# j04n-f/Encrypt-zkVM

Hardware: AMD Instinct MI355X
Metric: STARK prove: trace-steps/sec at 2^20 steps; achieved HBM GB/s vs 8 TB/s peak (higher is better)
Workload: dtype f128

## Files before the change

### encrypt-zkvm_amd/csrc/kernels.hip

```cpp
#include <hip/hip_runtime.h>
#include <bitset>
#include <mutex>
#include <stdlib.h>
#include <string.h>

#include "blake3.hpp"
#include "fri_small.hpp"
#include "rescue_consts.hpp"
#include "zk_internal.hpp"

namespace zk {

#define ZK_LAUNCH_CHECK() (void)hipGetLastError()

static inline unsigned cdiv(size_t a, size_t b) { return (unsigned)((a + b - 1) / b); }

__device__ __forceinline__ fe ld_fe(const fe *p) { return *p; }
__device__ __forceinline__ void st_fe(fe *p, fe v) { *p = v; }

template <class T>
__device__ __forceinline__ T pow_split(const T *lo, const T *hi, size_t t) {
    return ChalOf<T>::mul(lo[t & 2047], hi[t >> 11]);
}

// ... 1896 lines not shown
    comp_cross_mapped(st, m, T8n, inv3, scale, w8inv, inv3n, ncols, polys, nonzero_flag);
}

void comp_cross_mapped(hipStream_t st, const CrossMap &m, const NttTables &T8n, const PowTable &inv3, fe scale,
                       fe w8inv, fe inv3n, int ncols, fe *polys, unsigned *nonzero_flag) {
    unsigned blocks = cdiv(m.kcount, 256);
    if (blocks > 65536) blocks = 65536;
    ZK_PROF(st, "comp_cross", (128.0 + 16.0 * ncols) * m.kcount, hipLaunchKernelGGL(k_comp_cross, dim3(blocks), dim3(256), 0, st, m, T8n.inv_lo,
                                                 T8n.inv_hi, inv3.lo, inv3.hi, scale, w8inv, inv3n, ncols, polys,
                                                 nonzero_flag));
}

constexpr int OOD_GROUP = 7;

template <int KX>
__global__ void k_ood_tables(typename Chal<KX>::T z, typename Chal<KX>::T zg, uint64_t chunk, int nw,
                             typename Chal<KX>::T *tab) {
    typedef typename Chal<KX>::T T;
    const int t = blockIdx.x * blockDim.x + threadIdx.x;
    if (t >= 128 + 2 * nw) return;
    T x;
    uint64_t e;
    if (t < 128) {
        x = t < 64 ? z : zg;
        e = t & 63;
    } else {
        const int u = t - 128;
        x = u < nw ? z : zg;
        e = chunk * (uint64_t)(u < nw ? u : u - nw);
    }
    tab[t] = Chal<KX>::exp(x, e);
}

template <int KX, int E>
__global__ void __launch_bounds__(256) k_ood_eval(const fe *tpolys, int W, const fe *cpolys, int C, size_t n,
                                                  const typename Chal<KX>::T *tab, int nw, int w0, int w1,
                                                  fe *partials) {
    typedef Chal<KX> X;
    typedef typename X::T T;
    const int gw = w0 + (int)((blockIdx.x * blockDim.x + threadIdx.x) >> 6);
    const int lane = threadIdx.x & 63;
    const size_t plane = (size_t)(2 * W + C) * nw;
    const int tgroups = (W + OOD_GROUP - 1) / OOD_GROUP;
    const int g = blockIdx.y;
    const bool comp = g >= tgroups;
    const int p0 = comp ? 0 : g * OOD_GROUP;
    const int p1 = comp ? C : min(W, p0 + OOD_GROUP);
    const size_t base = (size_t)gw * 64 * E + lane;
    __shared__ T Y[2][E];
    if (threadIdx.x < 2 * E) {
        const int which = threadIdx.x / E, e = threadIdx.x % E;
        const T y = which ? X::mul(tab[127], tab[65]) : X::mul(tab[63], tab[1]);
        Y[which][e] = X::exp(y, (uint64_t)e);
    }
    __syncthreads();
    if (gw >= w1) return;
    const T wz = X::mul(tab[lane], tab[128 + gw]);
    const T wzg = comp ? X::zero() : X::mul(tab[64 + lane], tab[128 + nw + gw]);
    for (int p = p0; p < p1; p++) {
        const fe *c = (comp ? cpolys : tpolys) + (size_t)p * n;
        fe v[E];
#pragma unroll
        for (int e = 0; e < E; e++) {
            const size_t k = base + 64 * (size_t)e;
            v[e] = k < n ? c[k] : fe_zero();
        }
        const T hz = wave_sum(X::mul(dot_base<E>(v, Y[0]), wz));
        if (lane == 0) X::st(partials + (size_t)(comp ? 2 * W + p : p) * nw + gw, plane, hz);
        if (!comp) {
            const T hg = wave_sum(X::mul(dot_base<E>(v, Y[1]), wzg));
            if (lane == 0) X::st(partials + (size_t)(W + p) * nw + gw, plane, hg);
        }
    }
}

int ood_waves(size_t n) { return (int)std::max<size_t>(1, n / 1024); }

template <class T>
void ood_eval(hipStream_t st, const fe *tpolys, int W, const fe *cpolys, int C, int log_n, T z, T zg, fe *tab,
              fe *partials, fe *out, int rank, int G) {
    constexpr int KX = ChalOf<T>::KX;
    const size_t n = (size_t)1 << log_n;
    const int E = n >= 1024 ? 16 : std::max<int>(1, (int)(n / 64));
    const int nw = (int)((n + 64 * E - 1) / (64 * E));
    const int w0 = (int)((int64_t)nw * rank / G), w1 = (int)((int64_t)nw * (rank + 1) / G);
    T *t = reinterpret_cast<T *>(tab);
    hipLaunchKernelGGL(k_ood_tables<KX>, dim3(cdiv(128 + 2 * nw, 256)), dim3(256), 0, st, z, zg, (uint64_t)64 * E, nw, t);
    const dim3 grid(std::max(1u, cdiv(w1 - w0, 4)), (W + OOD_GROUP - 1) / OOD_GROUP + 1);
    const char *name = KX == 1 ? "ood_eval" : "ood_eval_ext";
#define ZK_OOD(EE) ZK_PROF(st, name, bytes, hipLaunchKernelGGL((k_ood_eval<KX, EE>), grid, dim3(256), 0, st, tpolys, W, cpolys, C, n, t, nw, w0, w1, partials))
    const double bytes = 16.0 * (W + C) * (double)n * (w1 - w0) / nw;
    switch (E) {
        case 16: ZK_OOD(16); break;
        case 8: ZK_OOD(8); break;
        case 4: ZK_OOD(4); break;
        case 2: ZK_OOD(2); break;
        default: ZK_OOD(1); break;
    }
#undef ZK_OOD
    sum_partials(st, partials, KX * (2 * W + C), nw, out, w0, w1);
}
template void ood_eval<fe>(hipStream_t, const fe *, int, const fe *, int, int, fe, fe, fe *, fe *, fe *, int, int);
template void ood_eval<fe2>(hipStream_t, const fe *, int, const fe *, int, int, fe2, fe2, fe *, fe *, fe *, int, int);

__global__ void k_sum_partials(const fe *partials, int nblk, int b0, int b1, fe *out) {
    __shared__ fe red[256];
    fe acc = fe_zero();
    for (int b = b0 + (int)threadIdx.x; b < b1; b += blockDim.x) acc = fe_add(acc, partials[(size_t)blockIdx.x * nblk + b]);
    red[threadIdx.x] = acc;
    __syncthreads();
    for (int s = 128; s > 0; s >>= 1) {
        if ((int)threadIdx.x < s) red[threadIdx.x] = fe_add(red[threadIdx.x], red[threadIdx.x + s]);
        __syncthreads();
    }
    if (threadIdx.x == 0) out[blockIdx.x] = red[0];
}

void sum_partials(hipStream_t st, const fe *partials, int npolys, int nblk, fe *out, int b0, int b1) {
    if (b1 < 0) b1 = nblk;
    hipLaunchKernelGGL(k_sum_partials, dim3(npolys), dim3(256), 0, st, partials, nblk, b0, b1, out);
}

constexpr int DIV_T = 256, DIV_E = 8, DIV_CH = DIV_T * DIV_E;
static_assert(DIV_CH == ZK_DEEP_RANGE_QUANTUM, "a sharded DEEP range is whole phase-3 chunks");
static_assert(DIV_T == ZK_DEEP_BLOCK, "DeepScratch counts phase-1 blocks");

template <int KX>
struct DeepPowBases {
    typename Chal<KX>::T b[4];
};
template <int KX>
__global__ void k_deep_pow_tables(DeepPowBases<KX> pb, size_t H, typename Chal<KX>::T *out) {
    const size_t per = 2048 + H;
    const size_t t = blockIdx.x * (size_t)blockDim.x + threadIdx.x;
    if (t >= 4 * per) return;
    const size_t b = t / per, e = t % per;
    const uint64_t ex = e < 2048 ? e : 2048 * (uint64_t)(e - 2048);
    out[t] = Chal<KX>::exp(pb.b[b], ex);
}

__device__ __forceinline__ fe block_sum256(fe v, fe *red) {
    v = wave_sum(v);
    const int w = threadIdx.x >> 6;
    if ((threadIdx.x & 63) == 0) red[w] = v;
    __syncthreads();
    fe r = red[0];
    for (int i = 1; i < DIV_T / 64; i++) r = fe_add(r, red[i]);
    __syncthreads();
    return r;
}

template <int KX>
__global__ void __launch_bounds__(DIV_T) k_deep_div_g(const fe *tpolys, const fe *cpolys, int ccols, size_t n,
                                                     const DeepConsts<KX> *D, const typename Chal<KX>::T *pw, size_t H,
                                                     typename Chal<KX>::T *g1, typename Chal<KX>::T *g2, fe *bs,
                                                     size_t kbase, size_t kend) {
    typedef Chal<KX> X;
    typedef typename X::T T;
    __shared__ fe red[DIV_T / 64];
    const size_t per = 2048 + H;
    const size_t k = kbase + blockIdx.x * (size_t)DIV_T + threadIdx.x;
    T v1 = X::zero(), v2 = X::zero();
    if (k < kend) {
        typename X::Acc aA = X::acc_zero();
#pragma unroll 4
        for (int c = 0; c < 28; c++) X::madd(aA, D->alpha_t[c], ld_fe(tpolys + (size_t)c * n + k));
        typename X::Acc aH = X::acc_zero();
        if constexpr (KX == 1) {
            for (int j = 0; j < ccols; j++) X::madd(aH, D->alpha_c[j], ld_fe(cpolys + (size_t)j * n + k));
        } else {
            for (int j = 0; j < ccols; j++) {
                const fe h0 = ld_fe(cpolys + (size_t)(2 * j) * n + k), h1 = ld_fe(cpolys + (size_t)(2 * j + 1) * n + k);
                const fe2 ac = D->alpha_c[j];
                acc288_madd(aH.a, ac.a, h0);
                acc288_madd(aH.a, ac.b, h1);
                acc288_madd(aH.b, ac.a, h1);
                acc288_madd(aH.b, ac.b, fe_add(h0, h1));
            }
        }
        const T A = X::reduce(aA);
        const T S = X::add(A, X::reduce(aH));
        v1 = X::mul(S, pow_split(pw, pw + 2048, k));
        v2 = X::mul(A, pow_split(pw + per, pw + per + 2048, k));
        g1[k] = v1;
        g2[k] = v2;
    }
    fe s[2 * KX];
#pragma unroll
    for (int c = 0; c < 2 * KX; c++) s[c] = block_sum256(X::comp(c < KX ? v1 : v2, c % KX), red);
    if (threadIdx.x == 0)
#pragma unroll
        for (int c = 0; c < 2 * KX; c++) bs[2 * KX * blockIdx.x + c] = s[c];
}

template <int NC>
__global__ void __launch_bounds__(1024) k_deep_div_scan(fe *bs, int nb, fe *total) {
    __shared__ fe t[NC][1024];
    const int per = (nb + 1023) / 1024, lo = threadIdx.x * per, hi = min(lo + per, nb);
    fe a[NC];
// ... 91 lines not shown
            if constexpr (!HOLD) r1 = X::add(r1, g1[k]), r2 = X::add(r2, g2[k]);
        }
        if constexpr (HOLD) r1 = X::add(r1, a[e]), r2 = X::add(r2, b[e]);
        pz = X::mul(pz, z);
        pg = X::mul(pg, zg);
    }
    if constexpr (KX == 1)
        if (rem_flag && k0 == 0 && !(fe_is_zero(r1) && fe_is_zero(r2))) atomicOr(rem_flag, 1u);
}

__global__ void __launch_bounds__(256) k_coset_to_natural(const fe *src, int log_n, int log_b, fe *out) {
    const size_t n = (size_t)1 << log_n, B = (size_t)1 << log_b, N = n << log_b;
    for (size_t i = blockIdx.x * (size_t)blockDim.x + threadIdx.x; i < N; i += (size_t)gridDim.x * blockDim.x)
        out[i] = ld_fe(src + (i & (B - 1)) * n + (i >> log_b));
}

void lde_cosets(hipStream_t st, const NttTables &Tn, const CosetTables &CT, const fe *coeffs, size_t n, size_t r0,
                size_t stride, int count, fe *out, fe *ntt_tmp) {
    ntt_lde(st, Tn, CT, coeffs, 0, 1, (int)r0, (int)stride, count, out, 0, n, ntt_tmp);
}

template <class T>
static void deep_tables(hipStream_t st, size_t n, T z, T zg, fe *scratch) {
    constexpr int KX = ChalOf<T>::KX;
    const DeepScratch S(scratch, n, KX);
    DeepPowBases<KX> pb;
    pb.b[0] = z;
    pb.b[1] = zg;
    pb.b[2] = ChalOf<T>::inv(z);
    pb.b[3] = ChalOf<T>::inv(zg);
    hipLaunchKernelGGL(k_deep_pow_tables<KX>, dim3(cdiv(4 * (2048 + S.H), 256)), dim3(256), 0, st, pb, S.H, (T *)S.pw);
}
template <class T>
static void deep_phase1(hipStream_t st, const fe *tpolys, const fe *cpolys, int ccols, size_t n,
                        const void *deep_consts_dev, fe *scratch, size_t k0, size_t kn, fe *total) {
    constexpr int KX = ChalOf<T>::KX;
    const DeepScratch S(scratch, n, KX);
    const size_t nb1 = (kn + DIV_T - 1) / DIV_T;
    ZK_PROF(st, "deep_combine", (16.0 * (28 + KX * ccols) + 32.0 * KX) * kn,
            hipLaunchKernelGGL(k_deep_div_g<KX>, dim3((unsigned)nb1), dim3(DIV_T), 0, st, tpolys, cpolys, ccols, n,
                               (const DeepConsts<KX> *)deep_consts_dev, (const T *)S.pw, S.H, (T *)S.g1, (T *)S.g2, S.bs, k0,
                               k0 + kn));
    hipLaunchKernelGGL(k_deep_div_scan<2 * KX>, dim3(1), dim3(1024), 0, st, S.bs, (int)nb1, total);
}
template <class T>
static void deep_phase3(hipStream_t st, size_t n, T z, T zg, fe *scratch, size_t k0, size_t kn, const fe *ext) {
    constexpr int KX = ChalOf<T>::KX;
    const DeepScratch S(scratch, n, KX);
    const size_t nb = (kn + DIV_CH - 1) / DIV_CH, nb1 = (kn + DIV_T - 1) / DIV_T;
    ZK_PROF(st, "deep_divide", KX * 48.0 * kn,
            hipLaunchKernelGGL((k_deep_div_q<KX, false>), dim3((unsigned)nb), dim3(DIV_T), 0, st, (const T *)S.g1,
                               (const T *)S.g2, S.bs, (int)nb1, k0 + kn, z, zg, (const T *)S.pw, S.H, S.out, n, nullptr, k0,
                               ext));
}
template <class T>
const fe *deep_poly(hipStream_t st, const fe *tpolys, const fe *cpolys, int ccols, int log_n,
                    const void *deep_consts_dev, T z, T zg, fe *scratch) {
    const size_t n = (size_t)1 << log_n;
    deep_tables(st, n, z, zg, scratch);
    deep_phase1<T>(st, tpolys, cpolys, ccols, n, deep_consts_dev, scratch, 0, n, nullptr);
    deep_phase3(st, n, z, zg, scratch, 0, n, nullptr);
    return DeepScratch(scratch, n, ChalOf<T>::KX).out;
}
template <class T>
const fe *deep_range_begin(hipStream_t st, const fe *tpolys, const fe *cpolys, int ccols, int log_n,
                           const void *deep_consts_dev, T z, T zg, fe *scratch, size_t k0, size_t kn) {
    const size_t n = (size_t)1 << log_n;
    deep_tables(st, n, z, zg, scratch);
    fe *total = DeepScratch(scratch, n, ChalOf<T>::KX).total;
    deep_phase1<T>(st, tpolys, cpolys, ccols, n, deep_consts_dev, scratch, k0, kn, total);
    return total;
}
template <class T>
const fe *deep_range_end(hipStream_t st, int log_n, T z, T zg, fe *scratch, size_t k0, size_t kn, const fe *ext) {
    const size_t n = (size_t)1 << log_n;
    deep_phase3(st, n, z, zg, scratch, k0, kn, ext);
    return DeepScratch(scratch, n, ChalOf<T>::KX).out;
}

struct BndPoly {
    fe cb[22];
    fe bnd1;
};
__global__ void __launch_bounds__(DIV_T) k_bnd_div_g(const fe *tpolys, size_t n, BndPoly bp, const fe *pw, size_t H,
                                                    fe *g1, fe *g2, fe *bs, size_t kbase, size_t kend) {
    __shared__ fe red[DIV_T / 64];
    const size_t per = 2048 + H;
    const size_t k = kbase + blockIdx.x * (size_t)DIV_T + threadIdx.x;
    fe v1 = fe_zero(), v2 = fe_zero();
    if (k < kend) {
        auto T = [&](int c) { return ld_fe(tpolys + (size_t)c * n + k); };
        acc288 a0 = acc288_zero(), a1 = acc288_zero();
        acc288_madd(a0, bp.cb[0], T(0));
        acc288_madd(a0, bp.cb[3], T(11));
        const fe t7 = T(7), t8 = T(8);
        acc288_madd(a0, bp.cb[1], t7);
        acc288_madd(a0, bp.cb[2], t8);
        acc288_madd(a1, bp.cb[12], t7);
        acc288_madd(a1, bp.cb[13], t8);
#pragma unroll
        for (int j = 0; j < 8; j++) {
            const fe c = T(12 + j);
            acc288_madd(a0, bp.cb[4 + j], c);
            acc288_madd(a1, bp.cb[14 + j], c);
        }
        v1 = acc288_reduce(a0);
        fe f1 = acc288_reduce(a1);
        if (k == 0) f1 = fe_sub(f1, bp.bnd1);
        v2 = fe_mul(f1, pow_split(pw + per, pw + per + 2048, k));
        g1[k] = v1;
        g2[k] = v2;
    }
    v1 = block_sum256(v1, red);
    v2 = block_sum256(v2, red);
    if (threadIdx.x == 0) {
        bs[2 * blockIdx.x] = v1;
        bs[2 * blockIdx.x + 1] = v2;
    }
}

static void bnd_tables_phase1(hipStream_t st, const fe *tpolys, size_t n, const AirConsts &K, fe c, fe *scratch,
                              size_t k0, size_t kn, fe *total) {
    const DeepScratch S(scratch, n, 1);
    const size_t nb1 = (kn + DIV_T - 1) / DIV_T;
    DeepPowBases<1> pb;
    pb.b[0] = fe_one();
    pb.b[1] = c;
    pb.b[2] = fe_one();
    pb.b[3] = fe_inv(c);
    hipLaunchKernelGGL(k_deep_pow_tables<1>, dim3(cdiv(4 * (2048 + S.H), 256)), dim3(256), 0, st, pb, S.H, S.pw);
    BndPoly bp;
    memcpy(bp.cb, K.coeff_b, sizeof bp.cb);
    bp.bnd1 = K.bnd1;
    ZK_PROF(st, "boundary_poly", (16.0 * 12 + 32.0) * kn,
            hipLaunchKernelGGL(k_bnd_div_g, dim3((unsigned)nb1), dim3(DIV_T), 0, st, tpolys, n, bp, S.pw, S.H, S.g1, S.g2,
                               S.bs, k0, k0 + kn));
    hipLaunchKernelGGL(k_deep_div_scan<2>, dim3(1), dim3(1024), 0, st, S.bs, (int)nb1, total);
}
static void bnd_phase3(hipStream_t st, size_t n, fe c, fe *scratch, size_t k0, size_t kn, const fe *ext, fe *col0,
                       unsigned *flag) {
    const DeepScratch S(scratch, n, 1);
    const size_t nb = (kn + DIV_CH - 1) / DIV_CH, nb1 = (kn + DIV_T - 1) / DIV_T;
    ZK_PROF(st, "boundary_poly", 64.0 * kn,
            hipLaunchKernelGGL((k_deep_div_q<1, true>), dim3((unsigned)nb), dim3(DIV_T), 0, st, S.g1, S.g2, S.bs, (int)nb1,
                               k0 + kn, fe_one(), c, S.pw, S.H, col0, 0, flag, k0, ext));
}

void boundary_poly_add(hipStream_t st, const fe *tpolys, int log_n, const AirConsts &K, fe c, fe *scratch, fe *col0,
                       unsigned *flag) {
    const size_t n = (size_t)1 << log_n;
    bnd_tables_phase1(st, tpolys, n, K, c, scratch, 0, n, nullptr);
    bnd_phase3(st, n, c, scratch, 0, n, nullptr, col0, flag);
}

const fe *boundary_range_begin(hipStream_t st, const fe *tpolys, int log_n, const AirConsts &K, fe c, fe *scratch,
                               size_t k0, size_t kn) {
    const size_t n = (size_t)1 << log_n;
    fe *total = DeepScratch(scratch, n, 1).total;
    bnd_tables_phase1(st, tpolys, n, K, c, scratch, k0, kn, total);
    return total;
}
void boundary_range_end(hipStream_t st, int log_n, fe c, fe *scratch, size_t k0, size_t kn, const fe *ext, fe *col0,
                        unsigned *flag) {
    bnd_phase3(st, (size_t)1 << log_n, c, scratch, k0, kn, ext, col0, flag);
}

template <class T>
void deep_coeff_launch(hipStream_t st, const NttTables &Tn, const fe *tpolys, const fe *cpolys, int ccols, int log_n,
                       int log_b, const void *deep_consts_dev, T z, T zg, const CosetTables &CT, fe *scratch,
                       fe *ulde, fe *ntt_tmp, fe *out) {
    constexpr int KX = ChalOf<T>::KX;
    const size_t n = (size_t)1 << log_n, B = (size_t)1 << log_b, N = n << log_b;
    const fe *Dk = deep_poly(st, tpolys, cpolys, ccols, log_n, deep_consts_dev, z, zg, scratch);
    for (int plane = 0; plane < KX; plane++) lde_cosets(st, Tn, CT, Dk + plane * n, n, 0, 1, (int)B, ulde + plane * N, ntt_tmp);
    if (!out) return;
    unsigned pb2 = cdiv(N, 256);
    if (pb2 > 65536) pb2 = 65536;
    for (int plane = 0; plane < KX; plane++)
        ZK_PROF(st, "deep", 32.0 * N,
                hipLaunchKernelGGL(k_coset_to_natural, dim3(pb2), dim3(256), 0, st, ulde + plane * N, log_n, log_b, out + plane * N));
}
#define ZK_DEEP_INSTANCES(T)                                                                                           \
    template const fe *deep_poly<T>(hipStream_t, const fe *, const fe *, int, int, const void *, T, T, fe *);          \
    template const fe *deep_range_begin<T>(hipStream_t, const fe *, const fe *, int, int, const void *, T, T, fe *,    \
                                           size_t, size_t);                                                            \
    template const fe *deep_range_end<T>(hipStream_t, int, T, T, fe *, size_t, size_t, const fe *);                    \
    template void deep_coeff_launch<T>(hipStream_t, const NttTables &, const fe *, const fe *, int, int, int,          \
                                       const void *, T, T, const CosetTables &, fe *, fe *, fe *, fe *);
ZK_DEEP_INSTANCES(fe)
ZK_DEEP_INSTANCES(fe2)
#undef ZK_DEEP_INSTANCES

__device__ __forceinline__ bool fe_canon_dev(uint32_t w0, uint32_t w1, uint32_t w2, uint32_t w3) {
    const uint64_t lo = (uint64_t)w0 | ((uint64_t)w1 << 32), hi = (uint64_t)w2 | ((uint64_t)w3 << 32);
    return !(hi == ZK_P_HI && lo >= ZK_P_LO);
}
__global__ void k_fri_coin(uint32_t *seed, const uint8_t *root, int k, fe *alpha_out, fe *alpha_log) {
    if (threadIdx.x != 0 || blockIdx.x != 0) return;
    uint32_t s[8], r[8], h[8];
    for (int i = 0; i < 8; i++) s[i] = seed[i];
    load_digest(root, r);
    b3::merge(s, r, h);
    for (int i = 0; i < 8; i++) seed[i] = h[i];
    for (uint32_t ctr = 1; ctr < 1000; ctr++) {
        uint32_t m[16] = {h[0], h[1], h[2], h[3], h[4], h[5], h[6], h[7], ctr, 0, 0, 0, 0, 0, 0, 0};
        uint32_t d[8];
        b3::iv(d);
        b3::compress(d, m, 0, 0, 40, b3::CHUNK_START | b3::CHUNK_END | b3::ROOT);
        if (fe_canon_dev(d[0], d[1], d[2], d[3]) && (k == 1 || fe_canon_dev(d[4], d[5], d[6], d[7]))) {
            const fe a0 = fe{(uint64_t)d[0] | ((uint64_t)d[1] << 32), (uint64_t)d[2] | ((uint64_t)d[3] << 32)};
            const fe a1 = fe{(uint64_t)d[4] | ((uint64_t)d[5] << 32), (uint64_t)d[6] | ((uint64_t)d[7] << 32)};
            alpha_out[0] = alpha_log[0] = a0;
            if (k == 2) alpha_out[1] = alpha_log[1] = a1;
            return;
        }
    }
}

void fri_coin_launch(hipStream_t st, uint32_t *seed_dev, const uint8_t *root_dev, int k, fe *alpha_dev,
                     fe *alpha_log) {
// ... 179 lines not shown
```

### encrypt-zkvm_amd/csrc/prover.hip

```cpp
#include <hip/hip_runtime.h>
#include <stdio.h>
#include <string.h>

#include <algorithm>
#include <chrono>
#include <cstdlib>
#include <map>
#include <memory>
#include <new>
#include <string>
#include <vector>

#include "host_pool.hpp"
#include "prover_internal.hpp"
#include "rescue_consts.hpp"

namespace zk {
thread_local std::string g_err;
struct HostTimer {
    bool on = getenv("ZK_HOST_TIMING") != nullptr;
    std::chrono::steady_clock::time_point t = std::chrono::steady_clock::now();
    std::string log;
    void start() { t = std::chrono::steady_clock::now(); }
    void stop(const char *what) {
// ... 485 lines not shown
    out->hint_redos = p->hint_redos;
    for (const auto &h : p->hint_sets) out->hint_sets += h.n != 0 && h.have ? 1u : 0u;
    out->hinted_sparse = p->tc.sp_hinted;
    out->derived = p->tc.clk_used ? 1u : 0u;
    for (int i = 0; i < zk_prover::ZK_FIXED_SNAPS; i++) {
        const auto &s = p->fix_snaps[i];
        out->fixed_sets += s.live && s.owner >= 0 && p->hint_sets[s.owner].snap == i ? 1u : 0u;
    }
    return ZK_OK;
}

int zk_prover_upload_stats(zk_prover *p, uint64_t *bytes, uint32_t *sparse_cols, uint32_t *narrow8_cols,
                           uint32_t *narrow32_cols) {
    if (!p) ZK_FAIL(ZK_ERR_INVALID_ARG, "null prover");
    if (bytes) *bytes = p->tc.up_bytes;
    if (sparse_cols) *sparse_cols = p->tc.up_sparse;
    if (narrow8_cols) *narrow8_cols = p->tc.up_nw8;
    if (narrow32_cols) *narrow32_cols = p->tc.up_nw32;
    return ZK_OK;
}

int zk_prover_upload_derived(zk_prover *p, uint32_t *derived_cols) {
    if (!p || !derived_cols) ZK_FAIL(ZK_ERR_INVALID_ARG, "null argument");
    *derived_cols = p->tc.clk_used ? 1u : 0u;
    return ZK_OK;
}

int zk_prover_upload_fixed(zk_prover *p, uint32_t *fixed_cols) {
    if (!p || !fixed_cols) ZK_FAIL(ZK_ERR_INVALID_ARG, "null argument");
    *fixed_cols = p->tc.fix_used;
    return ZK_OK;
}

int zk_prover_exchange_stats_ex(zk_prover *p, const char **names, float *ms, float *exposed_ms, double *bytes,
                                int *calls, int cap, int *count) {
    if (!p) ZK_FAIL(ZK_ERR_INVALID_ARG, "null prover");
    std::vector<const char *> nm;
    std::vector<float> t, w;
    std::vector<double> b;
    std::vector<int> c;
    if (p->stage_done)
        for (const auto &r : p->xchg) {
            float x = 0, y = 0;
            (void)hipEventElapsedTime(&x, p->xchg_pool[r.ev], p->xchg_pool[r.ev + 1]);
            if (r.waited) (void)hipEventElapsedTime(&y, p->xchg_pool[r.ev + 2], p->xchg_pool[r.ev + 3]);
            size_t i = 0;
            while (i < nm.size() && strcmp(nm[i], r.name)) i++;
            if (i == nm.size()) {
                nm.push_back(r.name);
                t.push_back(0);
                w.push_back(0);
                b.push_back(0);
                c.push_back(0);
            }
            t[i] += x;
            w[i] += y;
            b[i] += r.bytes;
            c[i] += 1;
        }
    const int k = (int)nm.size();
    for (int i = 0; i < k && i < cap; i++) {
        if (names) names[i] = nm[i];
        if (ms) ms[i] = t[i];
        if (exposed_ms) exposed_ms[i] = w[i];
        if (bytes) bytes[i] = b[i];
        if (calls) calls[i] = c[i];
// ... 525 lines not shown
    return d2h_small(p, root, nodes + 32, 32);
}

static void coset_major_rows_to_host(zk_prover *p, const fe *base, int ncols, size_t n, uint32_t B, uint8_t *dst) {
    size_t N = n * B;
    std::vector<fe> h((size_t)ncols * N);
    (void)hipMemcpy(h.data(), base, h.size() * sizeof(fe), hipMemcpyDeviceToHost);
    fe *o = reinterpret_cast<fe *>(dst);
    for (int c = 0; c < ncols; c++)
        for (size_t i = 0; i < N; i++) o[i * ncols + c] = h[((size_t)c * B + (i % B)) * n + i / B];
}

int zk::ensure_ext(zk_prover *p) {
    if (p->x_comp) return ZK_OK;
    const size_t n = p->max_n, N = n * p->max_b, CE = 8 * n;
    const size_t Nl = p->shard_world ? N / (size_t)p->shard_world : N;
    DeviceArena &A = p->arena;
    ZK_CHECK_HIP(A.alloc(&p->x_comp, 2 * CE));
    ZK_CHECK_HIP(A.alloc(&p->x_ctmp, 2 * CE));
    ZK_CHECK_HIP(A.alloc(&p->x_clde, (size_t)2 * 8 * Nl));
    ZK_CHECK_HIP(A.alloc(&p->x_deep, 2 * Nl));
    ZK_CHECK_HIP(A.alloc(&p->x_fri, 2 * (N + 16)));
    ZK_CHECK_HIP(A.alloc(&p->x_partials, (size_t)2 * (2 * ZK_MAX_COLS + ZK_MAX_CCOLS) * ood_waves(n)));
    ZK_CHECK_HIP(A.alloc(&p->x_tab, (size_t)2 * (128 + 2 * ood_waves(n))));
    ZK_CHECK_HIP(A.alloc((uint8_t **)&p->x_air, 2 * sizeof(AirConsts)));
    ZK_CHECK_HIP(A.alloc((uint8_t **)&p->x_deep_consts, sizeof(DeepConsts<2>)));
    ZK_CHECK_HIP(A.alloc((uint8_t **)&p->x_fold_consts, sizeof(FoldConsts<2>)));
    if (!p->shard_world) ZK_CHECK_HIP(A.alloc(&p->x_ulde, 2 * N));
    ZK_CHECK_HIP(A.alloc(&p->x_dscratch, DeepScratch::size(n, 2)));
    return ZK_OK;
}

static int composition_stage(zk_prover *p, Plan *pl, int KX, int C, fe *comp, fe *ctmp, fe *clde, uint8_t root[32],
                             const AirConsts *bnd = nullptr, int nce = 8) {
    const size_t n = (size_t)1 << pl->log_n, CE = 8 * n;
    const int CK = C * KX;
    if (nce != 8 && (nce != 7 || C > 7)) ZK_FAIL(ZK_ERR_INVALID_ARG, "composition: unsupported CE coset count");
    if (nce == 8) ntt(p->st, pl->Tn, comp, n, ctmp, n, 8 * KX, true, nullptr, nullptr, p->tmp);
    else
        for (int j = 0; j < KX; j++) ntt(p->st, pl->Tn, comp + j * CE, n, ctmp + j * CE, n, nce, true, nullptr, nullptr, p->tmp);
    ZK_CHECK_HIP(hipMemsetAsync(p->flag, 0, 4, p->st));
    const fe w8 = h_root_of_unity(3);
    for (int j = 0; j < KX; j++) {
        CrossMap m;
        for (int r = 0; r < 8; r++) m.c[r] = ctmp + (size_t)(8 * j + r) * n;
        m.k0 = 0;
        m.kcount = n;
        m.pstride = (size_t)KX * n;
        if (nce == 7) {
            m.derive7 = 1;
            fe w = w8;
            for (int r = 0; r < 7; r++, w = fe_mul(w, w8)) m.k7[r] = fe_sub(fe_zero(), w);
        }
        comp_cross_mapped(p->st, m, pl->Tce, pl->inv3, h_inv(fe_make(CE)), h_inv(w8), h_inv(h_pow(fe_make(3), n)), C,
                          p->cpolys + (size_t)j * n, p->flag);
    }
    if (bnd)
        for (int j = 0; j < KX; j++)
            boundary_poly_add(p->st, p->polys, pl->log_n, bnd[j], bnd[0].g_last2, p->dscratch, p->cpolys + (size_t)j * n,
                              p->flag);
    return lde_commit(p, pl, p->cpolys, CK, clde, p->cleaves, p->cnodes, root);
}

static int check_ood_identity(const std::vector<fe2> &e, int C, const AirConsts *K, int KX, fe2 z, size_t n,
                              const zk_pub_inputs *pub) {
    fe2 ct[NUM_TCONS], cb[NUM_ASSERTS];
    for (int k = 0; k < NUM_TCONS; k++) ct[k] = fe2{K[0].coeff_t[k], KX == 2 ? K[1].coeff_t[k] : fe_zero()};
    for (int k = 0; k < NUM_ASSERTS; k++) cb[k] = fe2{K[0].coeff_b[k], KX == 2 ? K[1].coeff_b[k] : fe_zero()};
    if (!ood_identity(e.data(), C, ct, cb, z, n, pub))
        ZK_FAIL(ZK_ERR_DEGREE, "the trace does not satisfy ProcessorAir (out-of-domain constraint identity failed)");
    return ZK_OK;
}

static int prove_once(zk_prover *p, const TraceSrc &src, size_t n, const zk_options *opt, const zk_pub_inputs *pub,
                      uint8_t *proof_out, size_t *proof_len, zk_record *rec, const zk_dump *dump);

static int prove_impl(zk_prover *p, TraceSrc src, size_t n, const zk_options *opt, const zk_pub_inputs *pub,
                      uint8_t *proof_out, size_t *proof_len, zk_record *rec, const zk_dump *dump) {
    if (dump) src.no_virtual = true;
    if (src.cols && pub) {
        src.key = &pub->program_hash[0][0];
        src.lwe = pub->lwe_size;
    }
    p->tc = {};
    const size_t cap = proof_len ? *proof_len : 0;
    int rc = prove_once(p, src, n, opt, pub, proof_out, proof_len, rec, dump);
    if (trace_hints_refuted(p, src, n, rc)) {
        src.hint_ok = false;
        *proof_len = cap;
        rc = prove_once(p, src, n, opt, pub, proof_out, proof_len, rec, dump);
    }
    trace_hints_learn(p, src, n, rc);
    return rc;
// ... 50 lines not shown
    if (ht) {
        ht->stop("fri_replay");
        ht->start();
    }
    return remainder_step(KX, rv, B, coin, R, degree_flag, Y.rem_flat);
}

void Openings::unpack(const fe *got, size_t nu, int CK, const std::vector<std::vector<uint64_t>> &fri_pos,
                      uint32_t fold, int KX, size_t off_dig) {
    trace_rows.assign(got, got + nu * W);
    size_t off = nu * W;
    comp_rows.assign(got + off, got + off + nu * CK);
    off += nu * CK;
    for (size_t l = 0; l < fri_rows.size(); l++) {
        fri_rows[l].assign(got + off, got + off + fri_pos[l].size() * fold * KX);
        off += fri_pos[l].size() * fold * KX;
    }
    const uint8_t *dg = (const uint8_t *)(got + off_dig);
    for (size_t b = 0; b < plans.size(); b++) {
        const size_t bytes = 32 * plans[b].count();
        digests[b].assign(dg, dg + bytes);
        dg += bytes;
    }
}

template <int KX>
static int ood_deep_stage(zk_prover *p, Plan *pl, Coin &coin, zk_record &R, HostTimer &HT, int C, const AirConsts *Kp,
                          const zk_pub_inputs *pub, fe *deep_out, std::vector<fe> &h) {
    typedef Chal<KX> X;
    const Planes b = planes(p, KX);
    const int log_n = pl->log_n;
    const typename X::T z = X::make(coin.draw_ext(KX)), zg = X::mulb(z, h_root_of_unity(log_n));
    fe_to_bytes(X::comp(z, 0), R.z);
    ood_eval(p->st, p->polys, W, p->cpolys, C * KX, log_n, z, zg, b.ood_tab, b.partials, p->ood);
    HT.stop("z");
    std::vector<fe> hv((size_t)KX * (2 * W + C * KX));
    ZK_TRY(d2h_small(p, hv.data(), p->ood, hv.size() * sizeof(fe)));
    ZK_TRY(d2h_flush(p));
    HT.start();
    std::vector<fe2> e;
    ood_reseed(coin, KX, hv, C, R, e, h);
    stage_mark(p, "ood");
    const DeepConsts<KX> D = draw_deep_consts<KX>(coin, e, C, z, zg, R);
    ZK_TRY(h2d_small(p, b.deep_consts, &D, sizeof D));
    deep_coeff_launch(p->st, pl->Tn, p->polys, p->cpolys, C, log_n, pl->log_b, b.deep_consts, z, zg, pl->ct, b.dscratch,
                      b.ulde, p->tmp, deep_out);
    HT.stop("deep_consts");
    return check_ood_identity(e, C, Kp, KX, X::wide(z), (size_t)1 << log_n, pub);
}

static int prove_once(zk_prover *p, const TraceSrc &src, size_t n, const zk_options *opt, const zk_pub_inputs *pub,
                      uint8_t *proof_out, size_t *proof_len, zk_record *rec, const zk_dump *dump) {
    if (!p || !proof_len) ZK_FAIL(ZK_ERR_INVALID_ARG, "null argument");
    ZK_REQUIRE_FULL_PROVER(p);
    ZK_TRY(check_prove_args(n, p->max_n, p->max_b, opt, pub));
    DeviceBusy busy{p->dev_busy};
    struct CopyGuard {
        zk_prover *p;
        ~CopyGuard() {
            upload_drain(p);
            (void)hipStreamSynchronize(p->st);
        }
    } copy_guard{p};
    const int sched = p->upload_sched;
    p->lat_sched = sched == ZK_SCHED_LATENCY || (sched == ZK_SCHED_AUTO && busy.others == 0);
    p->last_sched = src.cols ? (p->lat_sched ? ZK_SCHED_LATENCY : ZK_SCHED_THROUGHPUT) : 0;
    const uint32_t B = opt->blowup, fold = opt->fri_folding;
    const size_t N = n * B;
    ZK_CHECK_HIP(hipSetDevice(p->device));
    IoScope io_scope(p);
    Plan *pl = nullptr;
    ZK_TRY(get_plan(p, n, B, &pl));
    const int log_n = pl->log_n, log_b = pl->log_b;
    const int C = num_comp_cols(n);
    if (C > 8) ZK_FAIL(ZK_ERR_INVALID_ARG, "composition column count exceeds 8");
    zk_record R = record_init(n, N, C);
    stage_begin(p);
    stage_mark(p, "start");

    Coin coin = seed_coin(n, opt, pub);

    ZK_TRY(trace_lde_commit(p, pl, src, n, R.trace_root));
    ZK_TRY(d2h_flush(p));
    stage_mark(p, "trace_commit");
    HostTimer HT;
    HT.start();
    coin.reseed(R.trace_root);

    const int KX = (int)opt->field_extension, CK = C * KX;
    if (KX == 2) ZK_TRY(ensure_ext(p));
    const Planes pb = planes(p, KX);
    fe *comp = pb.comp, *ctmp = pb.ctmp, *clde = pb.clde, *deep = pb.deep;
    const bool bnd_rows = dump && dump->composition;
    const int nce = (!bnd_rows && C <= 7) ? 7 : 8;
    AirConsts Kp[2];
    draw_air_consts(coin, pub, n, KX, Kp, R);
    ZK_TRY(h2d_small(p, pb.air_consts, Kp, KX * sizeof Kp[0]));
    const fe *binv = boundary_inverses(p, pl);
    if (!binv) ZK_FAIL(ZK_ERR_OUT_OF_MEMORY, "boundary divisor table");
    ZK_CHECK_HIP((KX == 1 ? eval_constraints : eval_constraints_ext)(p->st, p->lde, log_n, log_b, pl->periodic, binv,
                                                                     (const AirConsts *)pb.air_consts, comp, bnd_rows, nce));
    HT.stop("air_consts");
    stage_mark(p, "constraints");

    ZK_TRY(composition_stage(p, pl, KX, C, comp, ctmp, clde, R.constraint_root, bnd_rows ? nullptr : Kp, nce));
    unsigned degree_flag = 0;
    ZK_TRY(d2h_small(p, &degree_flag, p->flag, 4));
    ZK_TRY(d2h_flush(p));
    stage_mark(p, "composition");
    HT.start();
    coin.reseed(R.constraint_root);

    const int nl = fri_num_layers(N, opt);
    const int lb0 = nl > 0 ? log_b : 0;
    std::vector<fe> h;
    ZK_TRY(with_kx(KX, [&](auto kx) {
        return ood_deep_stage<decltype(kx)::value>(p, pl, coin, R, HT, C, Kp, pub, lb0 ? nullptr : deep, h);
    }));
    stage_mark(p, "deep");

    if (nl > ZK_MAX_FRI_LAYERS) ZK_FAIL(ZK_ERR_INVALID_ARG, "too many FRI layers");
    R.num_fri_layers = (uint32_t)nl;
    {
        size_t tot = 0, s = N;
        for (int l = 0; l < nl; l++) tot += (s /= fold);
        if (tot > p->max_n * p->max_b) ZK_FAIL(ZK_ERR_INVALID_ARG, "FRI layers exceed the prover's buffers");
    }
    FriLayers Y(nl);
    const fe *deep0 = lb0 ? pb.ulde : deep;
    Y.vals[0] = deep0;
    Y.len[0] = N;
    ZK_TRY(fri_lead_layers(p, pl, KX, fold, B, N, 0, lb0, pb.fri, p->fri_dig, Y, coin, R, degree_flag, &HT));
    stage_mark(p, "fri");

    HT.stop("remainder");
    HT.start();
    std::vector<uint64_t> pos;
    ZK_TRY(grind_and_positions(p, coin, opt, N, R, pos));
// ... 224 lines not shown
    return ZK_OK;
}

static int validate_first(zk_prover *p, const void *d_trace, const uint8_t *const *cols, size_t n, const zk_options *opt,
                          const zk_pub_inputs *pub, size_t *proof_len) {
    if (!p || !p->validate || !proof_len || p->shard_world > 1) return ZK_OK;
    if (check_prove_args(n, p->max_n, p->max_b, opt, pub) != ZK_OK) return ZK_OK;
    zk_validation v;
    const int rc = cols ? zk_validate_columns(p, cols, n, pub, &v) : zk_validate_device(p, d_trace, n, pub, &v);
    if (rc != ZK_OK) *proof_len = 0;
    return rc;
}

int zk_prove_device(zk_prover *p, const void *d_trace, size_t n, const zk_options *opt, const zk_pub_inputs *pub,
                    uint8_t *proof_out, size_t *proof_len, zk_record *rec, const zk_dump *dump) {
    if (!d_trace) ZK_FAIL(ZK_ERR_INVALID_ARG, "null argument");
    ZK_TRY(validate_first(p, d_trace, nullptr, n, opt, pub, proof_len));
    TraceSrc src;
    src.dev = (const fe *)d_trace;
    return prove_impl(p, src, n, opt, pub, proof_out, proof_len, rec, dump);
}

int zk::fixed_prefix(zk_prover *p, size_t n, uint32_t B, const FixedCols &fx) {
    p->fix_prefix_blocks = 0;
    Plan *pl = nullptr;
    ZK_TRY(get_plan(p, n, B, &pl));
    if (!p->fix_ws) ZK_CHECK_HIP(p->arena.alloc(&p->fix_ws, W));
    fe_ws ws[W];
    for (int c = 0; c < W; c++) ws[c] = make_fe_ws(fx.last[c]);
    ZK_TRY(h2d_small(p, p->fix_ws, ws, sizeof ws));
    constexpr int nb = 12 / 4;
    const size_t Bn = n << pl->log_b;
    if (fixed_fuse_on()) {
        fixed_axpy(p->st, fx, p->fix_ws, n, (size_t)1 << pl->log_b, p->polys, p->lde, 4 * nb);
        FixedHashCols A{};
        for (int c = 0; c < 4 * nb; c++) {
            A.mode[c] = FixedHashCols::FORM;
            A.src[c] = fx.flde + (size_t)c * Bn;
            A.wsi[c] = (uint8_t)c;
        }
        fixed_hash(p->st, A, fx.lagr_lde, p->fix_ws, p->lde, W, pl->log_n, pl->log_b, nb, p->leaves);
    } else {
        fixed_axpy(p->st, fx, p->fix_ws, n, (size_t)1 << pl->log_b, p->polys, p->lde);
        hash_rows_blocks(p->st, p->lde, W, pl->log_n, pl->log_b, 0, nb, p->leaves);
    }
    p->fix_prefix_blocks = nb;
    return ZK_OK;
}

int zk::prove_fixed(zk_prover *p, size_t n, const zk_options *opt, const zk_pub_inputs *pub, const FixedCols *fx,
                    uint8_t *proof_out, size_t *proof_len) {
    TraceSrc src;
    src.dev = p->d_trace;
    src.fixed = fx;
    return prove_impl(p, src, n, opt, pub, proof_out, proof_len, nullptr, nullptr);
}

int zk::prove_single(zk_prover *p, const uint8_t *trace, size_t n, const zk_options *opt, const zk_pub_inputs *pub,
                     uint8_t *proof_out, size_t *proof_len, zk_record *rec) {
    const uint8_t *cols[W];
    TraceSrc src;
    if (trace) {
        for (int c = 0; c < W; c++) cols[c] = trace + (size_t)c * n * sizeof(fe);
        src.cols = cols;
    } else {
        src.dev = p->d_trace;
    }
    return prove_impl(p, src, n, opt, pub, proof_out, proof_len, rec, nullptr);
}

int zk_prove_columns_ex(zk_prover *p, const uint8_t *const *columns, size_t n, const zk_options *opt,
                        const zk_pub_inputs *pub, uint8_t *proof_out, size_t *proof_len, zk_record *rec,
                        const zk_dump *dump) {
    if (!columns) ZK_FAIL(ZK_ERR_INVALID_ARG, "null argument");
    for (int c = 0; c < W; c++)
        if (!columns[c]) ZK_FAIL(ZK_ERR_INVALID_ARG, "null trace column");
// ... 182 lines not shown
    uint8_t r[32];
    if ((rc = composition_stage(p, pl, 1, (int)num_cols, p->comp, p->ctmp, p->clde, r))) return rc;
    unsigned degree_flag = 0;
    if ((rc = d2h_small(p, &degree_flag, p->flag, 4)) || (rc = d2h_flush(p))) return rc;
    if (degree_flag) ZK_FAIL(ZK_ERR_DEGREE, "composition polynomial degree exceeds num_cols * trace_len");
    if (polys_out)
        ZK_CHECK_HIP(hipMemcpy(polys_out, p->cpolys, (size_t)num_cols * n * sizeof(fe), hipMemcpyDeviceToHost));
    if (root) memcpy(root, r, 32);
    *out = new zk_comp_commit{p, n, h->B, (int)num_cols};
    return ZK_OK;
}

int zk_comp_query(zk_comp_commit *h, const uint64_t *positions, size_t k, uint8_t *rows_out, uint8_t *proof_out,
                  size_t *proof_len) {
    if (!h) ZK_FAIL(ZK_ERR_INVALID_ARG, "null argument");
    zk_prover *p = h->p;
    return query_committed_rows(p, p->clde, h->ncols, h->n, h->B, p->cleaves, p->cnodes, positions, k, rows_out,
                                proof_out, proof_len);
}

void zk_comp_free(zk_comp_commit *h) { delete h; }

extern "C" void zk_diag_dot_host(const uint8_t *a, const uint8_t *b, size_t count, uint8_t *out) {
    acc288 acc = acc288_zero();
    for (size_t i = 0; i < count; i++) acc288_madd(acc, fe_from_bytes(a + 16 * i), fe_from_bytes(b + 16 * i));
    fe_to_bytes(acc288_reduce(acc), out);
}

extern "C" void zk_diag_mul_limbs_host(const uint8_t *a, const uint8_t *b, uint8_t *out, size_t count) {
    for (size_t i = 0; i < count; i++) fe_to_bytes(fe_mul_limbs(fe_from_bytes(a + 16 * i), fe_from_bytes(b + 16 * i)), out + 16 * i);
}
extern "C" void zk_diag_blake3_host(const uint8_t *in, size_t len, uint8_t out[32]) { b3::hash_bytes(in, len, out); }

extern "C" int zk_diag_upload_plan(const uint32_t *in, size_t n, uint32_t *masks, int32_t *counts, int32_t *cols,
                                   int32_t *width, uint64_t *off, int32_t *pb, int32_t *gsz) {
    UploadPlanIn q;
    q.have = in[0], q.sparse = in[1], q.nw8 = in[2], q.nw32 = in[3], q.clk_off = in[4], q.fixed_off = in[5];
    q.snap = in[6], q.snap_mask = in[7], q.hint_ok = in[8], q.no_virtual = in[9], q.lat_sched = in[10], q.detect = in[11];
    q.sparse_on = in[12] & 1u, q.narrow_on = in[12] & 2u, q.clock_on = in[12] & 4u, q.fixed_on = in[12] & 8u;
    q.fixed_fuse_on = in[12] & 16u, q.virtual_on = in[12] & 32u;
    q.n = n;
    const UploadPlan u = upload_plan(q);
    const uint32_t m[8] = {u.hint, u.nw8, u.nw32, u.clk, u.fixm, u.virt, u.snap_now, u.lat};
    const int32_t k[7] = {u.nd, u.nh, u.nhv, u.nn, u.np, u.ngroups, u.fuse_nb};
    memcpy(masks, m, sizeof m);
    memcpy(counts, k, sizeof k);
    for (int i = 0; i < W; i++) {
        cols[i] = i < u.nd ? u.dense[i] : -1;
        cols[W + i] = i < u.nh ? u.hin[i] : -1;
        cols[2 * W + i] = i < u.nhv ? u.hnv[i] : -1;
        cols[3 * W + i] = i < u.nn ? u.nar[i] : -1;
        width[i] = i < u.nn ? u.width[i] : 0;
        off[i] = i < u.nn ? u.off[i] : 0;
        gsz[i] = i < u.ngroups ? u.gsz[i] : 0;
    }
    off[W] = u.pack_bytes;
    for (int i = 0; i <= W; i++) pb[i] = i <= u.np ? u.pb[i] : -1;
    if (u.status != ZK_OK) ZK_FAIL(u.status, "too many upload groups");
    return ZK_OK;
}

extern "C" int zk_diag_shard_rounds(const int32_t *U, int nU, int G, int rep, int32_t *out, size_t cap, int32_t *rounds) {
    if (!U || !out || !rounds || nU < 0 || nU > W || rep < 0 || rep > nU || (G != 2 && G != 4 && G != 8))
        ZK_FAIL(ZK_ERR_INVALID_ARG, "zk_diag_shard_rounds: up to 28 columns, 0 <= rep <= nU, G = 2, 4 or 8");
    const ShardRounds r = shard_round_plan(U, nU, G, rep);
    if (cap < (size_t)r.rounds * (3 + 2 * G)) ZK_FAIL(ZK_ERR_BUFFER_TOO_SMALL, "zk_diag_shard_rounds: out too small");
    for (int k = 0; k < r.rounds; k++) {
        int32_t *o = out + (size_t)k * (3 + 2 * G);
        o[0] = G * k, o[1] = r.real(k), o[2] = r.inplace(k);
        for (int g = 0; g < G; g++) {
            o[3 + g] = r.column(k, g);
            o[3 + G + g] = r.inplace(k) ? r.first(k) + g : -1;
        }
    }
    *rounds = r.rounds;
// ... 129 lines not shown
static bool diag_read_fe(const uint8_t *b, int ext, fe2 *out) {
    out->a = fe_from_bytes(b);
    out->b = ext == 2 ? fe_from_bytes(b + 16) : fe_zero();
    return fe_canonical(out->a) && fe_canonical(out->b);
}
static int diag_back_half_args(const char *who, const void *tpolys, const void *cpolys, int ccols, size_t n, int ext,
                               const uint8_t *z, const uint8_t *zg, const void *out, fe2 *zv, fe2 *zgv) {
    const bool ok = tpolys && cpolys && z && zg && out && n >= 16 && !(n & (n - 1)) && n <= ((size_t)1 << 22) &&
                    (ext == 1 ? ccols >= 1 && ccols <= 8 : ext == 2 && ccols >= 2 && ccols <= 16 && ccols % 2 == 0);
    if (!ok || !diag_read_fe(z, ext, zv) || !diag_read_fe(zg, ext, zgv))
        ZK_FAIL(ZK_ERR_INVALID_ARG, std::string(who) + ": n a power of two in [16, 2^22]; ext 1 with 1 .. 8 composition "
                                    "columns or ext 2 with 2, 4 .. 16 base columns; z and zg canonical");
    return ZK_OK;
}
static int diag_back_half_upload(zk_prover *p, const uint8_t *tpolys, const uint8_t *cpolys, int ccols, size_t n, int ext) {
    if (ext == 2) ZK_TRY(ensure_ext(p));
    ZK_CHECK_HIP(hipMemcpy(p->polys, tpolys, (size_t)W * n * 16, hipMemcpyHostToDevice));
    ZK_CHECK_HIP(hipMemcpy(p->cpolys, cpolys, (size_t)ccols * n * 16, hipMemcpyHostToDevice));
    return ZK_OK;
}

extern "C" int zk_diag_ood(int device, const uint8_t *tpolys, const uint8_t *cpolys, int ccols, size_t n, int ext,
                           const uint8_t *z, const uint8_t *zg, int rank, int G, uint8_t *out) {
    fe2 zv, zgv;
    ZK_TRY(diag_back_half_args("zk_diag_ood", tpolys, cpolys, ccols, n, ext, z, zg, out, &zv, &zgv));
    if (G < 1 || G > 64 || rank < 0 || rank >= G) ZK_FAIL(ZK_ERR_INVALID_ARG, "zk_diag_ood: 0 <= rank < G <= 64");
    zk_prover *p = nullptr;
    ZK_TRY(zk_prover_create(device, n, 8, &p));
    std::unique_ptr<zk_prover, void (*)(zk_prover *)> guard(p, zk_prover_destroy);
    ZK_TRY(diag_back_half_upload(p, tpolys, cpolys, ccols, n, ext));
    const Planes b = planes(p, ext);
    with_kx(ext, [&](auto kx) {
        typedef Chal<decltype(kx)::value> X;
        ood_eval(p->st, p->polys, W, p->cpolys, ccols, ilog2(n), X::make(zv), X::make(zgv), b.ood_tab, b.partials, p->ood, rank, G);
        return 0;
    });
    ZK_CHECK_HIP(hipStreamSynchronize(p->st));
    ZK_CHECK_HIP(hipMemcpy(out, p->ood, (size_t)ext * (2 * W + ccols) * 16, hipMemcpyDeviceToHost));
    return ZK_OK;
}

static int diag_deep(int device, const uint8_t *tpolys, const uint8_t *cpolys, int ccols, size_t n, int ext,
                     const uint8_t *z, const uint8_t *zg, const uint8_t *alpha_t, const uint8_t *alpha_c, int parts,
                     uint8_t *out) {
    fe2 zv, zgv;
    ZK_TRY(diag_back_half_args("zk_diag_deep", tpolys, cpolys, ccols, n, ext, z, zg, out, &zv, &zgv));
    if (!alpha_t || !alpha_c) ZK_FAIL(ZK_ERR_INVALID_ARG, "zk_diag_deep: null argument");
    if ((fe_is_zero(zv.a) && fe_is_zero(zv.b)) || (fe_is_zero(zgv.a) && fe_is_zero(zgv.b)))
        ZK_FAIL(ZK_ERR_INVALID_ARG, "zk_diag_deep: z and zg must be non-zero (their inverses are taken)");
    const int C = ccols / ext, log_n = ilog2(n);
    fe2 at[W], ac[8];
    for (int c = 0; c < W + C; c++)
        if (!diag_read_fe((c < W ? alpha_t + 16 * ext * c : alpha_c + 16 * ext * (c - W)), ext, c < W ? &at[c] : &ac[c - W]))
            ZK_FAIL(ZK_ERR_INVALID_ARG, "zk_diag_deep: non-canonical coefficient");
    zk_prover *p = nullptr;
    ZK_TRY(zk_prover_create(device, n, 8, &p));
    std::unique_ptr<zk_prover, void (*)(zk_prover *)> guard(p, zk_prover_destroy);
    ZK_TRY(diag_back_half_upload(p, tpolys, cpolys, ccols, n, ext));
    const Planes b = planes(p, ext);
    return with_kx(ext, [&](auto kx) -> int {
        constexpr int KX = decltype(kx)::value;
        typedef Chal<KX> X;
        const typename X::T z = X::make(zv), zg = X::make(zgv);
        DeepConsts<KX> D;
        memset(&D, 0, sizeof D);
        for (int c = 0; c < W; c++) D.alpha_t[c] = X::make(at[c]);
        for (int c = 0; c < C; c++) D.alpha_c[c] = X::make(ac[c]);
        D.z = z, D.zg = zg;
        ZK_CHECK_HIP(hipMemcpy(b.deep_consts, &D, sizeof D, hipMemcpyHostToDevice));
        const fe *Dk = nullptr;
        if (parts == 1) {
            Dk = deep_poly(p->st, p->polys, p->cpolys, C, log_n, b.deep_consts, z, zg, b.dscratch);
        } else {
            const DeepScratch S(b.dscratch, n, KX);
            const size_t kn = n / parts, nc = 2 * KX, ncarry = nc * (kn / ZK_DEEP_BLOCK);
            std::vector<fe> tot((size_t)parts * nc);
            for (int g = 0; g < parts; g++) {
                const fe *t = deep_range_begin(p->st, p->polys, p->cpolys, C, log_n, b.deep_consts, z, zg, b.dscratch, g * kn, kn);
                ZK_CHECK_HIP(hipMemcpyAsync(p->comp + g * ncarry, S.bs, ncarry * sizeof(fe), hipMemcpyDeviceToDevice, p->st));
                ZK_CHECK_HIP(hipMemcpyAsync(&tot[g * nc], t, nc * sizeof(fe), hipMemcpyDeviceToHost, p->st));
            }
            ZK_CHECK_HIP(hipStreamSynchronize(p->st));
            std::vector<fe> later((size_t)parts * nc, fe_zero());
            for (int g = parts - 2; g >= 0; g--)
                for (size_t c = 0; c < nc; c++) later[g * nc + c] = fe_add(later[(g + 1) * nc + c], tot[(g + 1) * nc + c]);
            ZK_CHECK_HIP(hipMemcpy(p->ood, later.data(), later.size() * sizeof(fe), hipMemcpyHostToDevice));
            for (int g = 0; g < parts; g++) {
                ZK_CHECK_HIP(hipMemcpyAsync(S.bs, p->comp + g * ncarry, ncarry * sizeof(fe), hipMemcpyDeviceToDevice, p->st));
                Dk = deep_range_end(p->st, log_n, z, zg, b.dscratch, g * kn, kn, p->ood + g * nc);
            }
        }
        ZK_CHECK_HIP(hipStreamSynchronize(p->st));
        ZK_CHECK_HIP(hipMemcpy(out, Dk, (size_t)KX * n * 16, hipMemcpyDeviceToHost));
        return ZK_OK;
    });
}
extern "C" int zk_diag_deep(int device, const uint8_t *tpolys, const uint8_t *cpolys, int ccols, size_t n, int ext,
                            const uint8_t *z, const uint8_t *zg, const uint8_t *alpha_t, const uint8_t *alpha_c,
                            uint8_t *out) {
    return diag_deep(device, tpolys, cpolys, ccols, n, ext, z, zg, alpha_t, alpha_c, 1, out);
}
extern "C" int zk_diag_deep_parts(int device, const uint8_t *tpolys, const uint8_t *cpolys, int ccols, size_t n, int ext,
                                  const uint8_t *z, const uint8_t *zg, const uint8_t *alpha_t, const uint8_t *alpha_c,
                                  int parts, uint8_t *out) {
    if (parts < 2 || parts > 8 || (parts & (parts - 1)) || n < (size_t)parts * ZK_DEEP_RANGE_QUANTUM)
        ZK_FAIL(ZK_ERR_INVALID_ARG, "zk_diag_deep_parts: 2, 4 or 8 ranges of at least 2048 coefficients");
    return diag_deep(device, tpolys, cpolys, ccols, n, ext, z, zg, alpha_t, alpha_c, parts, out);
}

extern "C" int zk_diag_fri_layer(int device, const uint8_t *layer, size_t L, int ext, int fold, int lb, size_t wstride,
                                 const uint8_t *alpha, uint8_t *root_out, uint8_t *next_out) {
    fe2 av;
    const size_t N = L * wstride;
    const bool ok = layer && alpha && root_out && next_out && (ext == 1 || ext == 2) &&
                    (fold == 2 || fold == 4 || fold == 8 || fold == 16) && L && !(L & (L - 1)) && wstride &&
                    !(wstride & (wstride - 1)) && L >= 4 * (size_t)fold && N >= 128 && N <= ((size_t)1 << 22) && lb >= 0 &&
                    ((size_t)1 << lb) <= L / fold;
    if (!ok || !diag_read_fe(alpha, ext, &av))
        ZK_FAIL(ZK_ERR_INVALID_ARG, "zk_diag_fri_layer: L and wstride powers of two, 128 <= L wstride <= 2^22, fold 2 .. 16, "
                                    "at least 4 rows, 2^lb <= L / fold, alpha canonical");
    zk_prover *p = nullptr;
    ZK_TRY(zk_prover_create(device, N / 8, 8, &p));
    std::unique_ptr<zk_prover, void (*)(zk_prover *)> guard(p, zk_prover_destroy);
    Plan *pl = nullptr;
    ZK_TRY(get_plan(p, N / 8, 8, &pl));
    if (ext == 2) ZK_TRY(ensure_ext(p));
    const Planes b = planes(p, ext);
    const size_t rows = L / fold;
    uint8_t *leaves = p->fri_dig, *nodes = leaves + 32 * rows;
    ZK_CHECK_HIP(hipMemcpy(b.deep, layer, (size_t)ext * L * 16, hipMemcpyHostToDevice));
    ZK_TRY(with_kx(ext, [&](auto kx) -> int {
        const auto F = fold_consts<decltype(kx)::value>(av, (uint32_t)fold);
        ZK_CHECK_HIP(hipMemcpy(b.fold_consts, &F, sizeof F, hipMemcpyHostToDevice));
        return ZK_OK;
    }));
    commit_fri_layer(p->st, ext, b.deep, L, fold, leaves, nodes, lb);
    fri_fold_launch(p->st, ext, b.deep, L, fold, b.fold_consts, pl->TN, wstride, b.fri, lb);
    ZK_CHECK_HIP(hipStreamSynchronize(p->st));
    ZK_CHECK_HIP(hipMemcpy(root_out, nodes + 32, 32, hipMemcpyDeviceToHost));
    ZK_CHECK_HIP(hipMemcpy(next_out, b.fri, (size_t)ext * rows * 16, hipMemcpyDeviceToHost));
// ... 22 lines not shown
```

### encrypt-zkvm_amd/csrc/prover_internal.hpp

```cpp
#pragma once
#include <hip/hip_runtime.h>
#include <stdlib.h>
#include <string.h>

#include <atomic>
#include <map>
#include <memory>
#include <mutex>
#include <string>
#include <vector>

#include "../../include/zkvm_gpu.h"
#include "air_shape.hpp"
#include "host_field.hpp"
#include "shard_plan.hpp"
#include "upload_plan.hpp"
#include "zk_internal.hpp"

namespace zk {

extern thread_local std::string g_err;

#define ZK_CHECK_HIP(expr)                                                                     \
    do {                                                                                       \
// ... 150 lines not shown
    HintSet hint_sets[ZK_HINT_SETS];
    struct FixedSnap {
        bool live = false;
        int owner = -1;
        size_t n = 0;
        uint32_t B = 0, lwe = 0;
        uint32_t mask = 0;
        int k = 0;
        uint8_t slot[zk::W] = {}, width[zk::W] = {};
        fe *fpolys = nullptr, *flde = nullptr;
        size_t cap_polys = 0, cap_lde = 0;
        std::unique_ptr<uint8_t[]> host[zk::W];
        uint64_t used = 0;
    };
    static constexpr int ZK_FIXED_SNAPS = 2;
    FixedSnap fix_snaps[ZK_FIXED_SNAPS];
    uint64_t hint_stamp = 0;
    uint32_t hint_redos = 0;
    unsigned *sp_h = nullptr;
    uint8_t *h_pack = nullptr;
    size_t h_pack_cap = 0;
    struct TraceOutcome {
        bool sp_used = false;
        uint32_t sp_hinted = 0, sp_bad = 0;
        bool clk_used = false, clk_bad = false;
        uint32_t fix_used = 0;
        bool fix_bad = false;
        int fix_pending = -1;
        uint64_t up_bytes = 0;
        uint32_t up_sparse = 0, up_nw8 = 0, up_nw32 = 0;
        uint32_t virt = 0;
        fe virt_last[28] = {};
        const fe *virt_lagr = nullptr;
    } tc;
    uint32_t sh_sparse = 0, sh_nw8 = 0, sh_nw32 = 0;
    bool sh_clock = false;
    size_t sh_hint_n = 0, sh_clock_off_n = 0;
    int sh_hint_g = 0;
    uint8_t sh_hint_key[32] = {};
    fe *sh_buf = nullptr;
    fe *sh_xr = nullptr;
    fe *sh_zero = nullptr;
    uint8_t *sh_roots = nullptr;
    uint8_t *sh_blk = nullptr, *sh_cblk = nullptr, *sh_fblk = nullptr;
    uint8_t *sh_f1blk = nullptr;
    unsigned *sh_flags = nullptr;
    fe *x_comp = nullptr, *x_ctmp = nullptr, *x_clde = nullptr, *x_deep = nullptr, *x_fri = nullptr,
       *x_partials = nullptr, *x_tab = nullptr;
    void *x_air = nullptr, *x_deep_consts = nullptr, *x_fold_consts = nullptr;
    uint32_t *pow_seed = nullptr;
    unsigned long long *pow_best = nullptr;
    std::map<std::pair<int, int>, std::unique_ptr<zk::Plan>> plans;
    std::vector<hipEvent_t> stage_pool;
    std::vector<const char *> stage_names;
    bool stage_done = false;
    std::vector<std::pair<const char *, float>> stage_ms;
    struct XchgRec {
        const char *name;
        double bytes;
        size_t ev;
        int op;
        bool waited;
    };
    std::vector<hipEvent_t> xchg_pool;
    size_t xchg_next = 0;
    std::vector<XchgRec> xchg;
    struct SchedEnt {
// ... 45 lines not shown
        ZK_CHECK_HIP(hipEventRecord(ev, st));
        return ZK_OK;
    }
    ~UploadEvent() {
        if (!done) (void)hipEventRecord(ev, st);
    }
};

struct FixedCols {
    int md;
    const fe *fpolys;
    const fe *flde;
    const fe *lagr;
    const fe *lagr_lde;
    fe last[W];
};
struct TraceSrc {
    const fe *dev = nullptr;
    const uint8_t *const *cols = nullptr;
    const FixedCols *fixed = nullptr;
    bool hint_ok = true;
    bool no_virtual = false;
    const uint8_t *key = nullptr;
    uint32_t lwe = 0;
};
int trace_lde_commit(zk_prover *p, Plan *pl, const TraceSrc &src, size_t n, uint8_t root[32]);
bool trace_hints_refuted(zk_prover *p, const TraceSrc &src, size_t n, int rc);
void trace_hints_learn(zk_prover *p, const TraceSrc &src, size_t n, int rc);
int ensure_pack(zk_prover *p, size_t bytes);
int sparse_begin(zk_prover *p, Plan *pl, SparseCols *out, const SparseCols **sp);
int prove_fixed(zk_prover *p, size_t n, const zk_options *opt, const zk_pub_inputs *pub, const FixedCols *fx,
                uint8_t *proof_out, size_t *proof_len);
void fixed_axpy(hipStream_t st, const FixedCols &fx, const fe_ws *ws_dev, size_t n, size_t B, fe *polys, fe *lde,
                int lde_c0 = 0);
struct FixedColList {
    int count = 0;
    uint8_t col[W], slot[W];
};
void fixed_cols_axpy(hipStream_t st, const FixedColList &L, bool snapshot, const fe *src_polys, const fe *src_lde,
                     const fe *lagr, const fe *lagr_lde, const fe_ws *ws_dev, size_t n, size_t B, fe *polys, fe *lde,
                     int lde_c0 = 0);
bool fixed_on();
bool fixed_fuse_on();
bool same_rows(const uint8_t *col, const uint8_t *snap, size_t r0, size_t r1, int width);
int fixed_prefix(zk_prover *p, size_t n, uint32_t B, const FixedCols &fx);
bool sparse_on();
bool clock_on();
bool narrow_on();
bool pack_rows(const uint8_t *col, size_t r0, size_t r1, int width, uint8_t *dst);
int clock_tables(zk_prover *p, Plan *pl);
bool zero_rows(const uint8_t *col, size_t r0, size_t r1);
bool clock_rows(const uint8_t *col, size_t r0, size_t r1);
int prove_sharded_entry(zk_comm *comm, zk_prover **provers, int nlocal, const uint8_t *trace, size_t n,
                        const zk_options *opt, const zk_pub_inputs *pub, uint8_t *proof_out, size_t *proof_len,
                        zk_record *rec, const FixedCols *fixed);
int shard_rank_of(const zk_comm *comm, int l);

int prove_single(zk_prover *p, const uint8_t *trace, size_t n, const zk_options *opt, const zk_pub_inputs *pub,
                 uint8_t *proof_out, size_t *proof_len, zk_record *rec);

inline uint8_t *io_take(zk_prover *p, size_t len) {
    const size_t a = (len + 63) & ~(size_t)63;
    if (p->io_used + a > p->io_cap) return nullptr;
    uint8_t *r = p->h_io + p->io_used;
    p->io_used += a;
    return r;
}
inline int h2d_small(zk_prover *p, void *dst_dev, const void *src, size_t len) {
    uint8_t *s = io_take(p, len);
    if (!s) ZK_FAIL(ZK_ERR_OUT_OF_MEMORY, "pinned staging area exhausted");
    memcpy(s, src, len);
    ZK_CHECK_HIP(hipMemcpyAsync(dst_dev, s, len, hipMemcpyHostToDevice, p->st));
    return ZK_OK;
}
// ... 151 lines not shown
```

### encrypt-zkvm_amd/csrc/shard.hip

```cpp
#include <hip/hip_runtime.h>
#include <string.h>

#include <algorithm>
#include <array>
#include <atomic>
#include <memory>
#include <string>
#include <type_traits>
#include <vector>

#include "blake3.hpp"
#include "comm.hpp"
#include "fri_small.hpp"
#include "host_pool.hpp"
#include "prover_internal.hpp"

using namespace zk;

namespace {

static inline unsigned cdiv(size_t a, size_t b) { return (unsigned)((a + b - 1) / b); }

struct LoopbackComm : zk_comm {
    bool loopback() const override { return true; }
// ... 818 lines not shown
    }
    size_t recv0() const { return (size_t)KX * Bl * n; }
    int constraints() {
        ZK_TRY(air_tables());
        hs.assign(Bl, XH{});
        for (int j = 0; j < Bl; j++) {
            ZK_TRY(each_rank(X, [this, j](int l, zk_prover *p, Plan *pl) -> int {
                const EvalMap em{1, X.rank[l] * Bl + j, 1, 0, Bl, (size_t)Bl * n};
                const Planes b = pb(p);
                if (KX == 1)
                    ZK_CHECK_HIP(eval_constraints_mapped(p->st, p->lde + (size_t)j * n, log_n, em, pl->periodic,
                                                         pl->sh_divs + (size_t)j * n, (const AirConsts *)p->air_consts,
                                                         p->comp + (size_t)j * n, !range_split));
                else
                    ZK_CHECK_HIP(eval_constraints_ext_mapped(p->st, p->lde + (size_t)j * n, log_n, em, pl->periodic,
                                                             pl->sh_divs + (size_t)j * n, (const AirConsts *)p->x_air,
                                                             (size_t)Bl * n, p->x_comp + (size_t)j * n, !range_split));
                fe *scr = p->tmp, *send = scr + (size_t)KX * n * (1 + j);
                ntt(p->st, pl->Tn, b.comp + (size_t)j * n, (size_t)Bl * n, b.ctmp + (size_t)j * n, (size_t)Bl * n, KX, true,
                    nullptr, nullptr, scr);
                hipLaunchKernelGGL(k_sh_pack_coset, dim3(cdiv((size_t)KX * n, 256)), dim3(256), 0, p->st,
                                   (const fe *)b.ctmp + (size_t)j * n, (size_t)Bl * n, log_n, KX, ilog2(kg), send);
                xb.set(l, send, b.comp + recv0() + (size_t)j * KX * n);
                return ZK_OK;
            }));
            ZK_TRY(xchg_start(X, "comp_slices", A2A, xb, (size_t)KX * kg * sizeof(fe), &hs[j]));
        }
        stage_mark(P0, "constraints");
        return ZK_OK;
    }

    int boundary_begin(int pln) {
        return each_rank(X, [this, pln](int l, zk_prover *p, Plan *) -> int {
            const void *sums = boundary_range_begin(p->st, p->polys, log_n, Kp[pln], K.g_last2, p->dscratch,
                                                    (size_t)X.rank[l] * kg, kg);
            xb.set(l, sums, p->sh_buf);
            return ZK_OK;
        });
    }
    int cross_step() {
        const fe scale = h_inv(fe_make(8 * n)), w8inv = h_inv(h_root_of_unity(3)), inv3n = h_inv(h_pow(fe_make(3), n));
        return each_rank(X, [=](int l, zk_prover *p, Plan *pl) -> int {
            const Planes b = pb(p);
            ZK_CHECK_HIP(hipMemsetAsync(p->flag, 0, 4, p->st));
            for (int pln = 0; pln < KX; pln++) {
                CrossMap cm;
                for (int r = 0; r < 8; r++)
                    cm.c[r] = b.comp + recv0() + ((size_t)(r % Bl) * G * KX + (size_t)(r / Bl) * KX + pln) * kg;
                cm.k0 = (size_t)X.rank[l] * kg;
                cm.kcount = kg;
                cm.pstride = (size_t)KX * kg;
                comp_cross_mapped(p->st, cm, pl->Tce, pl->inv3, scale, w8inv, inv3n, C, b.ctmp + pln * kg, p->flag);
            }
            return ZK_OK;
        });
    }
    int start_columns(int c0, int c1) {
        for (int c = c0; c < c1; c++)
            ZK_TRY(xchg_start(X, "comp_columns", AG, bufs([this, c](int, zk_prover *p) {
                return SR{pb(p).ctmp + c * kg, p->cpolys + (size_t)c * n};
            }), kg * sizeof(fe), &hc[c]));
        return ZK_OK;
    }
    int boundary_quotient(XH &hb0) {
        for (int pln = 0; range_split && pln < KX; pln++) {
            if (pln == 0) {
                ZK_TRY(xchg_wait(X, hb0));
            } else {
// ... 85 lines not shown
        ZK_TRY(xchg(X, "deep_totals", AG, xb, (size_t)nc * sizeof(fe)));
        ZK_TRY(each_rank(X, [this, end, nc](int l, zk_prover *p, Plan *) -> int {
            hipLaunchKernelGGL(k_sh_suffix_carry, dim3(1), dim3(64), 0, p->st, p->sh_buf, G, X.rank[l], nc, p->ood);
            Dk[l] = end(p, (size_t)X.rank[l] * kg, p->ood);
            return ZK_OK;
        }));
        XH hp[2];
        for (int plane = 0; plane < kx; plane++)
            ZK_TRY(xchg_start(X, "deep_slices", AG, bufs([this, plane](int l, zk_prover *) {
                fe *d = const_cast<fe *>(Dk[l]) + (size_t)plane * n;
                return SR{d + (size_t)X.rank[l] * kg, d};
            }), kg * sizeof(fe), &hp[plane]));
        for (int plane = 0; plane < kx; plane++) ZK_TRY(xchg_wait(X, hp[plane]));
        return ZK_OK;
    }
    int lde_deep() {
        ZK_TRY(each_rank(X, [this](int l, zk_prover *p, Plan *pl) -> int {
            for (int plane = 0; plane < KX; plane++)
                lde_cosets(p->st, pl->Tn, pl->ct, Dk[l] + plane * n, n, X.rank[l] * Bl, 1, Bl,
                           pb(p).deep + (size_t)plane * Bl * n, p->tmp);
            return ZK_OK;
        }));
        stage_mark(P0, "deep");
        return ZK_OK;
    }
    template <int KX_>
    int ood_deep_kx() {
        typedef Chal<KX_> XF;
        typedef typename XF::T T;
        const T z = XF::make(coin.draw_ext(KX_)), zg = XF::mulb(z, g);
        fe_to_bytes(XF::comp(z, 0), R.z);
        std::vector<fe> hv;
        ZK_TRY(ood_parts(KX_ * (2 * W + CK), [this, z, zg](zk_prover *p, int rank) {
            ood_eval(p->st, p->polys, W, p->cpolys, CK, log_n, z, zg, pb(p).ood_tab, pb(p).partials, p->ood, rank, G);
        }, hv));
        std::vector<fe2> e;
        ood_reseed(coin, KX_, hv, C, R, e, h);
        stage_mark(P0, "ood");
        const DeepConsts<KX_> D = draw_deep_consts<KX_>(coin, e, C, z, zg, R);
        auto upload = [this, D](zk_prover *p) { return h2d_small(p, pb(p).deep_consts, &D, sizeof D); };
        if (range_split) {
            ZK_TRY(deep_split_ranges(KX_, [this, z, zg](zk_prover *p, size_t k0) {
                return deep_range_begin(p->st, p->polys, p->cpolys, C, log_n, pb(p).deep_consts, z, zg, pb(p).dscratch, k0, kg);
            }, [this, z, zg](zk_prover *p, size_t k0, const fe *ext) {
                return deep_range_end(p->st, log_n, z, zg, pb(p).dscratch, k0, kg, ext);
            }, upload));
        } else {
            ZK_TRY(each_rank(X, [this, z, zg, upload](int l, zk_prover *p, Plan *) -> int {
                ZK_TRY(upload(p));
                Dk[l] = deep_poly(p->st, p->polys, p->cpolys, C, log_n, pb(p).deep_consts, z, zg, pb(p).dscratch);
                return ZK_OK;
            }));
        }
        return lde_deep();
    }
    int ood_deep() {
        return with_kx(KX, [this](auto kx) { return ood_deep_kx<decltype(kx)::value>(); });
    }

    void permute_gathered(const fe *stage, size_t mg) {
        for (int pln = 0; pln < KX; pln++)
            hipLaunchKernelGGL(k_sh_permute, dim3(cdiv(8 * mg, 256)), dim3(256), 0, P0->st,
                               (const uint8_t *)(stage + (size_t)pln * Bl * mg), G, Bl, ilog2(mg), 16, (size_t)KX * Bl * mg,
                               (uint8_t *)(pb(P0).fri + pln * 8 * mg));
    }
    int fri_none() {
        ZK_TRY(xchg(X, "remainder_layer", AG, bufs([this](int, zk_prover *p) { return SR{pb(p).deep, pb(p).comp}; }),
                    (size_t)KX * Bl * n * sizeof(fe)));
        ZK_TRY(lead_segment(X));
        ZK_CHECK_HIP(hipSetDevice(P0->device));
        permute_gathered(pb(P0).comp, n);
        std::vector<fe> rv(KX * N);
        ZK_TRY(d2h_small(P0, rv.data(), pb(P0).fri, rv.size() * sizeof(fe)));
        ZK_TRY(d2h_flush(P0));
        return remainder_step(KX, rv, 8, coin, R, degree_flag, Y.rem_flat);
    }
    int commit_sharded_layer(int layer, DistTree &T, bool ctmp, int log_len, int log_rows, const char *digests,
                             const char *roots) {
        ZK_TRY(dist_commit(X, T, rows0 >> (layer * ilog2(fold)), [=, &T](int l, uint8_t *send, int log_QG, int log_K, int k) {
            zk_prover *p = X.P[l];
            const fe *vals = ctmp ? pb(p).ctmp : pb(p).deep;
            with_bl(Bl, [=, &T](auto bl) {
                launch_fri0_blk<decltype(bl)::value>(p->st, KX, vals, log_len, (int)fold, log_rows, log_QG, log_K, k,
// ... 376 lines not shown
```

### encrypt-zkvm_amd/csrc/trace_commit.hip

```cpp
#include <hip/hip_runtime.h>
#include <string.h>

#include <new>

#include "host_pool.hpp"
#include "prover_internal.hpp"

using namespace zk;

bool zk::sparse_on() { static const bool on = env_switch("ZK_SPARSE"); return on; }
bool zk::narrow_on() { static const bool on = env_switch("ZK_NARROW"); return on; }
bool zk::clock_on() { static const bool on = env_switch("ZK_CLOCK"); return on; }
bool zk::fixed_on() { static const bool on = env_switch("ZK_FIXED"); return on; }
bool zk::fixed_fuse_on() { static const bool on = env_switch("ZK_FIXED_FUSE"); return on; }
static bool virtual_on() { static const bool on = env_switch("ZK_VIRTUAL"); return on; }

static void fixed_drop(zk_prover *p, int i) {
    if (i < 0) return;
    zk_prover::FixedSnap &s = p->fix_snaps[i];
    if (s.owner >= 0 && p->hint_sets[s.owner].snap == i) p->hint_sets[s.owner].snap = -1;
    s.live = false;
    s.owner = -1;
    s.mask = 0;
    for (auto &h : s.host) h.reset();
    if (p->tc.fix_pending == i) p->tc.fix_pending = -1;
}

static int fixed_slot(zk_prover *p, int owner, size_t n, uint32_t B, int k) {
    const size_t np = (size_t)k * n, nl = np * B;
    int best = -1;
    for (int i = 0; i < zk_prover::ZK_FIXED_SNAPS; i++) {
        const auto &s = p->fix_snaps[i];
        if (s.live) continue;
        if (best < 0 || (s.cap_polys == np && s.cap_lde == nl)) best = i;
    }
    if (best < 0) {
        best = 0;
        for (int i = 1; i < zk_prover::ZK_FIXED_SNAPS; i++)
            if (p->fix_snaps[i].used < p->fix_snaps[best].used) best = i;
        fixed_drop(p, best);
    }
    zk_prover::FixedSnap &s = p->fix_snaps[best];
    if (s.cap_polys != np || s.cap_lde != nl) {
        (void)hipFree(s.fpolys);
        (void)hipFree(s.flde);
        s.fpolys = s.flde = nullptr;
        s.cap_polys = s.cap_lde = 0;
        if (hipMalloc((void **)&s.fpolys, np * sizeof(fe)) != hipSuccess ||
// ... 134 lines not shown
        ZK_TRY(clock_tables(p, pl));
        out->id_poly = pl->id_poly;
        out->id_lde = pl->id_lde;
        out->idoff = 3 * W;
    }
    *sp = out;
    return ZK_OK;
}

int zk::ensure_pack(zk_prover *p, size_t bytes) {
    if (bytes <= p->h_pack_cap) return ZK_OK;
    if (p->h_pack) (void)hipHostFree(p->h_pack);
    p->h_pack = nullptr;
    p->h_pack_cap = 0;
    ZK_CHECK_HIP(hipHostMalloc((void **)&p->h_pack, bytes, hipHostMallocMapped | hipHostMallocCoherent));
    p->h_pack_cap = bytes;
    return ZK_OK;
}


static int upload_trace_group(zk_prover *p, const TraceSrc &src, size_t n, int c0, int nc) {
    const size_t col = n * sizeof(fe);
    p->tc.up_bytes += (uint64_t)nc * col;
    for (int c = c0; c < c0 + nc;) {
        int e = c + 1;
        while (e < c0 + nc && src.cols[e] == src.cols[e - 1] + col) e++;
        ZK_CHECK_HIP(hipMemcpyAsync(p->d_trace + (size_t)c * n, src.cols[c], (size_t)(e - c) * col, hipMemcpyHostToDevice,
                                    p->up));
        c = e;
    }
    return ZK_OK;
}

static int commit_device_fixed(zk_prover *p, Plan *pl, const TraceSrc &src, size_t n, uint8_t root[32]) {
    const FixedCols &fx = *src.fixed;
    const fe inv_n = h_inv(fe_make(n));
    const size_t B = (size_t)1 << pl->log_b, c0 = 12;
    if (fx.md > 0) {
        ntt(p->st, pl->Tn, src.dev + c0 * n, n, p->polys + c0 * n, n, fx.md, true, nullptr, &inv_n, p->tmp);
        ntt_lde(p->st, pl->Tn, pl->ct, p->polys + c0 * n, n, fx.md, 0, 1, (int)B, p->lde + c0 * B * n, B * n, n, p->tmp);
    }
    const int pre = p->fix_prefix_blocks;
    p->fix_prefix_blocks = 0;
    if (pre) {
        hash_rows_blocks(p->st, p->lde, W, pl->log_n, pl->log_b, pre, W / 4, p->leaves);
    } else {
        if (!p->fix_ws) ZK_CHECK_HIP(p->arena.alloc(&p->fix_ws, W));
        fe_ws ws[W];
        for (int c = 0; c < W; c++) ws[c] = make_fe_ws(fx.last[c]);
        ZK_TRY(h2d_small(p, p->fix_ws, ws, sizeof ws));
        fixed_axpy(p->st, fx, p->fix_ws, n, B, p->polys, p->lde);
        hash_rows_cosets(p->st, p->lde, W, pl->log_n, pl->log_b, 0, pl->log_b, p->leaves);
    }
    merkle_tree(p->st, p->leaves, n * B, p->nodes);
    return d2h_small(p, root, p->nodes + 32, 32);
}

static int commit_device(zk_prover *p, Plan *pl, const TraceSrc &src, size_t n, const SparseCols *sp, uint8_t root[32]) {
    const fe inv_n = h_inv(fe_make(n));
    const size_t B = (size_t)1 << pl->log_b;
    if (sp) sparse_detect(p->st, src.dev, n, 0, W, *sp);
    ntt(p->st, pl->Tn, src.dev, n, p->polys, n, W, true, nullptr, &inv_n, p->tmp, sp);
    ntt_lde(p->st, pl->Tn, pl->ct, p->polys, n, W, 0, 1, (int)B, p->lde, B * n, n, p->tmp, sp);
    hash_rows_cosets(p->st, p->lde, W, pl->log_n, pl->log_b, 0, pl->log_b, p->leaves);
    merkle_tree(p->st, p->leaves, n * B, p->nodes);
    return d2h_small(p, root, p->nodes + 32, 32);
}

namespace {

struct HostTraceCommit {
    zk_prover *const p;
    Plan *const pl;
    const TraceSrc &src;
    const size_t n, B;
    SparseCols spc;
    const SparseCols *const sp;
    const fe inv_n = h_inv(fe_make(n));
    zk_prover::HintSet *H = nullptr;
    bool fresh = false;
    zk_prover::FixedSnap *FS = nullptr;
    zk_prover::FixedSnap *snap = nullptr;
    UploadPlan u;
    bool ready[W] = {};
// ... 6 lines not shown
        const int *cols = nullptr;
        int nc = 0, part = -1, ev = 0;
    };
    int fallback[W], nfb = 0, good[W], ev = 0, gi = 0, di = 0;
    bool narrow_done[2] = {}, fb_done = false;
    NarrowCols G[W] = {};
    size_t part_off[W + 1];
    uint8_t *const stage = reinterpret_cast<uint8_t *>(p->ctmp);

    HostTraceCommit(zk_prover *p_, Plan *pl_, const TraceSrc &s, size_t n_, const SparseCols &c, bool detect)
        : p(p_), pl(pl_), src(s), n(n_), B((size_t)1 << pl_->log_b), spc(c), sp(detect ? &spc : nullptr) {}
    ~HostTraceCommit() {
        for (auto &l : packed) l.wait();
        for (Latch *l : {&checked, &clocked, &compared, &copied}) l->wait();
    }

    void classify() {
        H = sp && src.hint_ok ? hint_find(p, n, src.key) : nullptr;
        UploadPlanIn in;
        fresh = H && H->have;
        if (H) {
            in.have = H->have, in.sparse = H->sparse, in.nw8 = H->nw8, in.nw32 = H->nw32;
            in.clk_off = H->clk_off, in.fixed_off = H->fixed_off;
            if (H->snap >= 0) {
                zk_prover::FixedSnap &s = p->fix_snaps[H->snap];
                if (s.live && s.n == n && s.B == B && s.lwe == src.lwe) FS = &s;
            }
            in.snap = FS != nullptr;
            in.snap_mask = FS ? FS->mask : 0u;
        }
        in.hint_ok = src.hint_ok, in.no_virtual = src.no_virtual, in.lat_sched = p->lat_sched, in.detect = sp != nullptr;
        in.sparse_on = sparse_on(), in.narrow_on = narrow_on(), in.clock_on = clock_on();
        in.fixed_on = fixed_on(), in.fixed_fuse_on = fixed_fuse_on(), in.virtual_on = virtual_on(), in.n = n;
        u = upload_plan(in);
        if (!u.fix_ok) FS = nullptr;
        else if (!FS && H->snap >= 0) fixed_drop(p, H->snap);
        if (FS) FS->used = ++p->hint_stamp;
        zk_prover::TraceOutcome &tc = p->tc;
        tc.clk_used = u.clk;
        tc.fix_used = u.fixm;
        tc.clk_bad = tc.fix_bad = false;
        tc.fix_pending = -1;
        tc.sp_hinted = tc.up_sparse = u.hint;
        tc.up_nw8 = u.nw8 & u.fixm;
        tc.up_nw32 = u.nw32 & u.fixm;
        if (sp) spc.wstride = W;
        narrow_done[0] = u.np < 1, narrow_done[1] = u.np < 2;
        for (int k = 0; k <= u.np; k++) part_off[k] = u.pb[k] < u.nn ? u.off[u.pb[k]] : u.pack_bytes;
    }

    fe last_of(int c) const { return fe_from_bytes(src.cols[c] + (n - 1) * sizeof(fe)); }
    enum { INTERP = 1, LDE = 2 };
    int transform(int c0, int nc, bool fused, bool all = false, int what = INTERP | LDE) {
        SparseCols g = spc;
        g.col0 = c0, g.fused = fused, g.all = all;
        const SparseCols *gs = sp ? &g : nullptr;
        const size_t o = (size_t)c0 * n;
        if (what & INTERP) ntt(p->st, pl->Tn, p->d_trace + o, n, p->polys + o, n, nc, true, nullptr, &inv_n, p->tmp, gs);
        if (what & LDE)
            ntt_lde(p->st, pl->Tn, pl->ct, p->polys + o, n, nc, 0, 1, (int)B, p->lde + o * B, B * n, n, p->tmp, gs);
        return ZK_OK;
    }
    void hash_ready(bool last) {
        int b = hashed;
        while (b < W / 4 && ready[4 * b] && ready[4 * b + 1] && ready[4 * b + 2] && ready[4 * b + 3]) b++;
        if (b - hashed >= 2 || (last && b > hashed)) {
            hash_rows_blocks(p->st, p->lde, W, pl->log_n, pl->log_b, hashed, b, p->leaves,
                             VirtCols{p->tc.virt, p->sp_last, pl->lagr_lde});
            hashed = b;
        }
    }
    int process(const int *cols, int nc) {
        if (sp && !fresh)
            ZK_TRY(for_runs(cols, nc, [this](int c0, int k) {
                sparse_detect(p->st, p->d_trace, n, c0, k, spc);
                return ZK_OK;
            }));
        ZK_TRY(for_runs(cols, nc, [this](int c0, int k) { return transform(c0, k, fresh); }));
        for (int i = 0; i < nc; i++) ready[cols[i]] = true;
        hash_ready(false);
        return ZK_OK;
    }

    int start_checks() {
        ZK_TRY(ensure_pack(p, u.pack_bytes));
        for (int i = 0, k = 0; i < u.nn; i++) {
            if (i == u.pb[k + 1]) k++;
            row_tasks(packed[k], i, 0, n - 1, u.lat ? (size_t)1 << 16 : R, [this](int j, size_t r0, size_t r1) {
                uint8_t *dst = p->h_pack + u.off[j];
                if (!pack_rows(src.cols[u.nar[j]], r0, r1, u.width[j], dst)) pack_bad.fetch_or(1u << u.nar[j]);
                if (r1 == n - 1) memset(dst + (size_t)u.width[j] * (n - 1), 0, u.width[j]);
            });
        }
        for (int i = 0; i < u.nh; i++)
            row_tasks(checked, u.hin[i], 0, n - 1, R, [this](int c, size_t r0, size_t r1) {
                if (!zero_rows(src.cols[c], r0, r1)) sparse_bad.fetch_or(1u << c);
            });
        return ZK_OK;
    }

    int fill_sparse() {
        if (!u.nh) return ZK_OK;
        fe lastv[W] = {};
        for (int i = 0; i < u.nh; i++) lastv[u.hin[i]] = last_of(u.hin[i]);
        ZK_TRY(h2d_small(p, p->sp_last, lastv, sizeof lastv));
        ZK_TRY(for_runs(u.hin, u.nh, [this](int c0, int nc) { return transform(c0, nc, false, true, INTERP); }));
        ZK_TRY(for_runs(u.hnv, u.nhv, [this](int c0, int nc) { return transform(c0, nc, false, true, LDE); }));
        p->tc.virt = u.virt;
        memcpy(p->tc.virt_last, lastv, sizeof lastv);
        p->tc.virt_lagr = pl->lagr_lde;
        for (int i = 0; i < u.nh; i++) ready[u.hin[i]] = true;
        return ZK_OK;
    }

    int derive_clock() {
        if (!u.clk) return ZK_OK;
        ZK_TRY(clock_tables(p, pl));
        row_tasks(clocked, 0, 0, n - 1, R, [this](int, size_t r0, size_t r1) {
            if (!clock_rows(src.cols[0], r0, r1)) clock_bad.store(1u);
        });
        clk_d = make_fe_ws(fe_sub(last_of(0), fe_make(n - 1)));
        axpy_fill(p->st, pl->id_poly, pl->lagr, clk_d, n, p->polys);
        if (!u.fuse_nb) axpy_fill(p->st, pl->id_lde, pl->lagr_lde, clk_d, B * n, p->lde);
        ready[0] = true;
        return ZK_OK;
    }

    int form_fixed() {
        if (!u.fixm) return ZK_OK;
        if (!p->fix_ws) ZK_CHECK_HIP(p->arena.alloc(&p->fix_ws, W));
        fe_ws ws[W] = {};
        FixedColList L;
        for (int c = 0; c < W; c++) {
            if (!((u.fixm >> c) & 1u)) continue;
            ws[c] = make_fe_ws(last_of(c));
            L.col[L.count] = (uint8_t)c;
            L.slot[L.count] = FS->slot[c];
            L.count++;
        }
        if (u.fuse_nb) ws[0] = clk_d;
        ZK_TRY(h2d_small(p, p->fix_ws, ws, sizeof ws));
        fixed_cols_axpy(p->st, L, false, FS->fpolys, FS->flde, pl->lagr, pl->lagr_lde, p->fix_ws, n, B, p->polys, p->lde,
                        4 * u.fuse_nb);
        for (int k = 0; k < L.count; k++) ready[L.col[k]] = true;
        if (u.fuse_nb) {
            FixedHashCols A{};
            for (int c = 0; c < 4 * u.fuse_nb; c++) {
                A.wsi[c] = (uint8_t)c;
                A.mode[c] = FixedHashCols::LOAD;
                if ((u.clk && c == 0) || ((u.fixm >> c) & 1u)) {
                    A.mode[c] = FixedHashCols::FORM;
                    A.src[c] = c == 0 ? pl->id_lde : FS->flde + (size_t)FS->slot[c] * B * n;
                }
            }
            fixed_hash(p->st, A, pl->lagr_lde, p->fix_ws, p->lde, W, pl->log_n, pl->log_b, u.fuse_nb, p->leaves);
            hashed = u.fuse_nb;
        }
        hash_ready(false);
        for (int k = 0; k < L.count; k++)
            row_tasks(compared, L.col[k], 0, n - 1, R, [this](int c, size_t r0, size_t r1) {
                if (!same_rows(src.cols[c], FS->host[c].get(), r0, r1, FS->width[c])) fixed_bad.fetch_or(1u << c);
            });
        return ZK_OK;
    }

    bool narrow_item(int k, Item *it) {
        packed[k].wait();
        if (k < 2) narrow_done[k] = true;
        const uint32_t bad = pack_bad.load();
        NarrowCols &g = G[k];
        int *gd = good + u.pb[k], ng = 0;
        for (int i = u.pb[k]; i < u.pb[k + 1]; i++) {
            const int c = u.nar[i];
            if ((bad >> c) & 1u) {
                fallback[nfb++] = c;
                continue;
// ... 138 lines not shown
        p->tc.fix_pending = si;
        return ZK_OK;
    }

    void collect_verdicts() {
        for (Latch *l : {&checked, &clocked, &compared}) l->wait();
        p->tc.sp_bad = sparse_bad.load();
        p->tc.clk_bad = clock_bad.load() != 0;
        p->tc.fix_bad = fixed_bad.load() != 0;
    }

    int run(uint8_t root[32]) {
        classify();
        if (u.status != ZK_OK) ZK_FAIL(u.status, "too many upload groups");
        ZK_TRY(start_checks());
        ZK_TRY(fill_sparse());
        ZK_TRY(derive_clock());
        ZK_TRY(form_fixed());
        if (u.lat) ZK_TRY(run_latency());
        ZK_TRY(run_throughput());
        ZK_TRY(finish());
        ZK_TRY(take_snapshot());
        collect_verdicts();
        return d2h_small(p, root, p->nodes + 32, 32);
    }
};

}

int zk::trace_lde_commit(zk_prover *p, Plan *pl, const TraceSrc &src, size_t n, uint8_t root[32]) {
    zk_prover::TraceOutcome &tc = p->tc;
    tc.up_bytes = 0;
    tc.up_sparse = tc.up_nw8 = tc.up_nw32 = tc.virt = 0;
    SparseCols spc{};
    const SparseCols *sp = nullptr;
    if (!src.fixed) ZK_TRY(sparse_begin(p, pl, &spc, &sp));
    tc.sp_used = sp != nullptr;
    if (src.dev) return src.fixed ? commit_device_fixed(p, pl, src, n, root) : commit_device(p, pl, src, n, sp, root);
    return HostTraceCommit(p, pl, src, n, spc, sp != nullptr).run(root);
}

bool zk::trace_hints_refuted(zk_prover *p, const TraceSrc &src, size_t n, int rc) {
    zk_prover::TraceOutcome &tc = p->tc;
    const bool voided = tc.sp_bad || tc.clk_bad || tc.fix_bad;
    if (tc.fix_pending >= 0) {
        const int si = tc.fix_pending;
        tc.fix_pending = -1;
        if (rc == ZK_OK && !voided && src.cols && tc.sp_used) p->hint_sets[p->fix_snaps[si].owner].snap = si;
        else fixed_drop(p, si);
    }
    if (!src.cols || !tc.sp_used || !voided) return false;
    if (zk_prover::HintSet *h = hint_find(p, n, src.key)) {
        if (tc.clk_bad) h->clk_off = true;
        if (tc.fix_bad) h->fixed_off = true;
        fixed_drop(p, h->snap);
        h->have = false;
        h->sparse = h->nw8 = h->nw32 = 0;
    }
    p->hint_redos++;
    tc = {};
    return true;
}

void zk::trace_hints_learn(zk_prover *p, const TraceSrc &src, size_t n, int rc) {
    const zk_prover::TraceOutcome &tc = p->tc;
    const bool completed = rc == ZK_OK || rc == ZK_ERR_DEGREE || rc == ZK_ERR_BUFFER_TOO_SMALL;
// ... 21 lines not shown
```

### encrypt-zkvm_amd/csrc/upload_plan.hpp

```cpp
#pragma once
#include <stddef.h>
#include <stdint.h>

#include "../../include/zkvm_gpu.h"

namespace zk {

static constexpr int ZK_UPLOAD_GROUPS_MAX = 14;
constexpr int ZK_VIRT_MIN_COL = 22;
constexpr uint32_t ZK_FIXED_CAND = 0xFFEu;

struct UploadPlanIn {
    bool have = false, clk_off = false, fixed_off = false;
    uint32_t sparse = 0, nw8 = 0, nw32 = 0;
    bool snap = false;
    uint32_t snap_mask = 0;
    bool hint_ok = true, no_virtual = false;
    bool lat_sched = false, detect = true;
    bool sparse_on = true, narrow_on = true, clock_on = true, fixed_on = true, fixed_fuse_on = true, virtual_on = true;
    size_t n = 0;
};

struct UploadPlan {
    static constexpr int W = ZK_TRACE_WIDTH;
    int status = ZK_OK;
    uint32_t hint = 0, nw8 = 0, nw32 = 0, fixm = 0, virt = 0;
    bool clk = false;
    bool fix_ok = false;
    bool snap_now = false;
    bool lat = false;
    int dense[W] = {}, nd = 0, hin[W] = {}, nh = 0, hnv[W] = {}, nhv = 0, nar[W] = {}, nn = 0;
    int width[W] = {};
    size_t off[W] = {}, pack_bytes = 0;
    int pb[W + 1] = {}, np = 0;
    int gsz[W] = {}, ngroups = 0;
    int fuse_nb = 0;
};

inline UploadPlan upload_plan(const UploadPlanIn &in) {
    constexpr int W = UploadPlan::W;
    UploadPlan P;
    const bool fresh = in.detect && in.sparse_on && in.hint_ok && in.have;
    P.hint = fresh ? in.sparse : 0u;
    P.nw8 = fresh && in.narrow_on ? in.nw8 & ~P.hint : 0u;
    P.nw32 = fresh && in.narrow_on ? in.nw32 & ~P.hint & ~P.nw8 : 0u;
    P.clk = fresh && in.clock_on && (P.nw32 & 1u) && !in.clk_off;
    if (P.clk) P.nw32 &= ~1u;
    P.fix_ok = fresh && in.fixed_on && !in.fixed_off;
    const bool snap = P.fix_ok && in.snap;
    P.fixm = snap ? in.snap_mask & ~P.hint : 0u;
    P.snap_now = P.fix_ok && !snap;
    P.virt = !in.no_virtual && in.virtual_on ? P.hint & ~((1u << ZK_VIRT_MIN_COL) - 1u) : 0u;
    for (int c = 0; c < W; c++) {
        if ((P.clk && c == 0) || ((P.fixm >> c) & 1u)) continue;
        if ((P.hint >> c) & 1u) {
            P.hin[P.nh++] = c;
            if (!((P.virt >> c) & 1u)) P.hnv[P.nhv++] = c;
        } else if (((P.nw8 | P.nw32) >> c) & 1u) {
            P.nar[P.nn++] = c;
        } else {
            P.dense[P.nd++] = c;
        }
    }
    for (int i = 0; i < P.nn; i++) {
        P.width[i] = ((P.nw8 >> P.nar[i]) & 1u) ? 1 : 4;
        P.off[i] = P.pack_bytes;
        P.pack_bytes += ((size_t)P.width[i] * in.n + 15) & ~(size_t)15;
    }
    P.lat = in.lat_sched && P.nn > 0;
    if (P.lat) {
        for (int i = 0; i < P.nn;) {
            i += P.np == 0 ? 1 : 2;
            if (i > P.nn) i = P.nn;
            P.pb[++P.np] = i;
        }
    } else if (P.nn) {
        P.pb[1] = (P.nn + 1) / 2;
        P.pb[2] = P.nn;
        P.np = P.pb[1] < P.nn ? 2 : 1;
    }
    for (int left = P.nd; left > 0; left -= P.gsz[P.ngroups - 1]) {
        const int k = left > 4 ? 4 : left > 2 ? 2 : left;
        P.gsz[P.ngroups++] = left == 4 ? 2 : k;
    }
    if (P.ngroups + (P.lat ? 1 : P.np + 1) > ZK_UPLOAD_GROUPS_MAX) P.status = ZK_ERR_INVALID_ARG;
    if (P.fixm && in.fixed_fuse_on) {
        const uint32_t pre = (P.clk ? 1u : 0u) | P.fixm | (P.hint & ~P.virt);
        while (P.fuse_nb < W / 4 && ((pre >> (4 * P.fuse_nb)) & 0xFu) == 0xFu) P.fuse_nb++;
    }
    return P;
}

}
```

### encrypt-zkvm_amd/csrc/vm_gpu.hip

```cpp
#include <hip/hip_runtime.h>
#include <string.h>

#include <random>
#include <string>
#include <vector>

#include "comm.hpp"
#include "prover_internal.hpp"
#include "vm_internal.hpp"

using namespace zk;
using zk::vm::Op;
using zk::vm::VmState;

namespace {

constexpr int VM_S = 64;
constexpr int VM_K = 8;
constexpr int NREG = zk::vm::MAX_STACK;

struct DevState {
    fe t[NREG];
    uint32_t d, ta, tb;
};
// ... 329 lines not shown
            (void)hipFree(g->lagr);
            (void)hipFree(g->lagr_lde);
        }
    } unwind{&g};
    ZK_CHECK_HIP(hipMalloc(&g.fpolys, 12 * n * sizeof(fe)));
    ZK_CHECK_HIP(hipMalloc(&g.flde, 12 * nb * n * sizeof(fe)));
    ZK_CHECK_HIP(hipMalloc(&g.lagr, n * sizeof(fe)));
    ZK_CHECK_HIP(hipMalloc(&g.lagr_lde, nb * n * sizeof(fe)));
    fe zero[28], outs[NREG];
    memset(zero, 0, sizeof zero);
    uint32_t md = 0;
    size_t nn = 0;
    const DevProg dp{d->code, d->sponge};
    ZK_TRY(vm_generate(p, prog, in, zero, GenMode{true, NREG}, &nn, outs, &md, &dp));
    const fe inv_n = h_inv(fe_make(n));
    ntt(p->st, pl->Tn, p->d_trace, n, g.fpolys, n, 12, true, nullptr, &inv_n, p->tmp);
    ntt_lde(p->st, pl->Tn, pl->ct, g.fpolys, n, 12, r0, 1, (int)nb, g.flde, nb * n, n, p->tmp);
    ZK_CHECK_HIP(hipMemsetAsync(p->polys, 0, n * sizeof(fe), p->st));
    const fe one = fe_one();
    ZK_TRY(h2d_small(p, p->polys + (n - 1), &one, sizeof one));
    ntt(p->st, pl->Tn, p->polys, n, g.lagr, n, 1, true, nullptr, &inv_n, p->tmp);
    ntt_lde(p->st, pl->Tn, pl->ct, g.lagr, n, 1, r0, 1, (int)nb, g.lagr_lde, nb * n, n, p->tmp);
    ZK_TRY(io_rewind(p));
    g.md = (int)md;
    d->fixed.push_back(g);
    unwind.g = nullptr;
    *out = g;
    return ZK_OK;
}

}

void zk::fixed_axpy(hipStream_t st, const FixedCols &fx, const fe_ws *ws_dev, size_t n, size_t B, fe *polys, fe *lde,
                    int lde_c0) {
    AxpyCols A, E;
    A.ncol = E.ncol = 0;
    size_t ef = 0;
    for (int c = 0; c < W; c++) {
        if (c >= 12 && c < 12 + fx.md) continue;
        A.col[A.ncol] = (uint8_t)c;
        A.src[A.ncol] = (int8_t)(c < 12 ? c : -1);
        A.wsi[A.ncol] = (uint8_t)c;
        A.ncol++;
        if (c < lde_c0) continue;
        E.col[E.ncol] = (uint8_t)c;
        E.src[E.ncol] = (int8_t)(c < 12 ? c : -1);
        E.wsi[E.ncol] = (uint8_t)c;
        E.ncol++;
        ef += c < 12;
    }
    const size_t nf = 12, nz = (size_t)A.ncol - nf;
    ZK_PROF(st, "fixed_axpy", (double)n * 16 * (1 + 2 * nf + nz),
            hipLaunchKernelGGL(k_fixed_axpy, dim3((unsigned)((n + 255) / 256)), dim3(256), 0, st, fx.fpolys, fx.lagr, n, A,
                               ws_dev, polys));
    if (!E.ncol) return;
    ZK_PROF(st, "fixed_axpy", (double)B * n * 16 * (1 + ef + E.ncol),
            hipLaunchKernelGGL(k_fixed_axpy, dim3((unsigned)((B * n + 255) / 256)), dim3(256), 0, st, fx.flde,
                               fx.lagr_lde, B * n, E, ws_dev, lde));
}

void zk::fixed_cols_axpy(hipStream_t st, const FixedColList &L, bool snapshot, const fe *src_polys, const fe *src_lde,
                         const fe *lagr, const fe *lagr_lde, const fe_ws *ws_dev, size_t n, size_t B, fe *polys, fe *lde,
                         int lde_c0) {
    if (L.count <= 0) return;
    AxpyCols A, E;
    A.ncol = L.count;
    E.ncol = 0;
    for (int k = 0; k < L.count; k++) {
        A.col[k] = (uint8_t)(snapshot ? L.slot[k] : L.col[k]);
        A.src[k] = (int8_t)(snapshot ? L.col[k] : L.slot[k]);
        A.wsi[k] = (uint8_t)L.col[k];
        if (L.col[k] < lde_c0) continue;
        E.col[E.ncol] = A.col[k];
        E.src[E.ncol] = A.src[k];
        E.wsi[E.ncol] = A.wsi[k];
        E.ncol++;
    }
    const char *name = snapshot ? "fixed_snapshot" : "fixed_axpy";
    ZK_PROF(st, name, (double)n * 16.0 * (1 + 2 * A.ncol),
            hipLaunchKernelGGL(k_fixed_axpy, dim3((unsigned)((n + 255) / 256)), dim3(256), 0, st, src_polys, lagr, n, A,
                               ws_dev, polys));
    if (!E.ncol) return;
    ZK_PROF(st, name, (double)B * n * 16.0 * (1 + 2 * E.ncol),
            hipLaunchKernelGGL(k_fixed_axpy, dim3((unsigned)((B * n + 255) / 256)), dim3(256), 0, st, src_lde, lagr_lde,
                               B * n, E, ws_dev, lde));
}

zk_program::~zk_program() {
    for (auto &d : dev) {
        (void)hipSetDevice(d->device);
        (void)hipFree(d->code);
        (void)hipFree(d->sponge);
        for (auto &f : d->fixed) {
            (void)hipFree(f.fpolys);
            (void)hipFree(f.flde);
            (void)hipFree(f.lagr);
            (void)hipFree(f.lagr_lde);
        }
    }
}

static void read_last(const uint8_t *last_row, fe last[28]) {
    if (last_row)
        for (int c = 0; c < 28; c++) last[c] = fe_from_bytes(last_row + 16 * c);
    else
        random_last_row(last);
}

int zk_vm_trace_device(zk_prover *p, zk_program *prog, const uint8_t *public_in, size_t num_public,
                       const uint8_t *secret, size_t num_secret, uint32_t lwe_size, uint32_t delta,
                       const uint8_t *last_row, size_t *n_out, uint8_t *outputs) {
    if (!p || !prog || !n_out || (num_secret && !secret) || (num_public && !public_in))
        ZK_FAIL(ZK_ERR_INVALID_ARG, "null argument");
    fe outs[NREG], last[28];
// ... 119 lines not shown
```

### encrypt-zkvm_amd/csrc/zk_internal.hpp

```cpp
#pragma once
#include <hip/hip_runtime.h>
#include <stddef.h>
#include <stdint.h>

#include <string>
#include <vector>

#include "chal.hpp"
#include "f128.hpp"

namespace zk {

struct KernelProfiler {
    bool on = false;
    struct Rec {
        const char *name;
        hipEvent_t a, b;
        double bytes;
        double muls, addsubs;
    };
    std::vector<Rec> recs;
    std::vector<hipEvent_t> pool;
    size_t used = 0;
    hipEvent_t get() {
// ... 84 lines not shown

struct CosetTables {
    fe *full = nullptr, *stage = nullptr, *pass = nullptr;
    fe_ws *stage_ws = nullptr;
    fe_w2 *stage_w2 = nullptr;
};
void ntt_lde(hipStream_t st, const NttTables &T, const CosetTables &CT, const fe *in, size_t in_stride, int ncols,
             int r0, int rstride, int ncos, fe *out, size_t out_cstride, size_t out_jstride, fe *tmp,
             const SparseCols *sp = nullptr);
void axpy_fill(hipStream_t st, const fe *F, const fe *L, const fe_ws &d, size_t cnt, fe *out);

void grind_launch(hipStream_t st, const uint32_t *seed_dev, uint64_t start, uint32_t count, int bits,
                  unsigned long long *best_dev);

void hash_rows_cosets(hipStream_t st, const fe *base, int ncols, int log_n, int log_b, int r0, int log_rc,
                      uint8_t *leaves);
void commit_rows_coset_major(hipStream_t st, const fe *base, int ncols, int log_n, int log_b, uint8_t *leaves,
                             uint8_t *nodes);
struct VirtCols {
    uint32_t mask = 0;
    const fe *last = nullptr, *lagr_lde = nullptr;
};
void hash_rows_blocks(hipStream_t st, const fe *base, int ncols, int log_n, int log_b, int b0, int b1, uint8_t *leaves,
                      VirtCols virt = VirtCols());
struct FixedHashCols {
    enum : uint8_t { FORM = 0, FORM_NOSRC = 1, LOAD = 2 };
    static constexpr int MAXC = 28;
    const fe *src[MAXC];
    uint8_t wsi[MAXC];
    uint8_t mode[MAXC];
};
void fixed_hash(hipStream_t st, const FixedHashCols &A, const fe *lagr_lde, const fe_ws *ws_dev, fe *lde, int ncols,
                int log_n, int log_b, int nb, uint8_t *leaves);
struct FriLayout {
    int lb, lcn;
};
FriLayout fri_layout(size_t L, int lb);
void merkle_tree(hipStream_t st, const uint8_t *leaves, size_t nl, uint8_t *nodes);
constexpr size_t ZK_GATHER_CAP = 1 << 17;
void gather_chunks(hipStream_t st, const uint64_t *addr, size_t k, fe *out);
constexpr int ZK_COPY_LIST_MAX = 32;
struct CopyList {
    int n;
    const uint32_t *src[ZK_COPY_LIST_MAX];
    uint32_t *dst[ZK_COPY_LIST_MAX];
    uint32_t words[ZK_COPY_LIST_MAX];
};
hipError_t copy_to_host(hipStream_t st, const CopyList &L, size_t max_words);
void gather_digests(hipStream_t st, const uint8_t *src, const uint64_t *idx, size_t k, uint8_t *out);
void gather_rows(hipStream_t st, const fe *base, int ncols, int log_n, int log_b, const uint64_t *pos, size_t k,
                 fe *out);

struct AirConsts {
    fe coeff_t[20];
    fe coeff_b[22];
    int assert_col[22];
    int assert_grp[22];
    fe assert_val[22];
    fe inv_zn[8];
    fe xr[8];
    fe g_last2, g_last1;
    fe delta;
    fe bnd1;
    int lwe_size;
};
void batch_inv_pairs(hipStream_t st, const NttTables &Tn, const fe *xr, int log_b, int log_n, fe a, fe b,
                     fe *out);
struct Fe8 {
    fe v[8];
};
void divisor_tables(hipStream_t st, const NttTables &Tn, const fe *xr, int log_cos, int log_n, fe g1, fe g2,
                    const Fe8 &inv_zn, fe *out);
struct EvalMap {
    int nce, ce0, cestep, lshift, lde_cosets;
    size_t dplane = 0;
};
hipError_t upload_rescue_consts(hipStream_t st);
hipError_t eval_constraints_mapped(hipStream_t st, const fe *lde, int log_n, EvalMap map, const fe *periodic,
                             const fe *divs, const AirConsts *consts_dev, fe *comp, bool bnd = true);
struct ValReport {
    unsigned long long t_count[20];
    unsigned long long t_first[20];
    unsigned long long failing_steps;
    unsigned a_mask, pad_;
    fe a_found[22];
};
static_assert(sizeof(ValReport) < 1024, "the validation report stays a small transfer");
hipError_t validate_trace(hipStream_t st, const fe *trace, size_t n, const fe *per_tab, fe delta, int lwe_size,
                          ValReport *rep);
struct CrossMap {
    const fe *c[8];
    size_t k0, kcount, pstride;
    int derive7 = 0;
    fe k7[7] = {};
};
void comp_cross_mapped(hipStream_t st, const CrossMap &m, const NttTables &T8n, const PowTable &inv3, fe scale,
                       fe w8inv, fe inv3n, int ncols, fe *polys, unsigned *nonzero_flag);
hipError_t eval_constraints(hipStream_t st, const fe *lde, int log_n, int log_b, const fe *periodic, const fe *divs,
                      const AirConsts *consts_dev, fe *comp, bool bnd = true, int nce = 8);
void boundary_poly_add(hipStream_t st, const fe *tpolys, int log_n, const AirConsts &K, fe c, fe *scratch, fe *col0,
                       unsigned *flag);
const fe *boundary_range_begin(hipStream_t st, const fe *tpolys, int log_n, const AirConsts &K, fe c, fe *scratch,
                               size_t k0, size_t kn);
void boundary_range_end(hipStream_t st, int log_n, fe c, fe *scratch, size_t k0, size_t kn, const fe *ext, fe *col0,
                        unsigned *flag);
void comp_cross_coset(hipStream_t st, const fe *c, int log_n, const NttTables &T8n, const PowTable &inv3,
                      fe scale, fe w8inv, fe inv3n, int ncols, fe *polys, unsigned *nonzero_flag);

int ood_waves(size_t n);
template <class T>
void ood_eval(hipStream_t st, const fe *tpolys, int W, const fe *cpolys, int C, int log_n, T z, T zg, fe *tab,
              fe *partials, fe *out, int rank = 0, int G = 1);
void sum_partials(hipStream_t st, const fe *partials, int npolys, int nblk, fe *out, int b0 = 0, int b1 = -1);
template <int KX>
struct DeepConsts {
    typename Chal<KX>::T alpha_t[32];
    typename Chal<KX>::T alpha_c[16];
    typename Chal<KX>::T k1, k2, z, zg;
};
static_assert(sizeof(DeepConsts<1>) == 52 * sizeof(fe) && sizeof(DeepConsts<2>) == 52 * sizeof(fe2), "DeepConsts layout");
void lde_cosets(hipStream_t st, const NttTables &Tn, const CosetTables &CT, const fe *coeffs, size_t n, size_t r0,
                size_t stride, int count, fe *out, fe *ntt_tmp);
constexpr size_t ZK_DEEP_BLOCK = 256;
struct DeepScratch {
    size_t H;
    fe *pw, *g1, *g2, *out, *bs, *total;
    DeepScratch(fe *s, size_t n, int KX)
        : H(n / 2048 + 2),
          pw(s),
          g1(pw + 4 * KX * (2048 + H)),
          g2(g1 + KX * n),
          out(g2 + KX * n),
          bs(out + KX * n),
          total(bs + 2 * KX * ((n + ZK_DEEP_BLOCK - 1) / ZK_DEEP_BLOCK)) {}
    static size_t size(size_t n, int KX) { return KX * (4 * (2048 + n / 2048 + 2) + 3 * n + 2 * (n / ZK_DEEP_BLOCK + 1)); }
};
template <class T>
const fe *deep_poly(hipStream_t st, const fe *tpolys, const fe *cpolys, int ccols, int log_n,
                    const void *deep_consts_dev, T z, T zg, fe *scratch);
constexpr size_t ZK_DEEP_RANGE_QUANTUM = 2048;
template <class T>
const fe *deep_range_begin(hipStream_t st, const fe *tpolys, const fe *cpolys, int ccols, int log_n,
                           const void *deep_consts_dev, T z, T zg, fe *scratch, size_t k0, size_t kn);
template <class T>
const fe *deep_range_end(hipStream_t st, int log_n, T z, T zg, fe *scratch, size_t k0, size_t kn, const fe *ext);
template <class T>
void deep_coeff_launch(hipStream_t st, const NttTables &Tn, const fe *tpolys, const fe *cpolys, int ccols, int log_n,
                       int log_b, const void *deep_consts_dev, T z, T zg, const CosetTables &CT, fe *scratch,
                       fe *ulde, fe *ntt_tmp, fe *out);
template <int KX>
struct FoldConsts {
    fe zinv[16];
    typename Chal<KX>::T alpha;
    fe inv_offset, inv_fold;
};
static_assert(sizeof(FoldConsts<1>) == 19 * sizeof(fe) && offsetof(FoldConsts<1>, alpha) == 16 * sizeof(fe) &&
                  offsetof(FoldConsts<2>, alpha) == 16 * sizeof(fe),
              "FoldConsts layout");
void commit_fri_layer(hipStream_t st, int KX, const fe *layer, size_t L, int fold, uint8_t *leaves, uint8_t *nodes,
                      int lb = 0);
void fri_fold_launch(hipStream_t st, int KX, const fe *layer, size_t L, int fold, const void *fold_consts_dev,
                     const NttTables &TN, size_t wstride, fe *next, int lb = 0);
void coset_major_to_natural(hipStream_t st, const fe *src, int log_n, int log_b, fe *dst);
void fri_coin_launch(hipStream_t st, uint32_t *seed_dev, const uint8_t *root_dev, int k, fe *alpha_dev,
                     fe *alpha_log);

hipError_t eval_constraints_ext(hipStream_t st, const fe *lde, int log_n, int log_b, const fe *periodic, const fe *divs,
                          const AirConsts *consts2_dev, fe *comp, bool bnd = true, int nce = 8);
hipError_t eval_constraints_ext_mapped(hipStream_t st, const fe *lde, int log_n, EvalMap map, const fe *periodic,
                                 const fe *divs, const AirConsts *consts2_dev, size_t plane, fe *comp, bool bnd = true);
void gather_fe(hipStream_t st, const fe *src, const uint64_t *idx, size_t k, fe *out);

}

namespace zk {
void diag_field_op(hipStream_t st, int op, const fe *a, const fe *b, fe *out, size_t count, const fe_ws *ws = nullptr,
                   const fe_w2 *w2 = nullptr);
void diag_blake3_elems(hipStream_t st, const fe *in, int k, size_t count, uint8_t *out);
}
```

### encrypt-zkvm_amd/zkvm_amd/native.py

```python
from __future__ import annotations

import ctypes as C
import os
from pathlib import Path

PKG_ROOT = Path(__file__).resolve().parent.parent
LIB_PATH = Path(os.environ.get("ZKVM_GPU_LIB", PKG_ROOT / "lib" / "libzkvm_gpu.so"))

ZK_OK = 0
ZK_ERR_INVALID_ARG = -1
ZK_ERR_BUFFER_TOO_SMALL = -2
ZK_ERR_DEVICE = -3
ZK_ERR_OUT_OF_MEMORY = -4
ZK_ERR_PROGRAM = -10
ZK_ERR_STACK = -11
ZK_ERR_CHIPLETS = -12
ZK_ERR_DEGREE = -20
ZK_ERR_TRACE = -21
ZK_ERR_VERIFY = -30

MAX_COLS, MAX_TCONS, MAX_ASSERTS, MAX_CCOLS, MAX_FRI, MAX_REM, MAX_Q = 32, 32, 32, 16, 16, 256, 255

EXPORTED = (
    "zk_last_error", "zk_device_count", "zk_runtime_versions", "zk_device_pci_bus_id", "zk_device_synchronize",
    "zk_prover_create", "zk_prover_create_shard", "zk_prover_destroy",
    "zk_prover_acquire", "zk_prover_release", "zk_prover_pool_trim", "zk_prover_trace_buffer",
    "zk_prove", "zk_prove_columns", "zk_prove_columns_ex", "zk_host_alloc", "zk_host_free", "zk_host_register",
    "zk_host_unregister", "zk_prove_device", "zk_lde_new", "zk_lde_read_frame", "zk_lde_query", "zk_lde_free",
    "zk_eval_constraints", "zk_commit_composition", "zk_comp_query", "zk_comp_free", "zk_prover_stage_times", "zk_prover_profile", "zk_prover_kernel_stats", "zk_prover_kernel_ops", "zk_prover_exchange_stats", "zk_prover_exchange_stats_ex", "zk_prover_shard_schedule", "zk_prover_upload_stats", "zk_prover_upload_derived", "zk_prover_upload_fixed", "zk_prover_set_upload_schedule", "zk_prover_proof_info", "zk_vm_trace",
    "zk_verify", "zk_comm_create_loopback", "zk_comm_unique_id", "zk_comm_create_rccl", "zk_comm_create_host", "zk_comm_destroy", "zk_comm_set_measure", "zk_comm_set_trace_split", "zk_prove_sharded",
    "zk_program_compile", "zk_program_trace", "zk_program_free", "zk_vm_last_error", "zk_vm_trace_device",
    "zk_vm_prove",
    "zk_vm_prove_sharded",
    "zk_validate_device", "zk_validate_columns", "zk_prover_set_validate", "zk_prover_validation",
)


EXCHANGE_FN = C.CFUNCTYPE(C.c_int, C.c_void_p, C.c_int, C.c_void_p, C.c_void_p, C.c_size_t)
XCHG_ALL_TO_ALL, XCHG_ALL_GATHER = 0, 1


class ZkError(RuntimeError):
    def __init__(self, code: int, message: str):
        super().__init__(f"[{code}] {message}")
        self.code = code


class Options(C.Structure):
    _fields_ = [(f, C.c_uint32) for f in
                ("num_queries", "blowup", "grinding", "field_extension", "fri_folding", "fri_rem_max_deg")]


class PubInputs(C.Structure):
    _fields_ = [("program_hash", C.c_uint8 * 32), ("stack_outputs", C.c_uint8 * 256),
                ("lwe_size", C.c_uint32), ("delta", C.c_uint32)]


class ProofInfo(C.Structure):
    _fields_ = [("schedule", C.c_int32), ("hint_redos", C.c_uint32), ("hint_sets", C.c_uint32),
                ("hinted_sparse", C.c_uint32), ("derived", C.c_uint32), ("fixed_sets", C.c_uint32)]


# ... 120 lines not shown
        L.zk_prove_columns_ex.argtypes = [vp, C.POINTER(vp), sz, C.POINTER(Options), C.POINTER(PubInputs), vp,
                                          C.POINTER(sz), C.POINTER(Record), C.POINTER(Dump)]
        L.zk_host_alloc.argtypes = [sz, C.POINTER(vp)]
        L.zk_host_free.argtypes = [vp]
        L.zk_host_free.restype = None
        L.zk_host_register.argtypes = [vp, sz]
        L.zk_host_unregister.argtypes = [vp]
        L.zk_prove_device.argtypes = [vp, vp, sz, C.POINTER(Options), C.POINTER(PubInputs), vp, C.POINTER(sz),
                                      C.POINTER(Record), C.POINTER(Dump)]
        L.zk_validate_device.argtypes = [vp, vp, sz, C.POINTER(PubInputs), C.POINTER(Validation)]
        L.zk_validate_columns.argtypes = [vp, C.POINTER(vp), sz, C.POINTER(PubInputs), C.POINTER(Validation)]
        L.zk_prover_set_validate.argtypes = [vp, i32]
        L.zk_prover_validation.argtypes = [vp, C.POINTER(Validation)]
        L.zk_lde_new.argtypes = [vp, vp, sz, sz, u32, C.POINTER(vp), vp]
        L.zk_lde_read_frame.argtypes = [vp, sz, vp, vp]
        L.zk_lde_query.argtypes = [vp, vp, sz, vp, vp, C.POINTER(sz)]
        L.zk_lde_free.argtypes = [vp]
        L.zk_lde_free.restype = None
        L.zk_eval_constraints.argtypes = [vp, C.POINTER(PubInputs), vp, vp, vp]
        L.zk_commit_composition.argtypes = [vp, vp, u32, C.POINTER(vp), vp, vp]
        L.zk_comp_query.argtypes = [vp, vp, sz, vp, vp, C.POINTER(sz)]
        L.zk_comp_free.argtypes = [vp]
        L.zk_comp_free.restype = None
        L.zk_prover_stage_times.argtypes = [vp, C.POINTER(C.c_char_p), C.POINTER(C.c_float), i32, C.POINTER(i32)]
        L.zk_prover_profile.argtypes = [vp, i32]
        L.zk_prover_set_upload_schedule.argtypes = [vp, i32]
        L.zk_prover_proof_info.argtypes = [vp, C.POINTER(ProofInfo)]
        L.zk_prover_kernel_stats.argtypes = [vp, C.POINTER(C.c_char_p), C.POINTER(C.c_float), C.POINTER(i32),
                                             C.POINTER(C.c_double), i32, C.POINTER(i32)]
        L.zk_prover_kernel_ops.argtypes = [vp, C.POINTER(C.c_double), C.POINTER(C.c_double), i32, C.POINTER(i32)]
        L.zk_prover_upload_stats.argtypes = [vp, C.POINTER(C.c_uint64), C.POINTER(u32), C.POINTER(u32), C.POINTER(u32)]
        L.zk_prover_upload_derived.argtypes = [vp, C.POINTER(u32)]
        L.zk_prover_upload_fixed.argtypes = [vp, C.POINTER(u32)]
        L.zk_prover_exchange_stats.argtypes = [vp, C.POINTER(C.c_char_p), C.POINTER(C.c_float), C.POINTER(C.c_double),
                                               C.POINTER(i32), i32, C.POINTER(i32)]
        L.zk_verify.argtypes = [vp, sz, C.POINTER(PubInputs), u32, C.c_char_p, sz]
        L.zk_comm_create_loopback.argtypes = [i32, C.POINTER(vp)]
        L.zk_comm_unique_id.argtypes = [vp]
        L.zk_comm_create_rccl.argtypes = [vp, i32, i32, i32, C.POINTER(vp)]
        L.zk_comm_create_host.argtypes = [i32, i32, EXCHANGE_FN, vp, C.POINTER(vp)]
        L.zk_comm_destroy.argtypes = [vp]
        L.zk_comm_destroy.restype = None
        L.zk_comm_set_measure.argtypes = [vp, i32]
        L.zk_comm_set_trace_split.argtypes = [vp, i32]
        L.zk_prover_exchange_stats_ex.argtypes = [vp, C.POINTER(C.c_char_p), C.POINTER(C.c_float), C.POINTER(C.c_float),
                                                  C.POINTER(C.c_double), C.POINTER(i32), i32, C.POINTER(i32)]
        L.zk_prover_shard_schedule.argtypes = [vp, C.c_char_p, sz, C.POINTER(sz)]
        L.zk_prove_sharded.argtypes = [vp, C.POINTER(vp), i32, vp, sz, C.POINTER(Options), C.POINTER(PubInputs), vp,
                                       C.POINTER(sz), C.POINTER(Record)]
        L.zk_vm_trace.argtypes = [C.c_char_p, vp, sz, vp, sz, u32, u32, vp, vp, sz, C.POINTER(sz), vp, vp]
        L.zk_vm_last_error.restype = C.c_char_p
        L.zk_program_compile.argtypes = [C.c_char_p, C.POINTER(vp), vp, C.POINTER(sz)]
        L.zk_program_trace.argtypes = [vp, vp, sz, vp, sz, u32, u32, vp, vp, sz, C.POINTER(sz), vp]
        L.zk_vm_trace_device.argtypes = [vp, vp, vp, sz, vp, sz, u32, u32, vp, C.POINTER(sz), vp]
        L.zk_vm_prove.argtypes = [vp, vp, vp, sz, vp, sz, u32, u32, vp, C.POINTER(Options), vp, C.POINTER(sz), vp, vp]
        L.zk_vm_prove_sharded.argtypes = [vp, vp, C.c_int, vp, vp, sz, vp, sz, u32, u32, vp, C.POINTER(Options), vp,
                                          C.POINTER(sz), vp, vp]
        L.zk_diag_vm_states.argtypes = [vp, vp, sz, vp, sz, u32, u32, sz, sz, vp, vp]
        L.zk_program_free.argtypes = [vp]
        L.zk_program_free.restype = None
        L.zk_diag_mul_limbs_host.argtypes = [vp, vp, vp, sz]
        L.zk_diag_mul_limbs_host.restype = None
        L.zk_diag_dot_host.argtypes = [vp, vp, sz, vp]
        L.zk_diag_dot_host.restype = None
        L.zk_diag_blake3_host.argtypes = [vp, sz, vp]
        L.zk_diag_blake3_host.restype = None
# ... 50 lines not shown
```

### encrypt-zkvm_amd/zkvm_amd/prover.py

```python
from __future__ import annotations

import ctypes as C
from dataclasses import dataclass

import numpy as np

from . import native
from .native import Dump, Options, PubInputs, Record, ZkError, check, lib

P = 2**128 - 45 * 2**40 + 1
FIELD_EXTENSION_NONE = 1
FIELD_EXTENSION_QUADRATIC = 2


@dataclass(frozen=True)
class ProofOptions:
    num_queries: int = 32
    blowup_factor: int = 8
    grinding_factor: int = 0
    field_extension: int = FIELD_EXTENSION_NONE
    fri_folding_factor: int = 8
    fri_remainder_max_degree: int = 127

    def to_c(self) -> Options:
# ... 127 lines not shown
        n = trace.shape[1]
        if n > self.max_trace_len:
            raise ZkError(native.ZK_ERR_INVALID_ARG, "trace longer than max_trace_len")
        d = self.trace_buffer()
        hip = _hip()
        rc = hip.hipMemcpy(ctypes.c_void_p(d), trace.ctypes.data_as(ctypes.c_void_p), trace.nbytes, 1)
        if rc != 0:
            raise ZkError(native.ZK_ERR_DEVICE, f"hipMemcpy failed ({rc})")
        return d, n

    def prove(self, trace: np.ndarray, pub: PubInputs, options: ProofOptions = REFERENCE_OPTIONS, **kw):
        if trace.shape[1] > self.max_trace_len:
            raise ZkError(native.ZK_ERR_INVALID_ARG, "trace longer than max_trace_len")
        return self.prove_host(trace, pub, options, **kw)

    def stage_times(self) -> dict:
        names = (C.c_char_p * 32)()
        ms = (C.c_float * 32)()
        cnt = C.c_int(0)
        check(lib().zk_prover_stage_times(self.handle, names, ms, 32, C.byref(cnt)))
        return {names[i].decode(): ms[i] for i in range(min(cnt.value, 32))}

    def upload_stats(self) -> dict:
        b = C.c_uint64(0)
        sp, n8, n32 = C.c_uint32(0), C.c_uint32(0), C.c_uint32(0)
        check(lib().zk_prover_upload_stats(self.handle, C.byref(b), C.byref(sp), C.byref(n8), C.byref(n32)))
        dv = C.c_uint32(0)
        check(lib().zk_prover_upload_derived(self.handle, C.byref(dv)))
        fx = C.c_uint32(0)
        check(lib().zk_prover_upload_fixed(self.handle, C.byref(fx)))
        cols = lambda m: [c for c in range(28) if (m >> c) & 1]
        return {"bytes": b.value, "sparse": cols(sp.value), "narrow8": cols(n8.value), "narrow32": cols(n32.value),
                "derived": cols(dv.value), "fixed": cols(fx.value)}

    UPLOAD_SCHEDULES = {"auto": 0, "throughput": 1, "latency": 2}

    def proof_info(self) -> dict:
        from .native import ProofInfo
        info = ProofInfo()
        check(lib().zk_prover_proof_info(self.handle, C.byref(info)))
        cols = lambda m: [c for c in range(28) if (m >> c) & 1]
        return {"schedule": {1: "throughput", 2: "latency"}.get(info.schedule), "hint_redos": info.hint_redos,
                "hint_sets": info.hint_sets, "hinted_sparse": cols(info.hinted_sparse), "derived": cols(info.derived),
                "fixed_sets": info.fixed_sets}

    def set_upload_schedule(self, schedule: str):
        check(lib().zk_prover_set_upload_schedule(self.handle, self.UPLOAD_SCHEDULES[schedule]))

    def profile(self, on: bool):
        check(lib().zk_prover_profile(self.handle, 1 if on else 0))
        check(lib().zk_prover_kernel_stats(self.handle, None, None, None, None, 0, None))

    def kernel_stats(self) -> dict:
        names = (C.c_char_p * 64)()
        ms = (C.c_float * 64)()
        nl = (C.c_int * 64)()
        by = (C.c_double * 64)()
        cnt = C.c_int(0)
        check(lib().zk_prover_kernel_stats(self.handle, names, ms, nl, by, 64, C.byref(cnt)))
        return {names[i].decode(): (ms[i], nl[i], by[i]) for i in range(min(cnt.value, 64))}

    def kernel_ops(self) -> dict:
        names = (C.c_char_p * 64)()
        ms = (C.c_float * 64)()
        nl = (C.c_int * 64)()
        by = (C.c_double * 64)()
# ... 203 lines not shown
```

### include/zkvm_gpu.h

```cpp
#ifndef ZKVM_GPU_H
#define ZKVM_GPU_H

#include <stddef.h>
#include <stdint.h>

#ifdef __cplusplus
extern "C" {
#endif

#define ZK_OK 0
#define ZK_ERR_INVALID_ARG -1
#define ZK_ERR_BUFFER_TOO_SMALL -2
#define ZK_ERR_DEVICE -3
#define ZK_ERR_OUT_OF_MEMORY -4
#define ZK_ERR_PROGRAM -10
#define ZK_ERR_STACK -11
#define ZK_ERR_CHIPLETS -12
#define ZK_ERR_DEGREE -20
#define ZK_ERR_VERIFY -30

#define ZK_TRACE_WIDTH 28
#define ZK_MAX_COLS 32
#define ZK_MAX_TCONS 32
#define ZK_MAX_ASSERTS 32
// ... 113 lines not shown

int zk_eval_constraints(zk_trace_lde *lde, const zk_pub_inputs *pub, const uint8_t *coeff_t, const uint8_t *coeff_b,
                        uint8_t *out);

typedef struct zk_comp_commit zk_comp_commit;
int zk_commit_composition(zk_trace_lde *lde, const uint8_t *composition, uint32_t num_cols, zk_comp_commit **out,
                          uint8_t root[32], uint8_t *polys_out);
int zk_comp_query(zk_comp_commit *comp, const uint64_t *positions, size_t k, uint8_t *rows_out, uint8_t *proof_out,
                  size_t *proof_len);
void zk_comp_free(zk_comp_commit *comp);

typedef struct zk_comm zk_comm;
int zk_comm_create_loopback(int world, zk_comm **out);
int zk_comm_unique_id(uint8_t id[128]);
int zk_comm_create_rccl(const uint8_t id[128], int rank, int world, int device, zk_comm **out);
typedef int (*zk_exchange_fn)(void *ctx, int op, const void *send, void *recv, size_t bytes);
enum { ZK_XCHG_ALL_TO_ALL = 0, ZK_XCHG_ALL_GATHER = 1 };
int zk_comm_create_host(int rank, int world, zk_exchange_fn fn, void *ctx, zk_comm **out);
void zk_comm_destroy(zk_comm *comm);
int zk_comm_set_measure(zk_comm *comm, int on);
int zk_comm_set_trace_split(zk_comm *comm, int replicated);
int zk_prove_sharded(zk_comm *comm, zk_prover **provers, int nlocal, const uint8_t *trace, size_t n,
                     const zk_options *opt, const zk_pub_inputs *pub, uint8_t *proof_out, size_t *proof_len,
                     zk_record *rec);
int zk_prover_exchange_stats(zk_prover *p, const char **names, float *ms, double *bytes, int *calls, int cap,
                             int *count);
int zk_prover_exchange_stats_ex(zk_prover *p, const char **names, float *ms, float *exposed_ms, double *bytes,
                                int *calls, int cap, int *count);
int zk_prover_shard_schedule(zk_prover *p, char *buf, size_t cap, size_t *len);
int zk_prover_upload_stats(zk_prover *p, uint64_t *bytes, uint32_t *sparse_cols, uint32_t *narrow8_cols,
                           uint32_t *narrow32_cols);
int zk_prover_upload_derived(zk_prover *p, uint32_t *derived_cols);
int zk_prover_upload_fixed(zk_prover *p, uint32_t *fixed_cols);
enum { ZK_SCHED_AUTO = 0, ZK_SCHED_THROUGHPUT = 1, ZK_SCHED_LATENCY = 2 };
int zk_prover_set_upload_schedule(zk_prover *p, int schedule);
typedef struct {
    int32_t schedule;
    uint32_t hint_redos;
    uint32_t hint_sets;
    uint32_t hinted_sparse;
    uint32_t derived;
    uint32_t fixed_sets;
} zk_proof_info;
int zk_prover_proof_info(const zk_prover *p, zk_proof_info *out);

int zk_verify(const uint8_t *proof, size_t proof_len, const zk_pub_inputs *pub, uint32_t min_security, char *msg,
              size_t msg_cap);

int zk_prover_stage_times(zk_prover *p, const char **names, float *ms, int cap, int *count);
int zk_prover_profile(zk_prover *p, int enable);
int zk_prover_kernel_stats(zk_prover *p, const char **names, float *total_ms, int *launches, double *total_bytes,
                           int cap, int *count);
int zk_prover_kernel_ops(zk_prover *p, double *total_muls, double *total_addsubs, int cap, int *count);

int zk_vm_trace(const char *source, const uint8_t *public_in, size_t num_public, const uint8_t *secret,
                size_t num_secret, uint32_t lwe_size, uint32_t delta, const uint8_t *last_row, uint8_t *trace_out,
                size_t cap_rows, size_t *n_out, uint8_t *outputs, uint8_t *program_hash);
typedef struct zk_program zk_program;
int zk_program_compile(const char *source, zk_program **out, uint8_t *program_hash, size_t *trace_len);
int zk_program_trace(const zk_program *prog, const uint8_t *public_in, size_t num_public, const uint8_t *secret,
                     size_t num_secret, uint32_t lwe_size, uint32_t delta, const uint8_t *last_row,
                     uint8_t *trace_out, size_t cap_rows, size_t *n_out, uint8_t *outputs);
void zk_program_free(zk_program *prog);
const char *zk_vm_last_error(void);

int zk_vm_trace_device(zk_prover *p, zk_program *prog, const uint8_t *public_in, size_t num_public,
// ... 15 lines not shown
```

Baseline: 116.2 million.

## Use per-column coefficient sources to skip zero and derived trace polys

Introduces a CoeffSrc descriptor so OOD evaluation, DEEP combine and boundary-poly kernels read trace coefficient planes per column. Zero columns are skipped, and derived columns are folded through one shared Lagrange poly with host-side weights. This cuts HBM reads in these bandwidth-bound kernels when trace columns are zero or derived. The cost is extra host bookkeeping, pointer-array kernel arguments and a post-hoc fold of OOD values, which must stay in sync with the verifier's expectations.

After: 118.4 million, median of 6. 1.02x the previous value.

```diff
diff --git a/encrypt-zkvm_amd/csrc/kernels.hip b/encrypt-zkvm_amd/csrc/kernels.hip
--- a/encrypt-zkvm_amd/csrc/kernels.hip
+++ b/encrypt-zkvm_amd/csrc/kernels.hip
@@ -1952,20 +1952,25 @@
     tab[t] = Chal<KX>::exp(x, e);
 }
 
+struct OodPolys {
+    static constexpr int MAXP = CoeffSrc::MAXC + 16 + 1;
+    int count, count2;
+    uint32_t zero;
+    const fe *poly[MAXP];
+    uint8_t rz[MAXP], rg[MAXP];
+};
 template <int KX, int E>
-__global__ void __launch_bounds__(256) k_ood_eval(const fe *tpolys, int W, const fe *cpolys, int C, size_t n,
-                                                  const typename Chal<KX>::T *tab, int nw, int w0, int w1,
-                                                  fe *partials) {
+__global__ void __launch_bounds__(256) k_ood_eval(OodPolys L, int W, int np, size_t n, const typename Chal<KX>::T *tab,
+                                                  int nw, int w0, int w1, fe *partials) {
     typedef Chal<KX> X;
     typedef typename X::T T;
     const int gw = w0 + (int)((blockIdx.x * blockDim.x + threadIdx.x) >> 6);
     const int lane = threadIdx.x & 63;
-    const size_t plane = (size_t)(2 * W + C) * nw;
-    const int tgroups = (W + OOD_GROUP - 1) / OOD_GROUP;
-    const int g = blockIdx.y;
-    const bool comp = g >= tgroups;
-    const int p0 = comp ? 0 : g * OOD_GROUP;
-    const int p1 = comp ? C : min(W, p0 + OOD_GROUP);
+    const size_t plane = (size_t)np * nw;
+    const int tg = (L.count2 + OOD_GROUP - 1) / OOD_GROUP, g = blockIdx.y;
+    const bool two = g < tg;
+    const int p0 = two ? g * OOD_GROUP : L.count2 + (g - tg) * OOD_GROUP;
+    const int p1 = min(two ? L.count2 : L.count, p0 + OOD_GROUP);
     const size_t base = (size_t)gw * 64 * E + lane;
     __shared__ T Y[2][E];
     if (threadIdx.x < 2 * E) {
@@ -1975,21 +1980,24 @@
     }
     __syncthreads();
     if (gw >= w1) return;
+    if (blockIdx.y == 0 && L.zero && lane == 0)
+        for (int c = 0; c < W; c++)
+            if ((L.zero >> c) & 1u) {
+                X::st(partials + (size_t)c * nw + gw, plane, X::zero());
+                X::st(partials + (size_t)(W + c) * nw + gw, plane, X::zero());
+            }
     const T wz = X::mul(tab[lane], tab[128 + gw]);
-    const T wzg = comp ? X::zero() : X::mul(tab[64 + lane], tab[128 + nw + gw]);
+    const T wzg = two ? X::mul(tab[64 + lane], tab[128 + nw + gw]) : X::zero();
     for (int p = p0; p < p1; p++) {
-        const fe *c = (comp ? cpolys : tpolys) + (size_t)p * n;
+        const fe *c = L.poly[p] + base;
         fe v[E];
 #pragma unroll
-        for (int e = 0; e < E; e++) {
-            const size_t k = base + 64 * (size_t)e;
-            v[e] = k < n ? c[k] : fe_zero();
-        }
+        for (int e = 0; e < E; e++) v[e] = base + 64 * (size_t)e < n ? c[64 * e] : fe_zero();
         const T hz = wave_sum(X::mul(dot_base<E>(v, Y[0]), wz));
-        if (lane == 0) X::st(partials + (size_t)(comp ? 2 * W + p : p) * nw + gw, plane, hz);
-        if (!comp) {
+        if (lane == 0) X::st(partials + (size_t)L.rz[p] * nw + gw, plane, hz);
+        if (two) {
             const T hg = wave_sum(X::mul(dot_base<E>(v, Y[1]), wzg));
-            if (lane == 0) X::st(partials + (size_t)(W + p) * nw + gw, plane, hg);
+            if (lane == 0) X::st(partials + (size_t)L.rg[p] * nw + gw, plane, hg);
         }
     }
 }
@@ -1997,7 +2005,7 @@
 int ood_waves(size_t n) { return (int)std::max<size_t>(1, n / 1024); }
 
 template <class T>
-void ood_eval(hipStream_t st, const fe *tpolys, int W, const fe *cpolys, int C, int log_n, T z, T zg, fe *tab,
+void ood_eval(hipStream_t st, const CoeffSrc &S, int W, const fe *cpolys, int C, int log_n, T z, T zg, fe *tab,
               fe *partials, fe *out, int rank, int G) {
     constexpr int KX = ChalOf<T>::KX;
     const size_t n = (size_t)1 << log_n;
@@ -2006,10 +2014,24 @@
     const int w0 = (int)((int64_t)nw * rank / G), w1 = (int)((int64_t)nw * (rank + 1) / G);
     T *t = reinterpret_cast<T *>(tab);
     hipLaunchKernelGGL(k_ood_tables<KX>, dim3(cdiv(128 + 2 * nw, 256)), dim3(256), 0, st, z, zg, (uint64_t)64 * E, nw, t);
-    const dim3 grid(std::max(1u, cdiv(w1 - w0, 4)), (W + OOD_GROUP - 1) / OOD_GROUP + 1);
+    const int np = ood_out_values(S, W, C);
+    OodPolys L{};
+    auto add = [&L](const fe *poly, int rz, int rg) {
+        L.poly[L.count] = poly, L.rz[L.count] = (uint8_t)rz, L.rg[L.count] = (uint8_t)rg;
+        L.count++;
+    };
+    for (int c = 0; c < W; c++) {
+        if (S.mode[c] == CoeffSrc::ZERO) L.zero |= 1u << c;
+        else add(S.plane[c], c, W + c);
+    }
+    if (S.lagr) add(S.lagr, np - 2, np - 1);
+    L.count2 = L.count;
+    for (int j = 0; j < C; j++) add(cpolys + (size_t)j * n, 2 * W + j, 0);
+    const dim3 grid(std::max(1u, cdiv(w1 - w0, 4)),
+                    (L.count2 + OOD_GROUP - 1) / OOD_GROUP + (L.count - L.count2 + OOD_GROUP - 1) / OOD_GROUP);
     const char *name = KX == 1 ? "ood_eval" : "ood_eval_ext";
-#define ZK_OOD(EE) ZK_PROF(st, name, bytes, hipLaunchKernelGGL((k_ood_eval<KX, EE>), grid, dim3(256), 0, st, tpolys, W, cpolys, C, n, t, nw, w0, w1, partials))
-    const double bytes = 16.0 * (W + C) * (double)n * (w1 - w0) / nw;
+#define ZK_OOD(EE) ZK_PROF(st, name, bytes, hipLaunchKernelGGL((k_ood_eval<KX, EE>), grid, dim3(256), 0, st, L, W, np, n, t, nw, w0, w1, partials))
+    const double bytes = 16.0 * L.count * (double)n * (w1 - w0) / nw;
     switch (E) {
         case 16: ZK_OOD(16); break;
         case 8: ZK_OOD(8); break;
@@ -2018,10 +2040,26 @@
         default: ZK_OOD(1); break;
     }
 #undef ZK_OOD
-    sum_partials(st, partials, KX * (2 * W + C), nw, out, w0, w1);
-}
-template void ood_eval<fe>(hipStream_t, const fe *, int, const fe *, int, int, fe, fe, fe *, fe *, fe *, int, int);
-template void ood_eval<fe2>(hipStream_t, const fe *, int, const fe *, int, int, fe2, fe2, fe *, fe *, fe *, int, int);
+    sum_partials(st, partials, KX * ood_out_values(S, W, C), nw, out, w0, w1);
+}
+template void ood_eval<fe>(hipStream_t, const CoeffSrc &, int, const fe *, int, int, fe, fe, fe *, fe *, fe *, int, int);
+template void ood_eval<fe2>(hipStream_t, const CoeffSrc &, int, const fe *, int, int, fe2, fe2, fe *, fe *, fe *, int, int);
+
+void ood_fold_sources(int KX, int W, int C, const CoeffSrc &S, const fe *w, const fe *raw, fe *hv) {
+    const int np = 2 * W + C, nr = ood_out_values(S, W, C);
+    for (int j = 0; j < KX; j++) {
+        const fe *r = raw + (size_t)j * nr;
+        fe *h = hv + (size_t)j * np;
+        for (int i = 0; i < np; i++) h[i] = r[i];
+        if (!S.lagr) continue;
+        const fe ez = r[np], ezg = r[np + 1];
+        for (int c = 0; c < W; c++) {
+            if (!S.derived(c)) continue;
+            h[c] = fe_add(h[c], fe_mul(w[c], ez));
+            h[W + c] = fe_add(h[W + c], fe_mul(w[c], ezg));
+        }
+    }
+}
 
 __global__ void k_sum_partials(const fe *partials, int nblk, int b0, int b1, fe *out) {
     __shared__ fe red[256];
@@ -2071,7 +2109,7 @@
 }
 
 template <int KX>
-__global__ void __launch_bounds__(DIV_T) k_deep_div_g(const fe *tpolys, const fe *cpolys, int ccols, size_t n,
+__global__ void __launch_bounds__(DIV_T) k_deep_div_g(CoeffSrc TS, const fe *cpolys, int ccols, size_t n,
                                                      const DeepConsts<KX> *D, const typename Chal<KX>::T *pw, size_t H,
                                                      typename Chal<KX>::T *g1, typename Chal<KX>::T *g2, fe *bs,
                                                      size_t kbase, size_t kend) {
@@ -2084,7 +2122,9 @@
     if (k < kend) {
         typename X::Acc aA = X::acc_zero();
 #pragma unroll 4
-        for (int c = 0; c < 28; c++) X::madd(aA, D->alpha_t[c], ld_fe(tpolys + (size_t)c * n + k));
+        for (int c = 0; c < 28; c++)
+            if (TS.mode[c] != CoeffSrc::ZERO) X::madd(aA, D->alpha_t[c], ld_fe(TS.plane[c] + k));
+        if (TS.lagr) X::madd(aA, D->alpha_t[ZK_DEEP_LAGR], ld_fe(TS.lagr + k));
         typename X::Acc aH = X::acc_zero();
         if constexpr (KX == 1) {
             for (int j = 0; j < ccols; j++) X::madd(aH, D->alpha_c[j], ld_fe(cpolys + (size_t)j * n + k));
@@ -2242,13 +2282,15 @@
     hipLaunchKernelGGL(k_deep_pow_tables<KX>, dim3(cdiv(4 * (2048 + S.H), 256)), dim3(256), 0, st, pb, S.H, (T *)S.pw);
 }
 template <class T>
-static void deep_phase1(hipStream_t st, const fe *tpolys, const fe *cpolys, int ccols, size_t n,
+static void deep_phase1(hipStream_t st, const CoeffSrc &TS, const fe *cpolys, int ccols, size_t n,
                         const void *deep_consts_dev, fe *scratch, size_t k0, size_t kn, fe *total) {
     constexpr int KX = ChalOf<T>::KX;
     const DeepScratch S(scratch, n, KX);
     const size_t nb1 = (kn + DIV_T - 1) / DIV_T;
-    ZK_PROF(st, "deep_combine", (16.0 * (28 + KX * ccols) + 32.0 * KX) * kn,
-            hipLaunchKernelGGL(k_deep_div_g<KX>, dim3((unsigned)nb1), dim3(DIV_T), 0, st, tpolys, cpolys, ccols, n,
+    int tplanes = TS.lagr ? 1 : 0;
+    for (int c = 0; c < 28; c++) tplanes += TS.mode[c] != CoeffSrc::ZERO;
+    ZK_PROF(st, "deep_combine", (16.0 * (tplanes + KX * ccols) + 32.0 * KX) * kn,
+            hipLaunchKernelGGL(k_deep_div_g<KX>, dim3((unsigned)nb1), dim3(DIV_T), 0, st, TS, cpolys, ccols, n,
                                (const DeepConsts<KX> *)deep_consts_dev, (const T *)S.pw, S.H, (T *)S.g1, (T *)S.g2, S.bs, k0,
                                k0 + kn));
     hipLaunchKernelGGL(k_deep_div_scan<2 * KX>, dim3(1), dim3(1024), 0, st, S.bs, (int)nb1, total);
@@ -2264,21 +2306,21 @@
                                ext));
 }
 template <class T>
-const fe *deep_poly(hipStream_t st, const fe *tpolys, const fe *cpolys, int ccols, int log_n,
+const fe *deep_poly(hipStream_t st, const CoeffSrc &TS, const fe *cpolys, int ccols, int log_n,
                     const void *deep_consts_dev, T z, T zg, fe *scratch) {
     const size_t n = (size_t)1 << log_n;
     deep_tables(st, n, z, zg, scratch);
-    deep_phase1<T>(st, tpolys, cpolys, ccols, n, deep_consts_dev, scratch, 0, n, nullptr);
+    deep_phase1<T>(st, TS, cpolys, ccols, n, deep_consts_dev, scratch, 0, n, nullptr);
     deep_phase3(st, n, z, zg, scratch, 0, n, nullptr);
     return DeepScratch(scratch, n, ChalOf<T>::KX).out;
 }
 template <class T>
-const fe *deep_range_begin(hipStream_t st, const fe *tpolys, const fe *cpolys, int ccols, int log_n,
+const fe *deep_range_begin(hipStream_t st, const CoeffSrc &TS, const fe *cpolys, int ccols, int log_n,
                            const void *deep_consts_dev, T z, T zg, fe *scratch, size_t k0, size_t kn) {
     const size_t n = (size_t)1 << log_n;
     deep_tables(st, n, z, zg, scratch);
     fe *total = DeepScratch(scratch, n, ChalOf<T>::KX).total;
-    deep_phase1<T>(st, tpolys, cpolys, ccols, n, deep_consts_dev, scratch, k0, kn, total);
+    deep_phase1<T>(st, TS, cpolys, ccols, n, deep_consts_dev, scratch, k0, kn, total);
     return total;
 }
 template <class T>
@@ -2289,30 +2331,24 @@
 }
 
 struct BndPoly {
-    fe cb[22];
+    static constexpr int MAXT = 13;
+    int nt;
     fe bnd1;
+    const fe *plane[MAXT];
+    fe c0[MAXT], c1[MAXT];
 };
-__global__ void __launch_bounds__(DIV_T) k_bnd_div_g(const fe *tpolys, size_t n, BndPoly bp, const fe *pw, size_t H,
-                                                    fe *g1, fe *g2, fe *bs, size_t kbase, size_t kend) {
+__global__ void __launch_bounds__(DIV_T) k_bnd_div_g(BndPoly bp, const fe *pw, size_t H, fe *g1, fe *g2, fe *bs,
+                                                    size_t kbase, size_t kend) {
     __shared__ fe red[DIV_T / 64];
     const size_t per = 2048 + H;
     const size_t k = kbase + blockIdx.x * (size_t)DIV_T + threadIdx.x;
     fe v1 = fe_zero(), v2 = fe_zero();
     if (k < kend) {
-        auto T = [&](int c) { return ld_fe(tpolys + (size_t)c * n + k); };
         acc288 a0 = acc288_zero(), a1 = acc288_zero();
-        acc288_madd(a0, bp.cb[0], T(0));
-        acc288_madd(a0, bp.cb[3], T(11));
-        const fe t7 = T(7), t8 = T(8);
-        acc288_madd(a0, bp.cb[1], t7);
-        acc288_madd(a0, bp.cb[2], t8);
-        acc288_madd(a1, bp.cb[12], t7);
-        acc288_madd(a1, bp.cb[13], t8);
-#pragma unroll
-        for (int j = 0; j < 8; j++) {
-            const fe c = T(12 + j);
-            acc288_madd(a0, bp.cb[4 + j], c);
-            acc288_madd(a1, bp.cb[14 + j], c);
+        for (int i = 0; i < bp.nt; i++) {
+            const fe t = ld_fe(bp.plane[i] + k);
+            acc288_madd(a0, bp.c0[i], t);
+            acc288_madd(a1, bp.c1[i], t);
         }
         v1 = acc288_reduce(a0);
         fe f1 = acc288_reduce(a1);
@@ -2329,8 +2365,8 @@
     }
 }
 
-static void bnd_tables_phase1(hipStream_t st, const fe *tpolys, size_t n, const AirConsts &K, fe c, fe *scratch,
-                              size_t k0, size_t kn, fe *total) {
+static void bnd_tables_phase1(hipStream_t st, const CoeffSrc &TS, const fe *w, size_t n, const AirConsts &K, fe c,
+                              fe *scratch, size_t k0, size_t kn, fe *total) {
     const DeepScratch S(scratch, n, 1);
     const size_t nb1 = (kn + DIV_T - 1) / DIV_T;
     DeepPowBases<1> pb;
@@ -2339,12 +2375,29 @@
     pb.b[2] = fe_one();
     pb.b[3] = fe_inv(c);
     hipLaunchKernelGGL(k_deep_pow_tables<1>, dim3(cdiv(4 * (2048 + S.H), 256)), dim3(256), 0, st, pb, S.H, S.pw);
-    BndPoly bp;
-    memcpy(bp.cb, K.coeff_b, sizeof bp.cb);
+    BndPoly bp{};
     bp.bnd1 = K.bnd1;
-    ZK_PROF(st, "boundary_poly", (16.0 * 12 + 32.0) * kn,
-            hipLaunchKernelGGL(k_bnd_div_g, dim3((unsigned)nb1), dim3(DIV_T), 0, st, tpolys, n, bp, S.pw, S.H, S.g1, S.g2,
-                               S.bs, k0, k0 + kn));
+    static const int col0[12] = {0, 7, 8, 11, 12, 13, 14, 15, 16, 17, 18, 19};
+    fe le0 = fe_zero(), le1 = fe_zero();
+    for (int i = 0; i < 12; i++) {
+        const int cc = col0[i];
+        const fe b0 = K.coeff_b[i], b1 = i == 0 || i == 3 ? fe_zero() : K.coeff_b[i < 3 ? 11 + i : 10 + i];
+        if (TS.mode[cc] != CoeffSrc::ZERO) {
+            bp.plane[bp.nt] = TS.plane[cc], bp.c0[bp.nt] = b0, bp.c1[bp.nt] = b1;
+            bp.nt++;
+        }
+        if (TS.lagr && TS.derived(cc)) {
+            le0 = fe_add(le0, fe_mul(b0, w[cc]));
+            le1 = fe_add(le1, fe_mul(b1, w[cc]));
+        }
+    }
+    if (TS.lagr) {
+        bp.plane[bp.nt] = TS.lagr, bp.c0[bp.nt] = le0, bp.c1[bp.nt] = le1;
+        bp.nt++;
+    }
+    ZK_PROF(st, "boundary_poly", (16.0 * bp.nt + 32.0) * kn,
+            hipLaunchKernelGGL(k_bnd_div_g, dim3((unsigned)nb1), dim3(DIV_T), 0, st, bp, S.pw, S.H, S.g1, S.g2, S.bs, k0,
+                               k0 + kn));
     hipLaunchKernelGGL(k_deep_div_scan<2>, dim3(1), dim3(1024), 0, st, S.bs, (int)nb1, total);
 }
 static void bnd_phase3(hipStream_t st, size_t n, fe c, fe *scratch, size_t k0, size_t kn, const fe *ext, fe *col0,
@@ -2356,18 +2409,18 @@
                                k0 + kn, fe_one(), c, S.pw, S.H, col0, 0, flag, k0, ext));
 }
 
-void boundary_poly_add(hipStream_t st, const fe *tpolys, int log_n, const AirConsts &K, fe c, fe *scratch, fe *col0,
-                       unsigned *flag) {
+void boundary_poly_add(hipStream_t st, const CoeffSrc &TS, const fe *w, int log_n, const AirConsts &K, fe c, fe *scratch,
+                       fe *col0, unsigned *flag) {
     const size_t n = (size_t)1 << log_n;
-    bnd_tables_phase1(st, tpolys, n, K, c, scratch, 0, n, nullptr);
+    bnd_tables_phase1(st, TS, w, n, K, c, scratch, 0, n, nullptr);
     bnd_phase3(st, n, c, scratch, 0, n, nullptr, col0, flag);
 }
 
-const fe *boundary_range_begin(hipStream_t st, const fe *tpolys, int log_n, const AirConsts &K, fe c, fe *scratch,
-                               size_t k0, size_t kn) {
+const fe *boundary_range_begin(hipStream_t st, const CoeffSrc &TS, const fe *w, int log_n, const AirConsts &K, fe c,
+                               fe *scratch, size_t k0, size_t kn) {
     const size_t n = (size_t)1 << log_n;
     fe *total = DeepScratch(scratch, n, 1).total;
-    bnd_tables_phase1(st, tpolys, n, K, c, scratch, k0, kn, total);
+    bnd_tables_phase1(st, TS, w, n, K, c, scratch, k0, kn, total);
     return total;
 }
 void boundary_range_end(hipStream_t st, int log_n, fe c, fe *scratch, size_t k0, size_t kn, const fe *ext, fe *col0,
@@ -2376,12 +2429,12 @@
 }
 
 template <class T>
-void deep_coeff_launch(hipStream_t st, const NttTables &Tn, const fe *tpolys, const fe *cpolys, int ccols, int log_n,
+void deep_coeff_launch(hipStream_t st, const NttTables &Tn, const CoeffSrc &TS, const fe *cpolys, int ccols, int log_n,
                        int log_b, const void *deep_consts_dev, T z, T zg, const CosetTables &CT, fe *scratch,
                        fe *ulde, fe *ntt_tmp, fe *out) {
     constexpr int KX = ChalOf<T>::KX;
     const size_t n = (size_t)1 << log_n, B = (size_t)1 << log_b, N = n << log_b;
-    const fe *Dk = deep_poly(st, tpolys, cpolys, ccols, log_n, deep_consts_dev, z, zg, scratch);
+    const fe *Dk = deep_poly(st, TS, cpolys, ccols, log_n, deep_consts_dev, z, zg, scratch);
     for (int plane = 0; plane < KX; plane++) lde_cosets(st, Tn, CT, Dk + plane * n, n, 0, 1, (int)B, ulde + plane * N, ntt_tmp);
     if (!out) return;
     unsigned pb2 = cdiv(N, 256);
@@ -2391,11 +2444,11 @@
                 hipLaunchKernelGGL(k_coset_to_natural, dim3(pb2), dim3(256), 0, st, ulde + plane * N, log_n, log_b, out + plane * N));
 }
 #define ZK_DEEP_INSTANCES(T)                                                                                           \
-    template const fe *deep_poly<T>(hipStream_t, const fe *, const fe *, int, int, const void *, T, T, fe *);          \
-    template const fe *deep_range_begin<T>(hipStream_t, const fe *, const fe *, int, int, const void *, T, T, fe *,    \
-                                           size_t, size_t);                                                            \
+    template const fe *deep_poly<T>(hipStream_t, const CoeffSrc &, const fe *, int, int, const void *, T, T, fe *);    \
+    template const fe *deep_range_begin<T>(hipStream_t, const CoeffSrc &, const fe *, int, int, const void *, T, T,    \
+                                           fe *, size_t, size_t);                                                      \
     template const fe *deep_range_end<T>(hipStream_t, int, T, T, fe *, size_t, size_t, const fe *);                    \
-    template void deep_coeff_launch<T>(hipStream_t, const NttTables &, const fe *, const fe *, int, int, int,          \
+    template void deep_coeff_launch<T>(hipStream_t, const NttTables &, const CoeffSrc &, const fe *, int, int, int,    \
                                        const void *, T, T, const CosetTables &, fe *, fe *, fe *, fe *);
 ZK_DEEP_INSTANCES(fe)
 ZK_DEEP_INSTANCES(fe2)
diff --git a/encrypt-zkvm_amd/csrc/prover.hip b/encrypt-zkvm_amd/csrc/prover.hip
--- a/encrypt-zkvm_amd/csrc/prover.hip
+++ b/encrypt-zkvm_amd/csrc/prover.hip
@@ -541,6 +541,12 @@
     return ZK_OK;
 }
 
+int zk_prover_coeff_sources(zk_prover *p, uint32_t *cols) {
+    if (!p || !cols) ZK_FAIL(ZK_ERR_INVALID_ARG, "null argument");
+    *cols = p->tc.coeff_src;
+    return ZK_OK;
+}
+
 int zk_prover_exchange_stats_ex(zk_prover *p, const char **names, float *ms, float *exposed_ms, double *bytes,
                                 int *calls, int cap, int *count) {
     if (!p) ZK_FAIL(ZK_ERR_INVALID_ARG, "null prover");
@@ -1132,7 +1138,8 @@
 }
 
 static int composition_stage(zk_prover *p, Plan *pl, int KX, int C, fe *comp, fe *ctmp, fe *clde, uint8_t root[32],
-                             const AirConsts *bnd = nullptr, int nce = 8) {
+                             const AirConsts *bnd = nullptr, int nce = 8, const CoeffSrc *TS = nullptr,
+                             const fe *w = nullptr) {
     const size_t n = (size_t)1 << pl->log_n, CE = 8 * n;
     const int CK = C * KX;
     if (nce != 8 && (nce != 7 || C > 7)) ZK_FAIL(ZK_ERR_INVALID_ARG, "composition: unsupported CE coset count");
@@ -1155,10 +1162,12 @@
         comp_cross_mapped(p->st, m, pl->Tce, pl->inv3, h_inv(fe_make(CE)), h_inv(w8), h_inv(h_pow(fe_make(3), n)), C,
                           p->cpolys + (size_t)j * n, p->flag);
     }
-    if (bnd)
+    if (bnd) {
+        const CoeffSrc plain = coeff_plain(p->polys, n);
         for (int j = 0; j < KX; j++)
-            boundary_poly_add(p->st, p->polys, pl->log_n, bnd[j], bnd[0].g_last2, p->dscratch, p->cpolys + (size_t)j * n,
-                              p->flag);
+            boundary_poly_add(p->st, TS ? *TS : plain, w, pl->log_n, bnd[j], bnd[0].g_last2, p->dscratch,
+                              p->cpolys + (size_t)j * n, p->flag);
+    }
     return lde_commit(p, pl, p->cpolys, CK, clde, p->cleaves, p->cnodes, root);
 }
 
@@ -1275,18 +1284,21 @@
     const int log_n = pl->log_n;
     const typename X::T z = X::make(coin.draw_ext(KX)), zg = X::mulb(z, h_root_of_unity(log_n));
     fe_to_bytes(X::comp(z, 0), R.z);
-    ood_eval(p->st, p->polys, W, p->cpolys, C * KX, log_n, z, zg, b.ood_tab, b.partials, p->ood);
+    const CoeffSrc &TS = p->csrc;
+    ood_eval(p->st, TS, W, p->cpolys, C * KX, log_n, z, zg, b.ood_tab, b.partials, p->ood);
     HT.stop("z");
-    std::vector<fe> hv((size_t)KX * (2 * W + C * KX));
-    ZK_TRY(d2h_small(p, hv.data(), p->ood, hv.size() * sizeof(fe)));
+    std::vector<fe> raw((size_t)KX * ood_out_values(TS, W, C * KX)), hv((size_t)KX * (2 * W + C * KX));
+    ZK_TRY(d2h_small(p, raw.data(), p->ood, raw.size() * sizeof(fe)));
     ZK_TRY(d2h_flush(p));
     HT.start();
+    ood_fold_sources(KX, W, C * KX, TS, p->csrc_w, raw.data(), hv.data());
     std::vector<fe2> e;
     ood_reseed(coin, KX, hv, C, R, e, h);
     stage_mark(p, "ood");
-    const DeepConsts<KX> D = draw_deep_consts<KX>(coin, e, C, z, zg, R);
+    DeepConsts<KX> D = draw_deep_consts<KX>(coin, e, C, z, zg, R);
+    deep_source_weight(D, TS, p->csrc_w);
     ZK_TRY(h2d_small(p, b.deep_consts, &D, sizeof D));
-    deep_coeff_launch(p->st, pl->Tn, p->polys, p->cpolys, C, log_n, pl->log_b, b.deep_consts, z, zg, pl->ct, b.dscratch,
+    deep_coeff_launch(p->st, pl->Tn, TS, p->cpolys, C, log_n, pl->log_b, b.deep_consts, z, zg, pl->ct, b.dscratch,
                       b.ulde, p->tmp, deep_out);
     HT.stop("deep_consts");
     return check_ood_identity(e, C, Kp, KX, X::wide(z), (size_t)1 << log_n, pub);
@@ -1346,7 +1358,8 @@
     HT.stop("air_consts");
     stage_mark(p, "constraints");
 
-    ZK_TRY(composition_stage(p, pl, KX, C, comp, ctmp, clde, R.constraint_root, bnd_rows ? nullptr : Kp, nce));
+    ZK_TRY(composition_stage(p, pl, KX, C, comp, ctmp, clde, R.constraint_root, bnd_rows ? nullptr : Kp, nce, &p->csrc,
+                             p->csrc_w));
     unsigned degree_flag = 0;
     ZK_TRY(d2h_small(p, &degree_flag, p->flag, 4));
     ZK_TRY(d2h_flush(p));
@@ -1637,7 +1650,7 @@
     constexpr int nb = 12 / 4;
     const size_t Bn = n << pl->log_b;
     if (fixed_fuse_on()) {
-        fixed_axpy(p->st, fx, p->fix_ws, n, (size_t)1 << pl->log_b, p->polys, p->lde, 4 * nb);
+        fixed_axpy(p->st, fx, p->fix_ws, n, (size_t)1 << pl->log_b, p->polys, p->lde, 4 * nb, !coeff_src_on());
         FixedHashCols A{};
         for (int c = 0; c < 4 * nb; c++) {
             A.mode[c] = FixedHashCols::FORM;
@@ -1646,7 +1659,7 @@
         }
         fixed_hash(p->st, A, fx.lagr_lde, p->fix_ws, p->lde, W, pl->log_n, pl->log_b, nb, p->leaves);
     } else {
-        fixed_axpy(p->st, fx, p->fix_ws, n, (size_t)1 << pl->log_b, p->polys, p->lde);
+        fixed_axpy(p->st, fx, p->fix_ws, n, (size_t)1 << pl->log_b, p->polys, p->lde, 0, !coeff_src_on());
         hash_rows_blocks(p->st, p->lde, W, pl->log_n, pl->log_b, 0, nb, p->leaves);
     }
     p->fix_prefix_blocks = nb;
@@ -1895,15 +1908,21 @@
 }
 extern "C" void zk_diag_blake3_host(const uint8_t *in, size_t len, uint8_t out[32]) { b3::hash_bytes(in, len, out); }
 
-extern "C" int zk_diag_upload_plan(const uint32_t *in, size_t n, uint32_t *masks, int32_t *counts, int32_t *cols,
-                                   int32_t *width, uint64_t *off, int32_t *pb, int32_t *gsz) {
+static UploadPlanIn diag_upload_plan_in(const uint32_t *in, size_t n) {
     UploadPlanIn q;
     q.have = in[0], q.sparse = in[1], q.nw8 = in[2], q.nw32 = in[3], q.clk_off = in[4], q.fixed_off = in[5];
     q.snap = in[6], q.snap_mask = in[7], q.hint_ok = in[8], q.no_virtual = in[9], q.lat_sched = in[10], q.detect = in[11];
     q.sparse_on = in[12] & 1u, q.narrow_on = in[12] & 2u, q.clock_on = in[12] & 4u, q.fixed_on = in[12] & 8u;
-    q.fixed_fuse_on = in[12] & 16u, q.virtual_on = in[12] & 32u;
+    q.fixed_fuse_on = in[12] & 16u, q.virtual_on = in[12] & 32u, q.coeff_src_on = in[12] & 64u;
     q.n = n;
-    const UploadPlan u = upload_plan(q);
+    return q;
+}
+extern "C" int zk_diag_upload_plan_coeff_src(const uint32_t *in, size_t n) {
+    return upload_plan(diag_upload_plan_in(in, n)).coeff_src ? 1 : 0;
+}
+extern "C" int zk_diag_upload_plan(const uint32_t *in, size_t n, uint32_t *masks, int32_t *counts, int32_t *cols,
+                                   int32_t *width, uint64_t *off, int32_t *pb, int32_t *gsz) {
+    const UploadPlan u = upload_plan(diag_upload_plan_in(in, n));
     const uint32_t m[8] = {u.hint, u.nw8, u.nw32, u.clk, u.fixm, u.virt, u.snap_now, u.lat};
     const int32_t k[7] = {u.nd, u.nh, u.nhv, u.nn, u.np, u.ngroups, u.fuse_nb};
     memcpy(masks, m, sizeof m);
@@ -2099,7 +2118,8 @@
     const Planes b = planes(p, ext);
     with_kx(ext, [&](auto kx) {
         typedef Chal<decltype(kx)::value> X;
-        ood_eval(p->st, p->polys, W, p->cpolys, ccols, ilog2(n), X::make(zv), X::make(zgv), b.ood_tab, b.partials, p->ood, rank, G);
+        ood_eval(p->st, coeff_plain(p->polys, n), W, p->cpolys, ccols, ilog2(n), X::make(zv), X::make(zgv), b.ood_tab,
+                 b.partials, p->ood, rank, G);
         return 0;
     });
     ZK_CHECK_HIP(hipStreamSynchronize(p->st));
@@ -2136,14 +2156,15 @@
         D.z = z, D.zg = zg;
         ZK_CHECK_HIP(hipMemcpy(b.deep_consts, &D, sizeof D, hipMemcpyHostToDevice));
         const fe *Dk = nullptr;
+        const CoeffSrc TS = coeff_plain(p->polys, n);
         if (parts == 1) {
-            Dk = deep_poly(p->st, p->polys, p->cpolys, C, log_n, b.deep_consts, z, zg, b.dscratch);
+            Dk = deep_poly(p->st, TS, p->cpolys, C, log_n, b.deep_consts, z, zg, b.dscratch);
         } else {
             const DeepScratch S(b.dscratch, n, KX);
             const size_t kn = n / parts, nc = 2 * KX, ncarry = nc * (kn / ZK_DEEP_BLOCK);
             std::vector<fe> tot((size_t)parts * nc);
             for (int g = 0; g < parts; g++) {
-                const fe *t = deep_range_begin(p->st, p->polys, p->cpolys, C, log_n, b.deep_consts, z, zg, b.dscratch, g * kn, kn);
+                const fe *t = deep_range_begin(p->st, TS, p->cpolys, C, log_n, b.deep_consts, z, zg, b.dscratch, g * kn, kn);
                 ZK_CHECK_HIP(hipMemcpyAsync(p->comp + g * ncarry, S.bs, ncarry * sizeof(fe), hipMemcpyDeviceToDevice, p->st));
                 ZK_CHECK_HIP(hipMemcpyAsync(&tot[g * nc], t, nc * sizeof(fe), hipMemcpyDeviceToHost, p->st));
             }
@@ -2173,6 +2194,84 @@
     if (parts < 2 || parts > 8 || (parts & (parts - 1)) || n < (size_t)parts * ZK_DEEP_RANGE_QUANTUM)
         ZK_FAIL(ZK_ERR_INVALID_ARG, "zk_diag_deep_parts: 2, 4 or 8 ranges of at least 2048 coefficients");
     return diag_deep(device, tpolys, cpolys, ccols, n, ext, z, zg, alpha_t, alpha_c, parts, out);
+}
+
+extern "C" int zk_diag_coeff_sources(int device, const uint8_t *tplanes, const uint8_t *modes, const uint8_t *w,
+                                     const uint8_t *cpolys, int ccols, size_t n, int ext, const uint8_t *z,
+                                     const uint8_t *zg, const uint8_t *alpha_t, const uint8_t *alpha_c,
+                                     const uint8_t *coeff_b, const uint8_t *bnd1, const uint8_t *c, uint8_t *ood_out,
+                                     uint8_t *deep_out, uint8_t *col0_out, uint32_t *flag_out) {
+    fe2 zv, zgv;
+    ZK_TRY(diag_back_half_args("zk_diag_coeff_sources", tplanes, cpolys, ccols, n, ext, z, zg, ood_out, &zv, &zgv));
+    if (!modes || !w || !alpha_t || !alpha_c || !coeff_b || !bnd1 || !c || !deep_out || !col0_out || !flag_out)
+        ZK_FAIL(ZK_ERR_INVALID_ARG, "zk_diag_coeff_sources: null argument");
+    if ((fe_is_zero(zv.a) && fe_is_zero(zv.b)) || (fe_is_zero(zgv.a) && fe_is_zero(zgv.b)))
+        ZK_FAIL(ZK_ERR_INVALID_ARG, "zk_diag_coeff_sources: z and zg must be non-zero (their inverses are taken)");
+    const int C = ccols / ext, log_n = ilog2(n);
+    fe2 at[W], ac[8];
+    for (int k = 0; k < W + C; k++)
+        if (!diag_read_fe((k < W ? alpha_t + 16 * ext * k : alpha_c + 16 * ext * (k - W)), ext, k < W ? &at[k] : &ac[k - W]))
+            ZK_FAIL(ZK_ERR_INVALID_ARG, "zk_diag_coeff_sources: non-canonical coefficient");
+    fe wv[W];
+    AirConsts K[2];
+    memset(K, 0, sizeof K);
+    const fe cv = fe_from_bytes(c);
+    bool ok = fe_canonical(cv) && !fe_is_zero(cv);
+    for (int k = 0; k < W; k++) {
+        wv[k] = fe_from_bytes(w + 16 * k);
+        ok = ok && fe_canonical(wv[k]) && modes[k] <= CoeffSrc::ZERO;
+    }
+    for (int j = 0; j < ext; j++) {
+        for (int k = 0; k < NUM_ASSERTS; k++) {
+            K[j].coeff_b[k] = fe_from_bytes(coeff_b + 16 * (NUM_ASSERTS * j + k));
+            ok = ok && fe_canonical(K[j].coeff_b[k]);
+        }
+        K[j].bnd1 = fe_from_bytes(bnd1 + 16 * j);
+        ok = ok && fe_canonical(K[j].bnd1);
+    }
+    if (!ok) ZK_FAIL(ZK_ERR_INVALID_ARG, "zk_diag_coeff_sources: canonical values, modes 0 .. 2, c non-zero");
+    zk_prover *p = nullptr;
+    ZK_TRY(zk_prover_create(device, n, 8, &p));
+    std::unique_ptr<zk_prover, void (*)(zk_prover *)> guard(p, zk_prover_destroy);
+    if (ext == 2) ZK_TRY(ensure_ext(p));
+    ZK_CHECK_HIP(hipMemcpy(p->polys, tplanes, (size_t)(W + 1) * n * 16, hipMemcpyHostToDevice));
+    ZK_CHECK_HIP(hipMemcpy(p->cpolys, cpolys, (size_t)ccols * n * 16, hipMemcpyHostToDevice));
+    CoeffSrc TS = coeff_plain(p->polys, n);
+    for (int k = 0; k < W; k++) {
+        TS.mode[k] = modes[k];
+        if (modes[k] == CoeffSrc::ZERO) TS.plane[k] = nullptr;
+        if (modes[k] != CoeffSrc::PLAIN) TS.lagr = p->polys + (size_t)W * n;
+    }
+    const Planes b = planes(p, ext);
+    return with_kx(ext, [&](auto kx) -> int {
+        constexpr int KX = decltype(kx)::value;
+        typedef Chal<KX> X;
+        const typename X::T zz = X::make(zv), zzg = X::make(zgv);
+        ood_eval(p->st, TS, W, p->cpolys, ccols, log_n, zz, zzg, b.ood_tab, b.partials, p->ood);
+        std::vector<fe> raw((size_t)KX * ood_out_values(TS, W, ccols)), hv((size_t)KX * (2 * W + ccols));
+        ZK_CHECK_HIP(hipStreamSynchronize(p->st));
+        ZK_CHECK_HIP(hipMemcpy(raw.data(), p->ood, raw.size() * sizeof(fe), hipMemcpyDeviceToHost));
+        ood_fold_sources(KX, W, ccols, TS, wv, raw.data(), hv.data());
+        memcpy(ood_out, hv.data(), hv.size() * sizeof(fe));
+        DeepConsts<KX> D;
+        memset(&D, 0, sizeof D);
+        for (int k = 0; k < W; k++) D.alpha_t[k] = X::make(at[k]);
+        for (int k = 0; k < C; k++) D.alpha_c[k] = X::make(ac[k]);
+        D.z = zz, D.zg = zzg;
+        deep_source_weight(D, TS, wv);
+        ZK_CHECK_HIP(hipMemcpy(b.deep_consts, &D, sizeof D, hipMemcpyHostToDevice));
+        const fe *Dk = deep_poly(p->st, TS, p->cpolys, C, log_n, b.deep_consts, zz, zzg, b.dscratch);
+        ZK_CHECK_HIP(hipStreamSynchronize(p->st));
+        ZK_CHECK_HIP(hipMemcpy(deep_out, Dk, (size_t)KX * n * 16, hipMemcpyDeviceToHost));
+        ZK_CHECK_HIP(hipMemsetAsync(p->flag, 0, 4, p->st));
+        ZK_CHECK_HIP(hipMemsetAsync(p->ctmp, 0, (size_t)KX * n * 16, p->st));
+        for (int j = 0; j < KX; j++)
+            boundary_poly_add(p->st, TS, wv, log_n, K[j], cv, p->dscratch, p->ctmp + (size_t)j * n, p->flag);
+        ZK_CHECK_HIP(hipStreamSynchronize(p->st));
+        ZK_CHECK_HIP(hipMemcpy(col0_out, p->ctmp, (size_t)KX * n * 16, hipMemcpyDeviceToHost));
+        ZK_CHECK_HIP(hipMemcpy(flag_out, p->flag, 4, hipMemcpyDeviceToHost));
+        return ZK_OK;
+    });
 }
 
 extern "C" int zk_diag_fri_layer(int device, const uint8_t *layer, size_t L, int ext, int fold, int lb, size_t wstride,
diff --git a/encrypt-zkvm_amd/csrc/prover_internal.hpp b/encrypt-zkvm_amd/csrc/prover_internal.hpp
--- a/encrypt-zkvm_amd/csrc/prover_internal.hpp
+++ b/encrypt-zkvm_amd/csrc/prover_internal.hpp
@@ -206,7 +206,10 @@
         uint32_t virt = 0;
         fe virt_last[28] = {};
         const fe *virt_lagr = nullptr;
+        uint32_t coeff_src = 0;
     } tc;
+    zk::CoeffSrc csrc = {};
+    fe csrc_w[zk::W] = {};
     uint32_t sh_sparse = 0, sh_nw8 = 0, sh_nw32 = 0;
     bool sh_clock = false;
     size_t sh_hint_n = 0, sh_clock_off_n = 0;
@@ -318,14 +321,16 @@
 int prove_fixed(zk_prover *p, size_t n, const zk_options *opt, const zk_pub_inputs *pub, const FixedCols *fx,
                 uint8_t *proof_out, size_t *proof_len);
 void fixed_axpy(hipStream_t st, const FixedCols &fx, const fe_ws *ws_dev, size_t n, size_t B, fe *polys, fe *lde,
-                int lde_c0 = 0);
+                int lde_c0 = 0, bool coeffs = true);
+bool coeff_src_on();
+void fixed_coeff_src(zk_prover *p, const FixedCols &fx, size_t n);
 struct FixedColList {
     int count = 0;
     uint8_t col[W], slot[W];
 };
 void fixed_cols_axpy(hipStream_t st, const FixedColList &L, bool snapshot, const fe *src_polys, const fe *src_lde,
                      const fe *lagr, const fe *lagr_lde, const fe_ws *ws_dev, size_t n, size_t B, fe *polys, fe *lde,
-                     int lde_c0 = 0);
+                     int lde_c0 = 0, bool coeffs = true);
 bool fixed_on();
 bool fixed_fuse_on();
 bool same_rows(const uint8_t *col, const uint8_t *snap, size_t r0, size_t r1, int width);
diff --git a/encrypt-zkvm_amd/csrc/shard.hip b/encrypt-zkvm_amd/csrc/shard.hip
--- a/encrypt-zkvm_amd/csrc/shard.hip
+++ b/encrypt-zkvm_amd/csrc/shard.hip
@@ -874,8 +874,8 @@
 
     int boundary_begin(int pln) {
         return each_rank(X, [this, pln](int l, zk_prover *p, Plan *) -> int {
-            const void *sums = boundary_range_begin(p->st, p->polys, log_n, Kp[pln], K.g_last2, p->dscratch,
-                                                    (size_t)X.rank[l] * kg, kg);
+            const void *sums = boundary_range_begin(p->st, coeff_plain(p->polys, n), nullptr, log_n, Kp[pln], K.g_last2,
+                                                    p->dscratch, (size_t)X.rank[l] * kg, kg);
             xb.set(l, sums, p->sh_buf);
             return ZK_OK;
         });
@@ -1027,7 +1027,8 @@
         fe_to_bytes(XF::comp(z, 0), R.z);
         std::vector<fe> hv;
         ZK_TRY(ood_parts(KX_ * (2 * W + CK), [this, z, zg](zk_prover *p, int rank) {
-            ood_eval(p->st, p->polys, W, p->cpolys, CK, log_n, z, zg, pb(p).ood_tab, pb(p).partials, p->ood, rank, G);
+            ood_eval(p->st, coeff_plain(p->polys, n), W, p->cpolys, CK, log_n, z, zg, pb(p).ood_tab, pb(p).partials, p->ood,
+                     rank, G);
         }, hv));
         std::vector<fe2> e;
         ood_reseed(coin, KX_, hv, C, R, e, h);
@@ -1036,14 +1037,16 @@
         auto upload = [this, D](zk_prover *p) { return h2d_small(p, pb(p).deep_consts, &D, sizeof D); };
         if (range_split) {
             ZK_TRY(deep_split_ranges(KX_, [this, z, zg](zk_prover *p, size_t k0) {
-                return deep_range_begin(p->st, p->polys, p->cpolys, C, log_n, pb(p).deep_consts, z, zg, pb(p).dscratch, k0, kg);
+                return deep_range_begin(p->st, coeff_plain(p->polys, n), p->cpolys, C, log_n, pb(p).deep_consts, z, zg,
+                                        pb(p).dscratch, k0, kg);
             }, [this, z, zg](zk_prover *p, size_t k0, const fe *ext) {
                 return deep_range_end(p->st, log_n, z, zg, pb(p).dscratch, k0, kg, ext);
             }, upload));
         } else {
             ZK_TRY(each_rank(X, [this, z, zg, upload](int l, zk_prover *p, Plan *) -> int {
                 ZK_TRY(upload(p));
-                Dk[l] = deep_poly(p->st, p->polys, p->cpolys, C, log_n, pb(p).deep_consts, z, zg, pb(p).dscratch);
+                Dk[l] = deep_poly(p->st, coeff_plain(p->polys, n), p->cpolys, C, log_n, pb(p).deep_consts, z, zg,
+                                  pb(p).dscratch);
                 return ZK_OK;
             }));
         }
diff --git a/encrypt-zkvm_amd/csrc/trace_commit.hip b/encrypt-zkvm_amd/csrc/trace_commit.hip
--- a/encrypt-zkvm_amd/csrc/trace_commit.hip
+++ b/encrypt-zkvm_amd/csrc/trace_commit.hip
@@ -14,6 +14,7 @@
 bool zk::fixed_on() { static const bool on = env_switch("ZK_FIXED"); return on; }
 bool zk::fixed_fuse_on() { static const bool on = env_switch("ZK_FIXED_FUSE"); return on; }
 static bool virtual_on() { static const bool on = env_switch("ZK_VIRTUAL"); return on; }
+bool zk::coeff_src_on() { static const bool on = env_switch("ZK_COEFF_SRC"); return on; }
 
 static void fixed_drop(zk_prover *p, int i) {
     if (i < 0) return;
@@ -214,8 +215,20 @@
     return ZK_OK;
 }
 
+void zk::fixed_coeff_src(zk_prover *p, const FixedCols &fx, size_t n) {
+    for (int c = 0; c < W; c++) {
+        if (c >= 12 && c < 12 + fx.md) continue;
+        p->csrc.plane[c] = c < 12 ? fx.fpolys + (size_t)c * n : nullptr;
+        p->csrc.mode[c] = c < 12 ? CoeffSrc::BASE : CoeffSrc::ZERO;
+        p->csrc_w[c] = fx.last[c];
+        p->tc.coeff_src |= 1u << c;
+    }
+    p->csrc.lagr = fx.lagr;
+}
+
 static int commit_device_fixed(zk_prover *p, Plan *pl, const TraceSrc &src, size_t n, uint8_t root[32]) {
     const FixedCols &fx = *src.fixed;
+    if (coeff_src_on()) fixed_coeff_src(p, fx, n);
     const fe inv_n = h_inv(fe_make(n));
     const size_t B = (size_t)1 << pl->log_b, c0 = 12;
     if (fx.md > 0) {
@@ -231,7 +244,7 @@
         fe_ws ws[W];
         for (int c = 0; c < W; c++) ws[c] = make_fe_ws(fx.last[c]);
         ZK_TRY(h2d_small(p, p->fix_ws, ws, sizeof ws));
-        fixed_axpy(p->st, fx, p->fix_ws, n, B, p->polys, p->lde);
+        fixed_axpy(p->st, fx, p->fix_ws, n, B, p->polys, p->lde, 0, !coeff_src_on());
         hash_rows_cosets(p->st, p->lde, W, pl->log_n, pl->log_b, 0, pl->log_b, p->leaves);
     }
     merkle_tree(p->st, p->leaves, n * B, p->nodes);
@@ -304,6 +317,7 @@
         in.hint_ok = src.hint_ok, in.no_virtual = src.no_virtual, in.lat_sched = p->lat_sched, in.detect = sp != nullptr;
         in.sparse_on = sparse_on(), in.narrow_on = narrow_on(), in.clock_on = clock_on();
         in.fixed_on = fixed_on(), in.fixed_fuse_on = fixed_fuse_on(), in.virtual_on = virtual_on(), in.n = n;
+        in.coeff_src_on = coeff_src_on();
         u = upload_plan(in);
         if (!u.fix_ok) FS = nullptr;
         else if (!FS && H->snap >= 0) fixed_drop(p, H->snap);
@@ -322,6 +336,13 @@
     }
 
     fe last_of(int c) const { return fe_from_bytes(src.cols[c] + (n - 1) * sizeof(fe)); }
+    void source(int c, uint8_t mode, const fe *plane, fe w) {
+        p->csrc.plane[c] = plane;
+        p->csrc.mode[c] = mode;
+        p->csrc.lagr = pl->lagr;
+        p->csrc_w[c] = w;
+        p->tc.coeff_src |= 1u << c;
+    }
     enum { INTERP = 1, LDE = 2 };
     int transform(int c0, int nc, bool fused, bool all = false, int what = INTERP | LDE) {
         SparseCols g = spc;
@@ -376,7 +397,10 @@
         fe lastv[W] = {};
         for (int i = 0; i < u.nh; i++) lastv[u.hin[i]] = last_of(u.hin[i]);
         ZK_TRY(h2d_small(p, p->sp_last, lastv, sizeof lastv));
-        ZK_TRY(for_runs(u.hin, u.nh, [this](int c0, int nc) { return transform(c0, nc, false, true, INTERP); }));
+        if (u.coeff_src)
+            for (int i = 0; i < u.nh; i++) source(u.hin[i], CoeffSrc::ZERO, nullptr, lastv[u.hin[i]]);
+        else
+            ZK_TRY(for_runs(u.hin, u.nh, [this](int c0, int nc) { return transform(c0, nc, false, true, INTERP); }));
         ZK_TRY(for_runs(u.hnv, u.nhv, [this](int c0, int nc) { return transform(c0, nc, false, true, LDE); }));
         p->tc.virt = u.virt;
         memcpy(p->tc.virt_last, lastv, sizeof lastv);
@@ -391,8 +415,10 @@
         row_tasks(clocked, 0, 0, n - 1, R, [this](int, size_t r0, size_t r1) {
             if (!clock_rows(src.cols[0], r0, r1)) clock_bad.store(1u);
         });
-        clk_d = make_fe_ws(fe_sub(last_of(0), fe_make(n - 1)));
-        axpy_fill(p->st, pl->id_poly, pl->lagr, clk_d, n, p->polys);
+        const fe d = fe_sub(last_of(0), fe_make(n - 1));
+        clk_d = make_fe_ws(d);
+        if (u.coeff_src) source(0, CoeffSrc::BASE, pl->id_poly, d);
+        else axpy_fill(p->st, pl->id_poly, pl->lagr, clk_d, n, p->polys);
         if (!u.fuse_nb) axpy_fill(p->st, pl->id_lde, pl->lagr_lde, clk_d, B * n, p->lde);
         ready[0] = true;
         return ZK_OK;
@@ -405,15 +431,17 @@
         FixedColList L;
         for (int c = 0; c < W; c++) {
             if (!((u.fixm >> c) & 1u)) continue;
-            ws[c] = make_fe_ws(last_of(c));
+            const fe last = last_of(c);
+            ws[c] = make_fe_ws(last);
             L.col[L.count] = (uint8_t)c;
             L.slot[L.count] = FS->slot[c];
             L.count++;
+            if (u.coeff_src) source(c, CoeffSrc::BASE, FS->fpolys + (size_t)FS->slot[c] * n, last);
         }
         if (u.fuse_nb) ws[0] = clk_d;
         ZK_TRY(h2d_small(p, p->fix_ws, ws, sizeof ws));
         fixed_cols_axpy(p->st, L, false, FS->fpolys, FS->flde, pl->lagr, pl->lagr_lde, p->fix_ws, n, B, p->polys, p->lde,
-                        4 * u.fuse_nb);
+                        4 * u.fuse_nb, !u.coeff_src);
         for (int k = 0; k < L.count; k++) ready[L.col[k]] = true;
         if (u.fuse_nb) {
             FixedHashCols A{};
@@ -618,6 +646,9 @@
     zk_prover::TraceOutcome &tc = p->tc;
     tc.up_bytes = 0;
     tc.up_sparse = tc.up_nw8 = tc.up_nw32 = tc.virt = 0;
+    tc.coeff_src = 0;
+    p->csrc = coeff_plain(p->polys, n);
+    memset(p->csrc_w, 0, sizeof p->csrc_w);
     SparseCols spc{};
     const SparseCols *sp = nullptr;
     if (!src.fixed) ZK_TRY(sparse_begin(p, pl, &spc, &sp));
diff --git a/encrypt-zkvm_amd/csrc/upload_plan.hpp b/encrypt-zkvm_amd/csrc/upload_plan.hpp
--- a/encrypt-zkvm_amd/csrc/upload_plan.hpp
+++ b/encrypt-zkvm_amd/csrc/upload_plan.hpp
@@ -18,6 +18,7 @@
     bool hint_ok = true, no_virtual = false;
     bool lat_sched = false, detect = true;
     bool sparse_on = true, narrow_on = true, clock_on = true, fixed_on = true, fixed_fuse_on = true, virtual_on = true;
+    bool coeff_src_on = true;
     size_t n = 0;
 };
 
@@ -35,6 +36,7 @@
     int pb[W + 1] = {}, np = 0;
     int gsz[W] = {}, ngroups = 0;
     int fuse_nb = 0;
+    bool coeff_src = false;
 };
 
 inline UploadPlan upload_plan(const UploadPlanIn &in) {
@@ -88,6 +90,7 @@
         const uint32_t pre = (P.clk ? 1u : 0u) | P.fixm | (P.hint & ~P.virt);
         while (P.fuse_nb < W / 4 && ((pre >> (4 * P.fuse_nb)) & 0xFu) == 0xFu) P.fuse_nb++;
     }
+    P.coeff_src = in.coeff_src_on && !in.no_virtual && P.fixm != 0;
     return P;
 }
 
diff --git a/encrypt-zkvm_amd/csrc/vm_gpu.hip b/encrypt-zkvm_amd/csrc/vm_gpu.hip
--- a/encrypt-zkvm_amd/csrc/vm_gpu.hip
+++ b/encrypt-zkvm_amd/csrc/vm_gpu.hip
@@ -385,7 +385,7 @@
 }
 
 void zk::fixed_axpy(hipStream_t st, const FixedCols &fx, const fe_ws *ws_dev, size_t n, size_t B, fe *polys, fe *lde,
-                    int lde_c0) {
+                    int lde_c0, bool coeffs) {
     AxpyCols A, E;
     A.ncol = E.ncol = 0;
     size_t ef = 0;
@@ -403,9 +403,10 @@
         ef += c < 12;
     }
     const size_t nf = 12, nz = (size_t)A.ncol - nf;
-    ZK_PROF(st, "fixed_axpy", (double)n * 16 * (1 + 2 * nf + nz),
-            hipLaunchKernelGGL(k_fixed_axpy, dim3((unsigned)((n + 255) / 256)), dim3(256), 0, st, fx.fpolys, fx.lagr, n, A,
-                               ws_dev, polys));
+    if (coeffs)
+        ZK_PROF(st, "fixed_axpy", (double)n * 16 * (1 + 2 * nf + nz),
+                hipLaunchKernelGGL(k_fixed_axpy, dim3((unsigned)((n + 255) / 256)), dim3(256), 0, st, fx.fpolys, fx.lagr, n,
+                                   A, ws_dev, polys));
     if (!E.ncol) return;
     ZK_PROF(st, "fixed_axpy", (double)B * n * 16 * (1 + ef + E.ncol),
             hipLaunchKernelGGL(k_fixed_axpy, dim3((unsigned)((B * n + 255) / 256)), dim3(256), 0, st, fx.flde,
@@ -414,7 +415,7 @@
 
 void zk::fixed_cols_axpy(hipStream_t st, const FixedColList &L, bool snapshot, const fe *src_polys, const fe *src_lde,
                          const fe *lagr, const fe *lagr_lde, const fe_ws *ws_dev, size_t n, size_t B, fe *polys, fe *lde,
-                         int lde_c0) {
+                         int lde_c0, bool coeffs) {
     if (L.count <= 0) return;
     AxpyCols A, E;
     A.ncol = L.count;
@@ -430,9 +431,10 @@
         E.ncol++;
     }
     const char *name = snapshot ? "fixed_snapshot" : "fixed_axpy";
-    ZK_PROF(st, name, (double)n * 16.0 * (1 + 2 * A.ncol),
-            hipLaunchKernelGGL(k_fixed_axpy, dim3((unsigned)((n + 255) / 256)), dim3(256), 0, st, src_polys, lagr, n, A,
-                               ws_dev, polys));
+    if (coeffs)
+        ZK_PROF(st, name, (double)n * 16.0 * (1 + 2 * A.ncol),
+                hipLaunchKernelGGL(k_fixed_axpy, dim3((unsigned)((n + 255) / 256)), dim3(256), 0, st, src_polys, lagr, n, A,
+                                   ws_dev, polys));
     if (!E.ncol) return;
     ZK_PROF(st, name, (double)B * n * 16.0 * (1 + 2 * E.ncol),
             hipLaunchKernelGGL(k_fixed_axpy, dim3((unsigned)((B * n + 255) / 256)), dim3(256), 0, st, src_lde, lagr_lde,
diff --git a/encrypt-zkvm_amd/csrc/zk_internal.hpp b/encrypt-zkvm_amd/csrc/zk_internal.hpp
--- a/encrypt-zkvm_amd/csrc/zk_internal.hpp
+++ b/encrypt-zkvm_amd/csrc/zk_internal.hpp
@@ -140,6 +140,20 @@
 };
 void fixed_hash(hipStream_t st, const FixedHashCols &A, const fe *lagr_lde, const fe_ws *ws_dev, fe *lde, int ncols,
                 int log_n, int log_b, int nb, uint8_t *leaves);
+struct CoeffSrc {
+    enum : uint8_t { PLAIN = 0, BASE = 1, ZERO = 2 };
+    static constexpr int MAXC = 28;
+    const fe *plane[MAXC];
+    uint8_t mode[MAXC];
+    const fe *lagr;
+    bool derived(int c) const { return mode[c] != PLAIN; }
+};
+inline CoeffSrc coeff_plain(const fe *tpolys, size_t n, int ncols = CoeffSrc::MAXC) {
+    CoeffSrc S{};
+    for (int c = 0; c < ncols; c++) S.plane[c] = tpolys + (size_t)c * n;
+    return S;
+}
+
 struct FriLayout {
     int lb, lcn;
 };
@@ -206,10 +220,10 @@
                        fe w8inv, fe inv3n, int ncols, fe *polys, unsigned *nonzero_flag);
 hipError_t eval_constraints(hipStream_t st, const fe *lde, int log_n, int log_b, const fe *periodic, const fe *divs,
                       const AirConsts *consts_dev, fe *comp, bool bnd = true, int nce = 8);
-void boundary_poly_add(hipStream_t st, const fe *tpolys, int log_n, const AirConsts &K, fe c, fe *scratch, fe *col0,
-                       unsigned *flag);
-const fe *boundary_range_begin(hipStream_t st, const fe *tpolys, int log_n, const AirConsts &K, fe c, fe *scratch,
-                               size_t k0, size_t kn);
+void boundary_poly_add(hipStream_t st, const CoeffSrc &S, const fe *w, int log_n, const AirConsts &K, fe c, fe *scratch,
+                       fe *col0, unsigned *flag);
+const fe *boundary_range_begin(hipStream_t st, const CoeffSrc &S, const fe *w, int log_n, const AirConsts &K, fe c,
+                               fe *scratch, size_t k0, size_t kn);
 void boundary_range_end(hipStream_t st, int log_n, fe c, fe *scratch, size_t k0, size_t kn, const fe *ext, fe *col0,
                         unsigned *flag);
 void comp_cross_coset(hipStream_t st, const fe *c, int log_n, const NttTables &T8n, const PowTable &inv3,
@@ -217,9 +231,12 @@
 
 int ood_waves(size_t n);
 template <class T>
-void ood_eval(hipStream_t st, const fe *tpolys, int W, const fe *cpolys, int C, int log_n, T z, T zg, fe *tab,
+void ood_eval(hipStream_t st, const CoeffSrc &S, int W, const fe *cpolys, int C, int log_n, T z, T zg, fe *tab,
               fe *partials, fe *out, int rank = 0, int G = 1);
+inline int ood_out_values(const CoeffSrc &S, int W, int C) { return 2 * W + C + (S.lagr ? 2 : 0); }
+void ood_fold_sources(int KX, int W, int C, const CoeffSrc &S, const fe *w, const fe *raw, fe *hv);
 void sum_partials(hipStream_t st, const fe *partials, int npolys, int nblk, fe *out, int b0 = 0, int b1 = -1);
+constexpr int ZK_DEEP_LAGR = 28;
 template <int KX>
 struct DeepConsts {
     typename Chal<KX>::T alpha_t[32];
@@ -227,6 +244,15 @@
     typename Chal<KX>::T k1, k2, z, zg;
 };
 static_assert(sizeof(DeepConsts<1>) == 52 * sizeof(fe) && sizeof(DeepConsts<2>) == 52 * sizeof(fe2), "DeepConsts layout");
+template <int KX>
+inline void deep_source_weight(DeepConsts<KX> &D, const CoeffSrc &S, const fe *w) {
+    typedef Chal<KX> X;
+    typename X::T s = X::zero();
+    if (S.lagr)
+        for (int c = 0; c < CoeffSrc::MAXC; c++)
+            if (S.derived(c)) s = X::add(s, X::mulb(D.alpha_t[c], w[c]));
+    D.alpha_t[ZK_DEEP_LAGR] = s;
+}
 void lde_cosets(hipStream_t st, const NttTables &Tn, const CosetTables &CT, const fe *coeffs, size_t n, size_t r0,
                 size_t stride, int count, fe *out, fe *ntt_tmp);
 constexpr size_t ZK_DEEP_BLOCK = 256;
@@ -244,16 +270,16 @@
     static size_t size(size_t n, int KX) { return KX * (4 * (2048 + n / 2048 + 2) + 3 * n + 2 * (n / ZK_DEEP_BLOCK + 1)); }
 };
 template <class T>
-const fe *deep_poly(hipStream_t st, const fe *tpolys, const fe *cpolys, int ccols, int log_n,
+const fe *deep_poly(hipStream_t st, const CoeffSrc &S, const fe *cpolys, int ccols, int log_n,
                     const void *deep_consts_dev, T z, T zg, fe *scratch);
 constexpr size_t ZK_DEEP_RANGE_QUANTUM = 2048;
 template <class T>
-const fe *deep_range_begin(hipStream_t st, const fe *tpolys, const fe *cpolys, int ccols, int log_n,
+const fe *deep_range_begin(hipStream_t st, const CoeffSrc &S, const fe *cpolys, int ccols, int log_n,
                            const void *deep_consts_dev, T z, T zg, fe *scratch, size_t k0, size_t kn);
 template <class T>
 const fe *deep_range_end(hipStream_t st, int log_n, T z, T zg, fe *scratch, size_t k0, size_t kn, const fe *ext);
 template <class T>
-void deep_coeff_launch(hipStream_t st, const NttTables &Tn, const fe *tpolys, const fe *cpolys, int ccols, int log_n,
+void deep_coeff_launch(hipStream_t st, const NttTables &Tn, const CoeffSrc &S, const fe *cpolys, int ccols, int log_n,
                        int log_b, const void *deep_consts_dev, T z, T zg, const CosetTables &CT, fe *scratch,
                        fe *ulde, fe *ntt_tmp, fe *out);
 template <int KX>
diff --git a/encrypt-zkvm_amd/zkvm_amd/native.py b/encrypt-zkvm_amd/zkvm_amd/native.py
--- a/encrypt-zkvm_amd/zkvm_amd/native.py
+++ b/encrypt-zkvm_amd/zkvm_amd/native.py
@@ -27,7 +27,7 @@
     "zk_prover_acquire", "zk_prover_release", "zk_prover_pool_trim", "zk_prover_trace_buffer",
     "zk_prove", "zk_prove_columns", "zk_prove_columns_ex", "zk_host_alloc", "zk_host_free", "zk_host_register",
     "zk_host_unregister", "zk_prove_device", "zk_lde_new", "zk_lde_read_frame", "zk_lde_query", "zk_lde_free",
-    "zk_eval_constraints", "zk_commit_composition", "zk_comp_query", "zk_comp_free", "zk_prover_stage_times", "zk_prover_profile", "zk_prover_kernel_stats", "zk_prover_kernel_ops", "zk_prover_exchange_stats", "zk_prover_exchange_stats_ex", "zk_prover_shard_schedule", "zk_prover_upload_stats", "zk_prover_upload_derived", "zk_prover_upload_fixed", "zk_prover_set_upload_schedule", "zk_prover_proof_info", "zk_vm_trace",
+    "zk_eval_constraints", "zk_commit_composition", "zk_comp_query", "zk_comp_free", "zk_prover_stage_times", "zk_prover_profile", "zk_prover_kernel_stats", "zk_prover_kernel_ops", "zk_prover_exchange_stats", "zk_prover_exchange_stats_ex", "zk_prover_shard_schedule", "zk_prover_upload_stats", "zk_prover_upload_derived", "zk_prover_upload_fixed", "zk_prover_coeff_sources", "zk_prover_set_upload_schedule", "zk_prover_proof_info", "zk_vm_trace",
     "zk_verify", "zk_comm_create_loopback", "zk_comm_unique_id", "zk_comm_create_rccl", "zk_comm_create_host", "zk_comm_destroy", "zk_comm_set_measure", "zk_comm_set_trace_split", "zk_prove_sharded",
     "zk_program_compile", "zk_program_trace", "zk_program_free", "zk_vm_last_error", "zk_vm_trace_device",
     "zk_vm_prove",
@@ -214,6 +214,11 @@
         L.zk_prover_upload_stats.argtypes = [vp, C.POINTER(C.c_uint64), C.POINTER(u32), C.POINTER(u32), C.POINTER(u32)]
         L.zk_prover_upload_derived.argtypes = [vp, C.POINTER(u32)]
         L.zk_prover_upload_fixed.argtypes = [vp, C.POINTER(u32)]
+        if hasattr(L, "zk_prover_coeff_sources"):
+            L.zk_prover_coeff_sources.argtypes = [vp, C.POINTER(u32)]
+            L.zk_diag_upload_plan_coeff_src.argtypes = [vp, sz]
+            L.zk_diag_coeff_sources.argtypes = [i32, vp, vp, vp, vp, i32, sz, i32, vp, vp, vp, vp, vp, vp, vp, vp, vp,
+                                                vp, vp]
         L.zk_prover_exchange_stats.argtypes = [vp, C.POINTER(C.c_char_p), C.POINTER(C.c_float), C.POINTER(C.c_double),
                                                C.POINTER(i32), i32, C.POINTER(i32)]
         L.zk_verify.argtypes = [vp, sz, C.POINTER(PubInputs), u32, C.c_char_p, sz]
diff --git a/encrypt-zkvm_amd/zkvm_amd/prover.py b/encrypt-zkvm_amd/zkvm_amd/prover.py
--- a/encrypt-zkvm_amd/zkvm_amd/prover.py
+++ b/encrypt-zkvm_amd/zkvm_amd/prover.py
@@ -183,6 +183,11 @@
         cols = lambda m: [c for c in range(28) if (m >> c) & 1]
         return {"bytes": b.value, "sparse": cols(sp.value), "narrow8": cols(n8.value), "narrow32": cols(n32.value),
                 "derived": cols(dv.value), "fixed": cols(fx.value)}
+
+    def coeff_sources(self) -> list:
+        m = C.c_uint32(0)
+        check(lib().zk_prover_coeff_sources(self.handle, C.byref(m)))
+        return [c for c in range(28) if (m.value >> c) & 1]
 
     UPLOAD_SCHEDULES = {"auto": 0, "throughput": 1, "latency": 2}
 
diff --git a/include/zkvm_gpu.h b/include/zkvm_gpu.h
--- a/include/zkvm_gpu.h
+++ b/include/zkvm_gpu.h
@@ -169,6 +169,7 @@
                            uint32_t *narrow32_cols);
 int zk_prover_upload_derived(zk_prover *p, uint32_t *derived_cols);
 int zk_prover_upload_fixed(zk_prover *p, uint32_t *fixed_cols);
+int zk_prover_coeff_sources(zk_prover *p, uint32_t *cols);
 enum { ZK_SCHED_AUTO = 0, ZK_SCHED_THROUGHPUT = 1, ZK_SCHED_LATENCY = 2 };
 int zk_prover_set_upload_schedule(zk_prover *p, int schedule);
 typedef struct {
```
